# openGemini/openGemini

Measured on NVIDIA H100. Metric: decoded+aggregated rows/s, higher is better.
Workload: dtype f64

## Files before the change

### include/ogpu.h

```cpp
#ifndef OGPU_H
#define OGPU_H

#include <stddef.h>
#include <stdint.h>

#ifdef __cplusplus
extern "C" {
#endif

#define OG_API __attribute__((visibility("default")))

enum {
    OG_OK = 0,
    OG_EOF = 1,
    OG_E_INVAL = -1,
    OG_E_CUDA = -2,
    OG_E_NOMEM = -3,
    OG_E_UNSUPPORTED = -4,
    OG_E_CORRUPT = -5,
    OG_E_ABORTED = -6,
    OG_E_TYPE = -7,
    OG_E_STATE = -8
};

enum { OG_TYPE_INT = 1, OG_TYPE_FLOAT = 3, OG_TYPE_STRING = 4, OG_TYPE_BOOL = 5 };

enum { OG_AGG_COUNT = 1, OG_AGG_SUM = 2, OG_AGG_MIN = 3, OG_AGG_MAX = 4, OG_AGG_FIRST = 5, OG_AGG_LAST = 6 };

enum { OG_F_TERM = 0, OG_F_AND = 1, OG_F_OR = 2 };
enum { OG_OP_LT = 0, OG_OP_LTE = 1, OG_OP_GT = 2, OG_OP_GTE = 3, OG_OP_EQ = 4, OG_OP_NEQ = 5 };

typedef struct og_filter_item {
    int32_t kind;
    int32_t column;
    int32_t op;
    int32_t const_is_float;
    double fval;
    int64_t ival;
} og_filter_item;

typedef struct og_call {
    int32_t func;
    int32_t column;
} og_call;

enum { OG_GROUP_ALL = 0, OG_GROUP_PER_SERIES = 1, OG_GROUP_MAP = 2 };
enum {
    OG_Q_STRICT_ORDER = 1u << 0
    ,
    OG_Q_NO_FUSED = 1u << 1
    ,
    OG_Q_NO_FAST = 1u << 2
    ,
    OG_Q_RESERVED_8 = 1u << 3
    ,
    OG_Q_QUERY_GRID = 1u << 4
};

typedef struct og_query_desc {
    int64_t interval;
    int64_t offset;
    int64_t tmin, tmax;
    int32_t ascending;
    uint32_t n_calls;
    const og_call *calls;
    uint32_t n_filter;
    const og_filter_item *filter;
    int32_t group_mode;
    uint32_t n_groups;
    const uint32_t *series_group;
    int32_t chunk_size;
    uint32_t flags;
} og_query_desc;

typedef struct og_column_desc {
    const char *name;
    int32_t type;
    const uint64_t *page_off;
    const uint32_t *page_len;
} og_column_desc;

enum {
    OG_SHARD_DEVICE_DATA = 1u << 0
};

typedef struct og_shard_desc {
    const uint8_t *data;
    uint64_t data_len;
    uint32_t n_series;
    const uint64_t *sids;
    const uint32_t *series_seg_begin;
    uint32_t n_segments;
    const int64_t *seg_tmin;
    const int64_t *seg_tmax;
    uint32_t n_columns;
    const og_column_desc *columns;
    const uint64_t *time_page_off;
    const uint32_t *time_page_len;
    uint32_t flags;
} og_shard_desc;

typedef struct og_colval_view {
    const uint8_t *val;
    uint64_t val_bytes;
    const uint8_t *bitmap;
    const int64_t *times;
    int32_t type;
    int32_t len;
    int32_t nil_count;
    int32_t bitmap_offset;
} og_colval_view;

typedef struct og_record_view {
    uint32_t n_cols;
    const og_colval_view *cols;
    const int64_t *times;
    int32_t rows;
    uint32_t group;
    uint64_t sid;
} og_record_view;

typedef struct og_dense_col {
    void *values;
    uint8_t *valid;
    int64_t *times;
    int32_t type;
    int32_t func;
} og_dense_col;

typedef struct og_dense_view {
    uint32_t n_groups;
    uint32_t n_buckets;
    int64_t start;
    int64_t interval;
    uint32_t n_cols;
    const og_dense_col *cols;
    void *stream;
} og_dense_view;

typedef struct og_stats {
    uint64_t rows_decoded;
    uint64_t segments_scanned;
    uint64_t page_bytes;
    uint64_t dir_bytes;
    uint64_t out_bytes;
    double kernel_ms;
    double h2d_ms;
    double main_kernel_ms;
    uint32_t kernel_launches;
    int32_t path;
    int32_t il_state;
    int32_t per_series_cells_used;
    double il_build_ms;
    uint64_t il_bytes;
    uint64_t general_segments;
    double merge_ms;
    uint64_t il_packed_segments;
} og_stats;

typedef struct og_shard og_shard;
typedef struct og_query og_query;

OG_API int og_init(int device_ordinal);
OG_API int og_device_count(void);
OG_API const char *og_strerror(int status);
OG_API const char *og_last_error(void);
OG_API const char *og_version(void);
OG_API int og_release_cached_memory(void);

typedef struct og_tssp og_tssp;
OG_API int og_tssp_parse(const uint8_t *file, uint64_t len, og_tssp **out);
OG_API int og_tssp_desc(const og_tssp *t, og_shard_desc *out);
OG_API const char *og_tssp_measurement(const og_tssp *t);
OG_API int og_tssp_time_range(const og_tssp *t, int64_t *min_time, int64_t *max_time);
OG_API void og_tssp_free(og_tssp *t);

OG_API int og_shard_open(const og_shard_desc *desc, og_shard **out);
OG_API void og_shard_close(og_shard *s);
OG_API int og_shard_info(const og_shard *s, uint64_t *n_series, uint64_t *n_segments, uint64_t *n_rows,
                         uint64_t *page_bytes, int64_t *tmin, int64_t *tmax);

enum { OG_FILE_OUT_OF_ORDER = 1u << 0 };
OG_API int og_shard_open_files(const og_shard_desc *files, const uint32_t *file_flags, uint32_t n_files, og_shard **out);
typedef struct og_merge_info {
    uint32_t n_files, n_out_of_order_files;
    uint64_t series_merged;
    uint64_t out_of_order_rows;
    uint64_t rows_replaced;
    uint64_t rows_after_merge;
    uint64_t segments_kept;
    uint64_t segments_rewritten_in, segments_rewritten_out;
    double merge_ms;
} og_merge_info;
OG_API int og_shard_merge_info(const og_shard *s, og_merge_info *out);

OG_API int og_shard_append_files(og_shard *s, const og_shard_desc *files, const uint32_t *file_flags, uint32_t n_files);

typedef struct og_compact_desc {
    uint32_t rows_per_segment;
    uint32_t flags;
} og_compact_desc;
typedef struct og_compact_info {
    uint64_t series_rewritten;
    uint64_t segments_kept;
    uint64_t segments_rewritten_in, segments_rewritten_out;
    uint64_t rows_rewritten;
    double compact_ms;
} og_compact_info;
OG_API int og_shard_compact(og_shard *s, const og_compact_desc *d, og_compact_info *info );

OG_API int og_query_create(og_shard *s, const og_query_desc *desc, og_query **out);
OG_API int og_query_run(og_query *q);
OG_API int og_query_next(og_query *q, og_record_view *out);
OG_API int og_query_dense(og_query *q, og_dense_view *out);
OG_API int og_query_stats(const og_query *q, og_stats *out);
OG_API void og_query_abort(og_query *q);
OG_API void og_query_destroy(og_query *q);

OG_API int og_query_merge_dense(og_query *q, const og_dense_view *other);

typedef struct og_comm og_comm;
OG_API int og_comm_unique_id(uint8_t id[128]);
OG_API int og_comm_init_rank(const uint8_t id[128], int rank, int world, og_comm **out);
OG_API void og_comm_destroy(og_comm *c);
OG_API int og_comm_info(const og_comm *c, int *rank, int *world, int *nccl_version);
OG_API int og_comm_allreduce_f64(og_comm *c, double *vals, int n, int op_max);
OG_API int og_query_allreduce(og_query *q, og_comm *c);

OG_API int og_decode_segment(og_shard *s, uint32_t segment, og_record_view *out);
enum { OG_DECODE_DESCENDING = 1u << 0 };
OG_API int og_decode_segment_ex(og_shard *s, uint32_t segment, uint32_t flags, og_record_view *out);
OG_API int og_decode_column_device(og_shard *s, uint32_t column, uint32_t seg_begin, uint32_t seg_end,
                                   void *d_values, uint64_t value_stride_bytes, uint32_t *d_rows_out);

enum { OG_SYNTH_F_HI = 0, OG_SYNTH_F_LO = 1, OG_SYNTH_INT_WALK = 2, OG_SYNTH_BOOL = 3 };
typedef struct og_synth_column {
    int32_t type;
    int32_t dist;
    uint32_t null_permille;
} og_synth_column;
typedef struct og_synth_desc {
    uint32_t n_series;
    uint32_t rows_per_series;
    uint32_t rows_per_segment;
    int64_t t0;
    int64_t dt;
    uint64_t seed;
    uint32_t n_columns;
    const og_synth_column *columns;
    uint32_t series_base;
} og_synth_desc;
OG_API int og_shard_synth(const og_synth_desc *desc, og_shard **out);
typedef struct og_shard_layout {
    uint64_t data_len;
    uint32_t n_series, n_segments, n_columns;
} og_shard_layout;
OG_API int og_shard_layout_get(const og_shard *s, og_shard_layout *out);
OG_API int og_shard_export(const og_shard *s, uint8_t *data, uint64_t *sids, uint32_t *series_seg_begin,
                           int64_t *seg_tmin, int64_t *seg_tmax, uint64_t *page_off ,
                           uint32_t *page_len, int32_t *col_types );

OG_API int og_encode_pages(int32_t type, int32_t is_time, const void *d_values, const uint8_t *d_valid,
                           const uint32_t *d_rows , uint32_t n_segments,
                           uint32_t rows_per_segment, uint8_t *d_out, uint64_t out_cap, uint64_t *d_page_off,
                           uint32_t *d_page_len, uint64_t *total_bytes_out);

typedef struct og_downsampled og_downsampled;
OG_API int og_downsample(og_shard *s, uint32_t column, int64_t interval, int64_t tmin, int64_t tmax, og_downsampled **out);

typedef struct og_downsample_ops {
    int32_t type;
    uint32_t n_funcs;
    const int32_t *funcs;
} og_downsample_ops;
typedef struct og_downsample_desc {
    int64_t interval, tmin, tmax;
    uint32_t n_types;
    const og_downsample_ops *ops;
} og_downsample_desc;
OG_API int og_downsample_shard(og_shard *s, const og_downsample_desc *d, og_downsampled **out);
OG_API int og_downsampled_timing(const og_downsampled *d, double phase_ms[4]);
OG_API int og_downsampled_desc(const og_downsampled *d, og_shard_desc *desc, uint64_t *rows );
OG_API int og_downsampled_export(const og_downsampled *d, uint8_t *host_data );
OG_API void og_downsampled_free(og_downsampled *d);

typedef struct og_tssp_write_desc {
    const char *measurement;
    uint32_t series_begin, series_end;
    uint32_t flags;
} og_tssp_write_desc;
typedef struct og_tssp_image og_tssp_image;
OG_API int og_shard_write_tssp(og_shard *s, const og_tssp_write_desc *d, og_tssp_image **out);
OG_API int og_tssp_image_size(const og_tssp_image *f, uint64_t *bytes);
OG_API int og_tssp_image_export(const og_tssp_image *f, uint8_t *host);
OG_API int og_tssp_image_timing(const og_tssp_image *f, double phase_ms[4]);
OG_API void og_tssp_image_free(og_tssp_image *f);

#ifdef __cplusplus
}
#endif
#endif
```

### opengemini_b200/_lib.py

```python
import ctypes as C
import os

_HERE = os.path.dirname(os.path.abspath(__file__))
LIB_PATH = os.environ.get("OGPU_LIB") or os.path.join(_HERE, "libogpu.so")

OG_OK, OG_EOF = 0, 1
OG_E_INVAL, OG_E_CUDA, OG_E_NOMEM, OG_E_UNSUPPORTED, OG_E_CORRUPT, OG_E_ABORTED, OG_E_TYPE, OG_E_STATE = -1, -2, -3, -4, -5, -6, -7, -8
TYPE_INT, TYPE_FLOAT, TYPE_STRING, TYPE_BOOL = 1, 3, 4, 5
AGG_COUNT, AGG_SUM, AGG_MIN, AGG_MAX, AGG_FIRST, AGG_LAST = 1, 2, 3, 4, 5, 6
F_TERM, F_AND, F_OR = 0, 1, 2
OP_LT, OP_LTE, OP_GT, OP_GTE, OP_EQ, OP_NEQ = 0, 1, 2, 3, 4, 5
GROUP_ALL, GROUP_PER_SERIES, GROUP_MAP = 0, 1, 2
Q_STRICT_ORDER = 1
Q_NO_FUSED = 2
Q_NO_FAST = 4
Q_QUERY_GRID = 16
SYNTH_F_HI, SYNTH_F_LO, SYNTH_INT_WALK, SYNTH_BOOL = 0, 1, 2, 3
SHARD_DEVICE_DATA = 1
FILE_OUT_OF_ORDER = 1

u8p, u32p, u64p, i64p, i32p = C.POINTER(C.c_uint8), C.POINTER(C.c_uint32), C.POINTER(C.c_uint64), C.POINTER(C.c_int64), C.POINTER(C.c_int32)


class FilterItem(C.Structure):
    _fields_ = [("kind", C.c_int32), ("column", C.c_int32), ("op", C.c_int32), ("const_is_float", C.c_int32),
                ("fval", C.c_double), ("ival", C.c_int64)]


class Call(C.Structure):
    _fields_ = [("func", C.c_int32), ("column", C.c_int32)]


class QueryDesc(C.Structure):
    _fields_ = [("interval", C.c_int64), ("offset", C.c_int64), ("tmin", C.c_int64), ("tmax", C.c_int64),
                ("ascending", C.c_int32), ("n_calls", C.c_uint32), ("calls", C.POINTER(Call)),
                ("n_filter", C.c_uint32), ("filter", C.POINTER(FilterItem)), ("group_mode", C.c_int32),
                ("n_groups", C.c_uint32), ("series_group", u32p), ("chunk_size", C.c_int32), ("flags", C.c_uint32)]


class ColumnDesc(C.Structure):
    _fields_ = [("name", C.c_char_p), ("type", C.c_int32), ("page_off", u64p), ("page_len", u32p)]


class ShardDesc(C.Structure):
    _fields_ = [("data", u8p), ("data_len", C.c_uint64), ("n_series", C.c_uint32), ("sids", u64p),
                ("series_seg_begin", u32p), ("n_segments", C.c_uint32), ("seg_tmin", i64p), ("seg_tmax", i64p),
                ("n_columns", C.c_uint32), ("columns", C.POINTER(ColumnDesc)), ("time_page_off", u64p),
                ("time_page_len", u32p), ("flags", C.c_uint32)]


class ColValView(C.Structure):
    _fields_ = [("val", u8p), ("val_bytes", C.c_uint64), ("bitmap", u8p), ("times", i64p), ("type", C.c_int32),
                ("len", C.c_int32), ("nil_count", C.c_int32), ("bitmap_offset", C.c_int32)]


class RecordView(C.Structure):
    _fields_ = [("n_cols", C.c_uint32), ("cols", C.POINTER(ColValView)), ("times", i64p), ("rows", C.c_int32),
                ("group", C.c_uint32), ("sid", C.c_uint64)]


class DenseCol(C.Structure):
    _fields_ = [("values", C.c_void_p), ("valid", C.c_void_p), ("times", C.c_void_p), ("type", C.c_int32), ("func", C.c_int32)]


class DenseView(C.Structure):
    _fields_ = [("n_groups", C.c_uint32), ("n_buckets", C.c_uint32), ("start", C.c_int64), ("interval", C.c_int64),
                ("n_cols", C.c_uint32), ("cols", C.POINTER(DenseCol)), ("stream", C.c_void_p)]


class Stats(C.Structure):
    _fields_ = [("rows_decoded", C.c_uint64), ("segments_scanned", C.c_uint64), ("page_bytes", C.c_uint64),
                ("dir_bytes", C.c_uint64), ("out_bytes", C.c_uint64), ("kernel_ms", C.c_double), ("h2d_ms", C.c_double), ("main_kernel_ms", C.c_double),
                ("kernel_launches", C.c_uint32), ("path", C.c_int32), ("il_state", C.c_int32), ("per_series_cells_used", C.c_int32),
                ("il_build_ms", C.c_double), ("il_bytes", C.c_uint64), ("general_segments", C.c_uint64), ("merge_ms", C.c_double),
                ("il_packed_segments", C.c_uint64)]


class SynthColumn(C.Structure):
    _fields_ = [("type", C.c_int32), ("dist", C.c_int32), ("null_permille", C.c_uint32)]


class SynthDesc(C.Structure):
    _fields_ = [("n_series", C.c_uint32), ("rows_per_series", C.c_uint32), ("rows_per_segment", C.c_uint32),
                ("t0", C.c_int64), ("dt", C.c_int64), ("seed", C.c_uint64), ("n_columns", C.c_uint32),
                ("columns", C.POINTER(SynthColumn)), ("series_base", C.c_uint32)]


class ShardLayout(C.Structure):
    _fields_ = [("data_len", C.c_uint64), ("n_series", C.c_uint32), ("n_segments", C.c_uint32), ("n_columns", C.c_uint32)]


class DownsampleOps(C.Structure):
    _fields_ = [("type", C.c_int32), ("n_funcs", C.c_uint32), ("funcs", i32p)]


class DownsampleDesc(C.Structure):
    _fields_ = [("interval", C.c_int64), ("tmin", C.c_int64), ("tmax", C.c_int64), ("n_types", C.c_uint32),
                ("ops", C.POINTER(DownsampleOps))]


class MergeInfo(C.Structure):
    _fields_ = [("n_files", C.c_uint32), ("n_out_of_order_files", C.c_uint32), ("series_merged", C.c_uint64),
                ("out_of_order_rows", C.c_uint64), ("rows_replaced", C.c_uint64), ("rows_after_merge", C.c_uint64),
                ("segments_kept", C.c_uint64), ("segments_rewritten_in", C.c_uint64), ("segments_rewritten_out", C.c_uint64),
                ("merge_ms", C.c_double)]


class CompactDesc(C.Structure):
    _fields_ = [("rows_per_segment", C.c_uint32), ("flags", C.c_uint32)]


class CompactInfo(C.Structure):
    _fields_ = [("series_rewritten", C.c_uint64), ("segments_kept", C.c_uint64), ("segments_rewritten_in", C.c_uint64),
                ("segments_rewritten_out", C.c_uint64), ("rows_rewritten", C.c_uint64), ("compact_ms", C.c_double)]


class TsspWriteDesc(C.Structure):
    _fields_ = [("measurement", C.c_char_p), ("series_begin", C.c_uint32), ("series_end", C.c_uint32), ("flags", C.c_uint32)]


EXPORTS = [
    "og_init", "og_device_count", "og_strerror", "og_last_error", "og_version", "og_shard_open", "og_shard_close",
    "og_shard_info", "og_query_create", "og_query_run", "og_query_next", "og_query_dense", "og_query_stats",
    "og_query_abort", "og_query_destroy", "og_query_merge_dense", "og_decode_segment", "og_decode_segment_ex", "og_decode_column_device",
    "og_shard_synth", "og_shard_layout_get", "og_shard_export", "og_encode_pages",
    "og_release_cached_memory", "og_comm_unique_id", "og_comm_init_rank", "og_comm_destroy", "og_comm_info", "og_comm_allreduce_f64", "og_query_allreduce",
    "og_downsample", "og_downsampled_desc", "og_downsampled_export", "og_downsampled_free",
    "og_downsample_shard", "og_downsampled_timing",
    "og_tssp_parse", "og_tssp_desc", "og_tssp_measurement", "og_tssp_time_range", "og_tssp_free",
    "og_shard_open_files", "og_shard_merge_info", "og_shard_append_files", "og_shard_compact",
    "og_shard_write_tssp", "og_tssp_image_size", "og_tssp_image_export", "og_tssp_image_timing", "og_tssp_image_free",
]

_lib = None


class OgpuError(RuntimeError):
    def __init__(self, status, where):
        self.status = status
        msg = lib().og_last_error().decode(errors="replace")
        super().__init__(f"{where}: {lib().og_strerror(status).decode()} ({status}) {msg}")


def lib():
    global _lib
    if _lib is not None:
        return _lib
    if not os.path.exists(LIB_PATH):
        raise RuntimeError(f"{LIB_PATH} is missing: run `python -c 'import __graft_entry__ as g; g.build()'` "
                           "(nvcc, sm_90a). There is no CPU fallback for the scan/aggregate path.")
    L = C.CDLL(LIB_PATH)
    L.og_strerror.restype = C.c_char_p
    L.og_strerror.argtypes = [C.c_int]
    L.og_last_error.restype = C.c_char_p
    L.og_version.restype = C.c_char_p
    L.og_init.argtypes = [C.c_int]
    L.og_shard_open.argtypes = [C.POINTER(ShardDesc), C.POINTER(C.c_void_p)]
    L.og_shard_open_files.argtypes = [C.POINTER(ShardDesc), u32p, C.c_uint32, C.POINTER(C.c_void_p)]
    L.og_shard_merge_info.argtypes = [C.c_void_p, C.POINTER(MergeInfo)]
    L.og_shard_append_files.argtypes = [C.c_void_p, C.POINTER(ShardDesc), u32p, C.c_uint32]
    L.og_shard_compact.argtypes = [C.c_void_p, C.POINTER(CompactDesc), C.POINTER(CompactInfo)]
    L.og_shard_close.argtypes = [C.c_void_p]
    L.og_shard_close.restype = None
    L.og_shard_info.argtypes = [C.c_void_p, u64p, u64p, u64p, u64p, i64p, i64p]
    L.og_query_create.argtypes = [C.c_void_p, C.POINTER(QueryDesc), C.POINTER(C.c_void_p)]
    L.og_query_run.argtypes = [C.c_void_p]
    L.og_query_next.argtypes = [C.c_void_p, C.POINTER(RecordView)]
    L.og_query_dense.argtypes = [C.c_void_p, C.POINTER(DenseView)]
    L.og_query_stats.argtypes = [C.c_void_p, C.POINTER(Stats)]
    L.og_query_abort.argtypes = [C.c_void_p]
    L.og_query_abort.restype = None
    L.og_query_destroy.argtypes = [C.c_void_p]
    L.og_query_destroy.restype = None
    L.og_query_merge_dense.argtypes = [C.c_void_p, C.POINTER(DenseView)]
    L.og_decode_segment.argtypes = [C.c_void_p, C.c_uint32, C.POINTER(RecordView)]
    L.og_downsample.argtypes = [C.c_void_p, C.c_uint32, C.c_int64, C.c_int64, C.c_int64, C.POINTER(C.c_void_p)]
    L.og_downsample_shard.argtypes = [C.c_void_p, C.POINTER(DownsampleDesc), C.POINTER(C.c_void_p)]
    L.og_downsampled_timing.argtypes = [C.c_void_p, C.POINTER(C.c_double)]
    L.og_downsampled_desc.argtypes = [C.c_void_p, C.POINTER(ShardDesc), C.POINTER(C.c_uint64)]
    L.og_downsampled_export.argtypes = [C.c_void_p, C.c_void_p]
    L.og_downsampled_free.argtypes = [C.c_void_p]
    L.og_downsampled_free.restype = None
    L.og_tssp_parse.argtypes = [C.c_void_p, C.c_uint64, C.POINTER(C.c_void_p)]
    L.og_tssp_desc.argtypes = [C.c_void_p, C.POINTER(ShardDesc)]
    L.og_tssp_measurement.argtypes = [C.c_void_p]
    L.og_tssp_measurement.restype = C.c_char_p
    L.og_tssp_time_range.argtypes = [C.c_void_p, C.POINTER(C.c_int64), C.POINTER(C.c_int64)]
    L.og_tssp_free.argtypes = [C.c_void_p]
    L.og_tssp_free.restype = None
    L.og_shard_write_tssp.argtypes = [C.c_void_p, C.POINTER(TsspWriteDesc), C.POINTER(C.c_void_p)]
    L.og_tssp_image_size.argtypes = [C.c_void_p, u64p]
    L.og_tssp_image_export.argtypes = [C.c_void_p, C.c_void_p]
    L.og_tssp_image_timing.argtypes = [C.c_void_p, C.POINTER(C.c_double)]
    L.og_tssp_image_free.argtypes = [C.c_void_p]
    L.og_tssp_image_free.restype = None
    L.og_decode_segment_ex.argtypes = [C.c_void_p, C.c_uint32, C.c_uint32, C.POINTER(RecordView)]
    L.og_decode_column_device.argtypes = [C.c_void_p, C.c_uint32, C.c_uint32, C.c_uint32, C.c_void_p, C.c_uint64, C.c_void_p]
    L.og_shard_synth.argtypes = [C.POINTER(SynthDesc), C.POINTER(C.c_void_p)]
    L.og_shard_layout_get.argtypes = [C.c_void_p, C.POINTER(ShardLayout)]
    L.og_shard_export.argtypes = [C.c_void_p, C.c_void_p, C.c_void_p, C.c_void_p, C.c_void_p, C.c_void_p, C.c_void_p, C.c_void_p, C.c_void_p]
    L.og_encode_pages.argtypes = [C.c_int32, C.c_int32, C.c_void_p, C.c_void_p, C.c_void_p, C.c_uint32, C.c_uint32,
                                  C.c_void_p, C.c_uint64, C.c_void_p, C.c_void_p, u64p]
    L.og_comm_unique_id.argtypes = [C.c_void_p]
    L.og_comm_init_rank.argtypes = [C.c_void_p, C.c_int, C.c_int, C.POINTER(C.c_void_p)]
    L.og_comm_destroy.argtypes = [C.c_void_p]
    L.og_comm_destroy.restype = None
    L.og_comm_info.argtypes = [C.c_void_p, C.POINTER(C.c_int), C.POINTER(C.c_int), C.POINTER(C.c_int)]
    L.og_comm_allreduce_f64.argtypes = [C.c_void_p, C.POINTER(C.c_double), C.c_int, C.c_int]
    L.og_query_allreduce.argtypes = [C.c_void_p, C.c_void_p]
    _lib = L
    return L


def check(status, where):
    if status != OG_OK:
        raise OgpuError(status, where)
```

### opengemini_b200/csrc/agg_kernels.cuh

```cuda
#pragma once
#include "agg_ops.cuh"
#include "decode.cuh"
#include "internal.h"

namespace ogpu {

#define OG_NO_BUCKET 0xFFFFFFFFu

struct DirP {
    const uint8_t *data;
    const uint64_t *page_off;
    const uint32_t *page_len;
    const uint32_t *seg_series, *seg_rows, *series_seg_begin;
    const int64_t *seg_tmin, *seg_tmax;
    uint32_t n_segments, n_columns;
};

struct ChunkP {
    uint32_t series_begin, series_end;
    uint32_t seg_begin, seg_end;
    Tri cells[OG_MAX_CALLS];
    uint32_t nb;
    Tri edges[OG_MAX_CALLS];
    uint32_t *edge_bucket;
    Tri gcells[OG_MAX_CALLS];
    uint32_t gc_cols, gc_tail0, gc_edge0, gc_col0;
    uint32_t J;
    int *err;
    int *flags;
};

__device__ __forceinline__ size_t cell_idx(const ChunkP &ch, uint32_t series, uint32_t b) { return (size_t)(series - ch.series_begin) * ch.nb + b; }

__device__ __forceinline__ void report_err(int *err, int code, uint32_t seg) {
    if (atomicCAS(&err[0], 0, code) == 0) err[1] = (int)seg;
}

__device__ __forceinline__ void store_part(const Tri &a, size_t i, const Part &p) {
    a.val[i] = p.v; a.ok[i] = (uint8_t)p.ok;
    if (a.tim) a.tim[i] = p.t;
}
__device__ __forceinline__ Part load_part(const Tri &a, size_t i) {
    Part p; p.ok = a.ok[i]; p.v = a.val[i]; p.t = a.tim ? a.tim[i] : 0; return p;
}
__device__ __forceinline__ void store_cell(const ChunkP &ch, int call, uint32_t series, uint32_t b, const Part &p) {
    store_part(ch.cells[call], cell_idx(ch, series, b), p);
    ch.flags[0] = 1;
}

struct SegWindows {
    const QueryP &q; const ChunkP &ch;
    const uint32_t seg; const size_t e; const uint32_t series;
    uint32_t cur_b = OG_NO_BUCKET, head_b = OG_NO_BUCKET; bool head_done = false;
    int64_t we = 0;

    __device__ __forceinline__ SegWindows(const QueryP &q_, const ChunkP &ch_, uint32_t seg_, size_t e_, uint32_t series_)
        : q(q_), ch(ch_), seg(seg_), e(e_), series(series_) {}
    template <int NC> __device__ __forceinline__ void flush(const Part (&parts)[NC], bool final) {
        if (cur_b == OG_NO_BUCKET) return;
#pragma unroll
        for (int c = 0; c < NC; c++) {
            if (!head_done) store_part(ch.edges[c], e, parts[c]);
            else if (final) store_part(ch.edges[c], e + 1, parts[c]);
            else if (parts[c].ok) store_cell(ch, c, series, cur_b, parts[c]);
        }
        if (!head_done) { head_done = true; head_b = cur_b; }
    }
    template <int NC> __device__ __forceinline__ bool enter(int64_t t, Part (&parts)[NC]) {
        if (cur_b != OG_NO_BUCKET && t < we) return true;
        flush(parts, false);
        cur_b = bucket_of(t, q.start, q.interval);
        if (cur_b >= q.n_buckets) { report_err(ch.err, D_CORRUPT, seg); cur_b = OG_NO_BUCKET; return false; }
        we = q.start + (int64_t)(cur_b + 1) * q.interval;
#pragma unroll
        for (int c = 0; c < NC; c++) parts[c] = part_empty();
        return true;
    }
    template <int NC> __device__ __forceinline__ void end(const Part (&parts)[NC]) {
        const uint32_t last_b = cur_b;
        const bool single = !head_done;
        flush(parts, true);
        ch.edge_bucket[e] = head_b;
        ch.edge_bucket[e + 1] = (single || head_b == OG_NO_BUCKET) ? OG_NO_BUCKET : last_b;
        if (head_b != OG_NO_BUCKET) ch.flags[1] = 1;
    }
};

__global__ void k_validate(DirP d, const int32_t *col_types, uint32_t *seg_rows, unsigned long long *totals ,
                           uint32_t *max_rows, int *err) {
    uint32_t seg = blockIdx.x * blockDim.x + threadIdx.x;
    if (seg >= d.n_segments) return;
    size_t ti = (size_t)d.n_columns * d.n_segments + seg;
    TimeDesc t;
    int rc = parse_time_page(d.data + d.page_off[ti], d.page_len[ti], t);
    if (rc == D_OK && t.rows == 0) rc = D_CORRUPT;
    if (rc == D_OK) {
        int64_t last = t.t0; bool unsorted = false;
        if (t.kind == 0) last = (int64_t)((uint64_t)t.t0 + (uint64_t)(t.rows - 1) * t.delta);
        else {
            TimeIter it; it.init(t);
            for (uint32_t i = 0; i < t.rows; i++) { const int64_t x = it.next(); unsorted |= x < last; last = x; }
            it.finish(); rc = it.err;
        }
        if (rc == D_OK && (t.t0 < d.seg_tmin[seg] || last > d.seg_tmax[seg] || last < t.t0 || unsorted)) rc = D_CORRUPT;
    }
    if (rc != D_OK) { report_err(err, rc, seg); seg_rows[seg] = 0; return; }
    seg_rows[seg] = t.rows;
    unsigned long long bytes = d.page_len[ti];
    for (uint32_t c = 0; c < d.n_columns; c++) {
        size_t pi = (size_t)c * d.n_segments + seg;
        uint32_t len = d.page_len[pi];
        if (len == 0) continue;
        bytes += len;
        PageHdr h;
        rc = parse_field_header(d.data + d.page_off[pi], len, col_types[c], t.rows, h);
        if (rc == D_OK && h.rows != t.rows) rc = D_CORRUPT;
        if (rc == D_OK && h.bitmap && hdr_valid_rows(h) != h.rows - h.nil_count) rc = D_CORRUPT;
        if (rc == D_OK && !h.one_row && h.nil_count < h.rows) {
            if (h.block_len < 1) rc = D_CORRUPT;
            else {
                int tag = __ldg(h.block) >> 4, ty = col_types[c];
                if (ty == OG_TYPE_FLOAT) rc = (tag == 0 || tag == 3 || tag == 4 || tag == 5) ? D_OK : (tag == 1 || tag == 2 || tag == 6) ? D_UNSUPPORTED : D_CORRUPT;
                else if (ty == OG_TYPE_INT) rc = (tag == 1 || tag == 2 || tag == 4) ? D_OK : tag == 3 ? D_UNSUPPORTED : D_CORRUPT;
                else if (ty == OG_TYPE_BOOL) rc = tag == 1 ? D_OK : D_CORRUPT;
                else if (ty == OG_TYPE_STRING) rc = D_OK;
                else rc = D_UNSUPPORTED;
            }
        }
        if (rc != D_OK) { report_err(err, rc, seg); return; }
    }
    atomicAdd(&totals[0], (unsigned long long)t.rows);
    atomicAdd(&totals[1], bytes);
    atomicMax(max_rows, t.rows);
    if (t.kind != 0 && t.kind != 3) atomicAdd(&totals[2], 1ull);
}

__global__ void k_fill_seg_series(const uint32_t *series_seg_begin, uint32_t n_series, uint32_t *seg_series) {
    uint32_t s = blockIdx.x;
    if (s >= n_series) return;
    for (uint32_t g = series_seg_begin[s] + threadIdx.x; g < series_seg_begin[s + 1]; g += blockDim.x) seg_series[g] = s;
}

struct TileP {
    uint32_t tile_begin, tile_end, R;
    uint32_t S;
    uint64_t *vals[OG_MAX_COLS];
    uint8_t *okb[OG_MAX_COLS];
    int64_t *times;
    uint8_t *keep;
};

__global__ void k_decode_tile(DirP d, QueryP q, TileP tp, int *err) {
    uint32_t seg = tp.tile_begin + blockIdx.x * blockDim.x + threadIdx.x;
    if (seg >= tp.tile_end) return;
    uint32_t slot = blockIdx.y;
    const size_t base = seg - tp.tile_begin, S = tp.S;
    uint32_t rows = d.seg_rows[seg];
    if (slot == q.n_cols) {
        size_t ti = (size_t)d.n_columns * d.n_segments + seg;
        TimeDesc t;
        int rc = parse_time_page(d.data + d.page_off[ti], d.page_len[ti], t);
        if (rc == D_OK) {
            TimeIter it; it.init(t);
            for (uint32_t i = 0; i < t.rows; i++) tp.times[base + i * S] = it.next();
            it.finish(); rc = it.err;
        }
        if (rc != D_OK) report_err(err, rc, seg);
        return;
    }
    size_t pi = (size_t)q.col_index[slot] * d.n_segments + seg;
    uint64_t *out = tp.vals[slot] + base; uint8_t *okb = tp.okb[slot] + base;
    ColIter it;
    it.init(d.data + d.page_off[pi], d.page_len[pi], q.col_type[slot], rows);
    for (uint32_t i = 0; i < rows; i++) { uint64_t v = 0; okb[i * S] = it.next(v); out[i * S] = v; }
    it.finish();
    if (it.err != D_OK) report_err(err, it.err, seg);
}

__device__ __forceinline__ bool term_pass(const FilterP &f, uint64_t raw) {
// ... 7 lines not shown
        case OG_OP_GTE: return !(v < c);
        case OG_OP_EQ: return !(v != c);
        default: return !(v == c);
        }
    }
    int64_t v = f.type == OG_TYPE_BOOL ? (int64_t)(raw != 0) : (int64_t)raw, c = f.ival;
    switch (f.op) {
    case OG_OP_LT: return !(v >= c);
    case OG_OP_LTE: return !(v > c);
    case OG_OP_GT: return !(v <= c);
    case OG_OP_GTE: return !(v < c);
    case OG_OP_EQ: return !(v != c);
    default: return !(v == c);
    }
}

__global__ void k_filter_tile(DirP d, QueryP q, TileP tp) {
    size_t idx = (size_t)blockIdx.x * blockDim.x + threadIdx.x;
    size_t total = (size_t)tp.S * tp.R;
    if (idx >= total) return;
    uint32_t row = (uint32_t)(idx / tp.S), sl = (uint32_t)(idx % tp.S);
    if (sl >= tp.tile_end - tp.tile_begin) return;
    if (row >= d.seg_rows[tp.tile_begin + sl]) { tp.keep[idx] = 0; return; }
    int64_t t = tp.times[idx];
    bool keep = t >= q.tmin && t <= q.tmax;
    if (keep && q.n_filter) {
        uint32_t stack = 0; int sp = 0;
        for (uint32_t i = 0; i < q.n_filter; i++) {
            const FilterP &f = q.filter[i];
            if (f.kind == OG_F_TERM) {
                bool pass = tp.okb[f.col_slot][idx] && term_pass(f, tp.vals[f.col_slot][idx]);
                stack |= (uint32_t)pass << sp; sp++;
            } else {
                uint32_t b = (stack >> (sp - 1)) & 1, a = (stack >> (sp - 2)) & 1;
                uint32_t r = f.kind == OG_F_AND ? (a & b) : (a | b);
                sp -= 2; stack &= ~(3u << sp); stack |= r << sp; sp++;
            }
        }
        keep = stack & 1;
    }
    tp.keep[idx] = keep;
}

__global__ void k_window_reduce(DirP d, QueryP q, TileP tp, ChunkP ch) {
    uint32_t sl = blockIdx.x * blockDim.x + threadIdx.x;
    uint32_t seg = tp.tile_begin + sl;
    if (seg >= tp.tile_end) return;
    const uint32_t rows = d.seg_rows[seg], series = d.seg_series[seg];
    const size_t S = tp.S, e = 2 * (size_t)(seg - ch.seg_begin);
    Part parts[OG_MAX_CALLS];
    uint32_t cur_b = OG_NO_BUCKET, head_b = OG_NO_BUCKET; bool head_done = false;
    int64_t we = 0;
    auto flush = [&](bool final) {
        if (cur_b == OG_NO_BUCKET) return;
        for (uint32_t c = 0; c < q.n_calls; c++) {
            if (!head_done) store_part(ch.edges[c], e, parts[c]);
            else if (final) store_part(ch.edges[c], e + 1, parts[c]);
            else if (parts[c].ok) store_cell(ch, (int)c, series, cur_b, parts[c]);
        }
        if (!head_done) { head_done = true; head_b = cur_b; }
    };
    for (uint32_t r = 0; r < rows; r++) {
        const size_t ix = (size_t)r * S + sl;
        const int64_t t = tp.times[ix];
        if (t < q.tmin) continue;
        if (t > q.tmax) break;
        if (cur_b == OG_NO_BUCKET || t >= we) {
            flush(false);
            cur_b = bucket_of(t, q.start, q.interval);
            if (cur_b >= q.n_buckets) { report_err(ch.err, D_CORRUPT, seg); cur_b = OG_NO_BUCKET; break; }
            we = q.start + (int64_t)(cur_b + 1) * q.interval;
#pragma unroll
            for (uint32_t c = 0; c < OG_MAX_CALLS; c++) parts[c] = part_empty();
        }
        if (!tp.keep[ix]) continue;
#pragma unroll
        for (uint32_t c = 0; c < OG_MAX_CALLS; c++) {
            if (c >= q.n_calls) break;
            const CallP &cp = q.calls[c];
            if (tp.okb[cp.col_slot][ix]) acc_row(cp.func, cp.type, parts[c], tp.vals[cp.col_slot][ix], t);
        }
    }
    flush(true);
    ch.edge_bucket[e] = head_b;
    ch.edge_bucket[e + 1] = (head_b == OG_NO_BUCKET || cur_b == head_b) ? OG_NO_BUCKET : cur_b;
}

struct EdgeRuns { uint32_t hb, tb, s_end; bool head_leader; };
__device__ __forceinline__ EdgeRuns edge_runs(const DirP &d, const ChunkP &ch, uint32_t seg, uint32_t series) {
    EdgeRuns r;
    const uint32_t s_first = d.series_seg_begin[series];
    r.s_end = d.series_seg_begin[series + 1];
    const uint32_t *eb = ch.edge_bucket;
    const size_t e = 2 * (size_t)(seg - ch.seg_begin);
    r.hb = eb[e]; r.tb = eb[e + 1];
    r.head_leader = true;
    if (r.hb != OG_NO_BUCKET && seg > s_first) {
        const size_t pe = e - 2;
        const uint32_t pb = eb[pe + 1] != OG_NO_BUCKET ? eb[pe + 1] : eb[pe];
        if (pb != OG_NO_BUCKET && pb == r.hb) r.head_leader = false;
    }
    return r;
}
__device__ __forceinline__ Part edge_stitch(const QueryP &q, const ChunkP &ch, const EdgeRuns &r, uint32_t seg, int which, uint32_t c) {
    const CallP &cp = q.calls[c];
    const uint32_t *eb = ch.edge_bucket;
    const size_t e = 2 * (size_t)(seg - ch.seg_begin);
    const uint32_t b = which == 0 ? r.hb : r.tb;
    Part acc = load_part(ch.edges[c], e + which);
    if (which == 1 || r.tb == OG_NO_BUCKET) {
        for (uint32_t nx = seg + 1; nx < r.s_end; nx++) {
            const size_t ne = 2 * (size_t)(nx - ch.seg_begin);
            if (eb[ne] != b) break;
            acc = series_merge(cp.func, cp.type, acc, load_part(ch.edges[c], ne));
            if (eb[ne + 1] != OG_NO_BUCKET) break;
        }
    }
    return acc;
}

__global__ void k_fix_edges(DirP d, QueryP q, ChunkP ch) {
    uint32_t seg = ch.seg_begin + blockIdx.x * blockDim.x + threadIdx.x;
    if (seg >= ch.seg_end) return;
    const uint32_t series = d.seg_series[seg];
    const EdgeRuns r = edge_runs(d, ch, seg, series);
    if (r.hb == OG_NO_BUCKET) return;
    for (int which = 0; which < 2; which++) {
        if (which == 0 && !r.head_leader) continue;
        if (which == 1 && r.tb == OG_NO_BUCKET) continue;
        const uint32_t b = which == 0 ? r.hb : r.tb;
        if (b >= q.n_buckets) { report_err(ch.err, D_CORRUPT, seg); continue; }
        for (uint32_t c = 0; c < q.n_calls; c++) {
            const Part acc = edge_stitch(q, ch, r, seg, which, c);
            if (acc.ok) store_cell(ch, (int)c, series, b, acc);
        }
    }
}

__device__ __forceinline__ Part shfl_xor_part(const Part &p, int o, bool with_time) {
    Part r; r.v = __shfl_xor_sync(0xffffffffu, p.v, o); r.ok = __shfl_xor_sync(0xffffffffu, p.ok, o);
    r.t = with_time ? __shfl_xor_sync(0xffffffffu, p.t, o) : 0;
    return r;
}
__device__ __forceinline__ Part warp_fold(int func, int type, bool multi, Part p, bool with_time) {
#pragma unroll
    for (int o = 16; o; o >>= 1) { const Part other = shfl_xor_part(p, o, with_time); group_update(func, type, multi, p, other); }
    return p;
}
__device__ __forceinline__ bool call_has_time(const QueryP &q, uint32_t c) { return q.calls[c].func >= OG_AGG_MIN && !(q.multi && q.calls[c].func <= OG_AGG_MAX); }
__device__ __forceinline__ int call_ftype(const QueryP &q, uint32_t c) { return q.calls[c].func == OG_AGG_COUNT ? OG_TYPE_INT : q.calls[c].type; }

__global__ void k_fix_edges_fold(DirP d, QueryP q, ChunkP ch) {
    if (ch.flags[1] == 0) return;
    const uint32_t w = (blockIdx.x * blockDim.x + threadIdx.x) >> 5, lane = threadIdx.x & 31;
    const uint32_t n_blk = (ch.series_end - ch.series_begin + 31) / 32;
    if (w >= n_blk * ch.J) return;
    const uint32_t blk = w / ch.J, j = w % ch.J;
    const uint32_t series = ch.series_begin + blk * 32 + lane;
    const bool in = series < ch.series_end;
    const uint32_t seg = in ? d.series_seg_begin[series] + j : 0;
    EdgeRuns r; r.hb = r.tb = OG_NO_BUCKET; r.head_leader = false; r.s_end = 0;
    if (in) r = edge_runs(d, ch, seg, series);
    const uint32_t n_bk = (ch.gc_cols - ch.gc_edge0) / 3;
    for (int which = 0; which < 2; which++) {
        const uint32_t gcol = ch.gc_edge0 + (which ? 2u : (j & 1u)) * n_bk + ch.series_begin / 32 + blk - ch.gc_col0;
        const bool has = r.hb != OG_NO_BUCKET && (which == 0 ? r.head_leader : r.tb != OG_NO_BUCKET);
        const uint32_t b = which == 0 ? r.hb : r.tb;
        const uint32_t hm = __ballot_sync(0xffffffffu, has);
        if (hm == 0) continue;
        const int leader = __ffs(hm) - 1;
        const uint32_t bL = __shfl_sync(0xffffffffu, b, leader);
        const bool unif = __all_sync(0xffffffffu, !has || b == bL) && bL < q.n_buckets;
        if (!unif && has && b >= q.n_buckets) { report_err(ch.err, D_CORRUPT, seg); continue; }
        for (uint32_t c = 0; c < q.n_calls; c++) {
            Part acc = part_empty();
            if (has) acc = edge_stitch(q, ch, r, seg, which, c);
            if (unif) {
                acc = warp_fold(q.calls[c].func, call_ftype(q, c), q.multi != 0, acc, call_has_time(q, c));
                if ((int)lane == leader && acc.ok) store_part(ch.gcells[c], (size_t)bL * ch.gc_cols + gcol, acc);
            } else if (has && acc.ok) store_cell(ch, (int)c, series, b, acc);
        }
    }
}

struct GroupP {
    const uint32_t *grp_begin;
    const uint32_t *grp_series;
    uint32_t n_groups;
    Tri dense[OG_MAX_CALLS];
};

__global__ void k_merge_groups(QueryP q, ChunkP ch, GroupP gp) {
    if (ch.flags[0] == 0) return;
    size_t idx = (size_t)blockIdx.x * blockDim.x + threadIdx.x;
    size_t total = (size_t)gp.n_groups * q.n_buckets;
    if (idx >= total) return;
    uint32_t g = (uint32_t)(idx / q.n_buckets), b = (uint32_t)(idx % q.n_buckets);
    uint32_t lo = gp.grp_begin[g], hi = gp.grp_begin[g + 1];
    {
        uint32_t a = lo, z = hi;
        while (a < z) { uint32_t m = (a + z) >> 1; if (gp.grp_series[m] < ch.series_begin) a = m + 1; else z = m; }
        lo = a;
    }
    if (lo >= hi || gp.grp_series[lo] >= ch.series_end) return;
    {
        const uint32_t c = blockIdx.y;
        const CallP &cp = q.calls[c];
        Part acc = load_part(gp.dense[c], idx);
        const Tri cells = ch.cells[c];
        constexpr int U = 16;
        for (uint32_t i = lo; i < hi; i += U) {
            uint32_t okv[U]; uint64_t vv[U]; int64_t tt[U];
#pragma unroll
            for (int u = 0; u < U; u++) {
                uint32_t ii = i + u;
                uint32_t s = ii < hi ? gp.grp_series[ii] : 0xffffffffu;
                bool in = s < ch.series_end;
                size_t ci = in ? cell_idx(ch, s, b) : 0;
                okv[u] = in ? cells.ok[ci] : 0;
                vv[u] = okv[u] ? cells.val[ci] : 0;
                tt[u] = (okv[u] && cells.tim) ? cells.tim[ci] : 0;
            }
#pragma unroll
            for (int u = 0; u < U; u++) {
                if (!okv[u]) continue;
                Part p; p.ok = 1; p.v = vv[u]; p.t = tt[u];
                group_update(cp.func, cp.out_type == OG_TYPE_INT && cp.func == OG_AGG_COUNT ? OG_TYPE_INT : cp.type, q.multi != 0, acc, p);
            }
        }
        store_part(gp.dense[c], idx, acc);
    }
}

__global__ void k_merge_per_series(QueryP q, ChunkP ch, GroupP gp) {
    const uint32_t c = blockIdx.y;
    const size_t n = (size_t)(ch.series_end - ch.series_begin) * q.n_buckets;
    const size_t i = (size_t)blockIdx.x * blockDim.x + threadIdx.x;
    if (i >= n) return;
    const CallP &cp = q.calls[c];
    const int ftype = cp.out_type == OG_TYPE_INT && cp.func == OG_AGG_COUNT ? OG_TYPE_INT : cp.type;
    const uint32_t b = (uint32_t)(i % q.n_buckets);
    Part p; p.ok = ch.cells[c].ok[i]; p.v = p.ok ? ch.cells[c].val[i] : 0; p.t = (p.ok && ch.cells[c].tim) ? ch.cells[c].tim[i] : 0;
    Part a; a.v = 0; a.ok = 0; a.t = q.multi ? 0 : q.start + (int64_t)b * q.interval;
    group_update(cp.func, ftype, q.multi != 0, a, p);
    store_part(gp.dense[c], (size_t)ch.series_begin * q.n_buckets + i, a);
}

#define OG_MERGE_SB 256u
__global__ void __launch_bounds__(128) k_merge_all_blocks(QueryP q, ChunkP ch, GroupP gp) {
    if (ch.flags[0] == 0) return;
    const uint32_t b = blockIdx.x * blockDim.x + threadIdx.x, blk = blockIdx.y, c = blockIdx.z;
    if (b >= q.n_buckets) return;
    const uint32_t nS = ch.series_end - ch.series_begin;
    const uint32_t s0 = blk * OG_MERGE_SB, s1 = min(nS, s0 + OG_MERGE_SB);
    const int func = q.calls[c].func, ftype = call_ftype(q, c);
    const bool multi = q.multi != 0;
    const Tri cells = ch.cells[c];
    Part acc = part_empty();
    constexpr int U = 8;
    for (uint32_t s = s0; s < s1; s += U) {
        uint32_t okv[U]; uint64_t vv[U]; int64_t tt[U];
#pragma unroll
        for (int u = 0; u < U; u++) {
            const bool in = s + u < s1;
            const size_t ci = in ? (size_t)(s + u) * ch.nb + b : 0;
            okv[u] = in ? cells.ok[ci] : 0;
            vv[u] = okv[u] ? cells.val[ci] : 0;
            tt[u] = (okv[u] && cells.tim) ? cells.tim[ci] : 0;
        }
#pragma unroll
        for (int u = 0; u < U; u++) {
            if (!okv[u]) continue;
            Part p; p.ok = 1; p.v = vv[u]; p.t = tt[u];
            group_update(func, ftype, multi, acc, p);
        }
    }
    if (acc.ok) store_part(ch.gcells[c], (size_t)b * ch.gc_cols + blk, acc);
}

__global__ void k_merge_folded(QueryP q, ChunkP ch, GroupP gp) {
    const uint32_t b = (blockIdx.x * blockDim.x + threadIdx.x) >> 5, lane = threadIdx.x & 31, c = blockIdx.y;
    if (b >= q.n_buckets) return;
    const int func = q.calls[c].func, ftype = call_ftype(q, c);
    const bool wt = call_has_time(q, c), multi = q.multi != 0;
    const Tri g = ch.gcells[c];
    Part acc = part_empty();
    const size_t row = (size_t)b * ch.gc_cols;
    for (uint32_t col = lane; col < ch.gc_cols; col += 32) {
        if (!g.ok[row + col]) continue;
        Part p; p.ok = 1; p.v = g.val[row + col]; p.t = wt ? g.tim[row + col] : 0;
        group_update(func, ftype, multi, acc, p);
    }
    acc = warp_fold(func, ftype, multi, acc, wt);
    if (lane == 0 && acc.ok) {
        Part a = load_part(gp.dense[c], b);
        group_update(func, ftype, multi, a, acc);
        store_part(gp.dense[c], b, a);
    }
}

__global__ void k_init_dense(QueryP q, GroupP gp) {
    size_t idx = (size_t)blockIdx.x * blockDim.x + threadIdx.x;
    size_t total = (size_t)gp.n_groups * q.n_buckets;
    if (idx >= total) return;
    uint32_t b = (uint32_t)(idx % q.n_buckets);
    for (uint32_t c = 0; c < q.n_calls; c++) {
        gp.dense[c].val[idx] = 0; gp.dense[c].ok[idx] = 0;
        if (gp.dense[c].tim) gp.dense[c].tim[idx] = q.multi ? 0 : q.start + (int64_t)b * q.interval;
    }
}

__global__ void k_merge_dense(QueryP q, GroupP mine, GroupP other) {
    size_t idx = (size_t)blockIdx.x * blockDim.x + threadIdx.x;
    size_t total = (size_t)mine.n_groups * q.n_buckets;
    if (idx >= total) return;
    for (uint32_t c = 0; c < q.n_calls; c++) {
        const CallP &cp = q.calls[c];
        Part a = load_part(mine.dense[c], idx), p = load_part(other.dense[c], idx);
        group_update(cp.func, cp.func == OG_AGG_COUNT ? OG_TYPE_INT : cp.type, q.multi != 0, a, p);
        store_part(mine.dense[c], idx, a);
    }
}

}
```

### opengemini_b200/csrc/api.cu

```cuda
#include <algorithm>
#include <cstdarg>
#include <cstdio>
#include <cstring>
#include <numeric>

#include "agg_kernels.cuh"
#include "il_build.cuh"
#include "fused_multi.cuh"
#include "fused_cols.cuh"
#include "snappy_load.cuh"
#include <cub/device/device_scan.cuh>
#include <cub/device/device_radix_sort.cuh>
#include "internal.h"

namespace ogpu {

static thread_local char g_err[512] = "";
void set_error(const char *fmt, ...) {
    va_list ap; va_start(ap, fmt); vsnprintf(g_err, sizeof g_err, fmt, ap); va_end(ap);
}
int cuda_fail(cudaError_t e, const char *what, const char *file, int line) {
    set_error("CUDA error %d (%s) at %s:%d: %s", (int)e, cudaGetErrorString(e), file, line, what);
    return OG_E_CUDA;
}
// ... 247 lines not shown
}

OG_API int og_shard_export(const og_shard *s, uint8_t *data, uint64_t *sids, uint32_t *series_seg_begin, int64_t *seg_tmin,
                           int64_t *seg_tmax, uint64_t *page_off, uint32_t *page_len, int32_t *col_types) {
    if (!s) return OG_E_INVAL;
    CU(cudaSetDevice(s->device));
    size_t nseg = s->n_segments, ncol1 = (size_t)s->n_columns + 1;
    if (data) CU(cudaMemcpy(data, s->d_data, s->data_len, cudaMemcpyDeviceToHost));
    if (sids) memcpy(sids, s->sids.data(), s->sids.size() * 8);
    if (series_seg_begin) memcpy(series_seg_begin, s->h_series_seg_begin.data(), s->h_series_seg_begin.size() * 4);
    if (seg_tmin) CU(cudaMemcpy(seg_tmin, s->d_tmin, nseg * 8, cudaMemcpyDeviceToHost));
    if (seg_tmax) CU(cudaMemcpy(seg_tmax, s->d_tmax, nseg * 8, cudaMemcpyDeviceToHost));
    if (page_off) CU(cudaMemcpy(page_off, s->d_page_off, ncol1 * nseg * 8, cudaMemcpyDeviceToHost));
    if (page_len) CU(cudaMemcpy(page_len, s->d_page_len, ncol1 * nseg * 4, cudaMemcpyDeviceToHost));
    if (col_types) memcpy(col_types, s->col_types.data(), s->col_types.size() * 4);
    return OG_OK;
}

static const int64_t MIN_TIME = INT64_MIN + 2, MAX_TIME = INT64_MAX - 1;
static void window_of(int64_t interval, int64_t offset, int64_t tmin, int64_t tmax, int64_t t, int64_t *s, int64_t *e) {
    if (interval == 0) { *s = tmin; *e = tmax + 1; return; }
    t -= offset;
    int64_t dt = t % interval;
    if (dt < 0) dt += interval;
    int64_t st = ((int64_t)((uint64_t)MIN_TIME + (uint64_t)dt) >= t) ? MIN_TIME : t - dt;
    st += offset;
    int64_t d2 = interval - dt;
    int64_t en = (MAX_TIME - d2 <= t) ? MAX_TIME : t + d2;
    en += offset;
    *s = st; *e = en;
}
static bool window_clamped(int64_t interval, int64_t offset, int64_t t) {
    const __int128 x = (__int128)t - offset;
    __int128 r = x % interval;
    if (r < 0) r += interval;
    const __int128 s = x - r, e = s + interval;
    return s < MIN_TIME || e > MAX_TIME || s + offset < INT64_MIN || e + offset > INT64_MAX;
}

}
namespace { void free_plan(void *plan); }
extern "C" void og_query_free_merge_state(void *p);
og_query::~og_query() {
    if (stream) cudaStreamSynchronize(stream);
    if (live) { std::lock_guard<std::mutex> lock(live->mu); live->n--; }
    og_query_free_merge_state(merge_state);
    free_plan(plan);
    if (ev0) cudaEventDestroy(ev0);
    if (ev1) cudaEventDestroy(ev1);
    for (cudaEvent_t e : main_ev) cudaEventDestroy(e);
    if (stream) cudaStreamDestroy(stream);
}
extern "C" {
OG_API void og_query_destroy(og_query *q) { delete q; }

OG_API int og_query_create(og_shard *s, const og_query_desc *d_in, og_query **out) {
    if (!s || !d_in || !out) { set_error("null argument"); return OG_E_INVAL; }
    *out = nullptr;
    og_query_desc d_clamped = *d_in;
    d_clamped.tmin = std::max(d_in->tmin, MIN_TIME); d_clamped.tmax = std::min(d_in->tmax, MAX_TIME);
    const og_query_desc *d = &d_clamped;
    CU(cudaSetDevice(s->device));
    if (d->n_calls == 0 || d->n_calls > OG_MAX_CALLS) { set_error("n_calls must be 1..%d", OG_MAX_CALLS); return OG_E_INVAL; }
    if (d->n_filter > OG_MAX_FILTER) { set_error("filter too long (max %d items)", OG_MAX_FILTER); return OG_E_INVAL; }
    if (d->interval < 0 || d->tmin > d->tmax) { set_error("bad interval or time range"); return OG_E_INVAL; }
    std::unique_ptr<og_query> q(new og_query);
    {
        std::lock_guard<std::mutex> lock(s->live->mu);
        s->live->n++;
        q->sh = s; q->live = s->live;
    }
    q->desc = *d;
    q->calls.assign(d->calls, d->calls + d->n_calls);
    if (d->n_filter) q->filter.assign(d->filter, d->filter + d->n_filter);
    q->desc.calls = q->calls.data(); q->desc.filter = q->filter.data();
    QueryP &p = q->qp;
    memset(&p, 0, sizeof p);
    auto slot_of = [&](int col) -> int {
        for (uint32_t i = 0; i < p.n_cols; i++) if (p.col_index[i] == col) return (int)i;
        if (p.n_cols >= OG_MAX_COLS) return -1;
        p.col_index[p.n_cols] = col; p.col_type[p.n_cols] = s->col_types[col];
        return (int)p.n_cols++;
    };
    for (uint32_t i = 0; i < d->n_calls; i++) {
        const og_call &c = d->calls[i];
        if (c.column < 0 || (uint32_t)c.column >= s->n_columns || c.func < OG_AGG_COUNT || c.func > OG_AGG_LAST) { set_error("call %u: bad column or function", i); return OG_E_INVAL; }
        int type = s->col_types[c.column];
        if (type == OG_TYPE_STRING && c.func != OG_AGG_COUNT) { set_error("call %u: only count() is pushed down for string columns (their values are never decoded on the GPU path)", i); return OG_E_UNSUPPORTED; }
        if (c.func == OG_AGG_SUM && type == OG_TYPE_BOOL) { set_error("sum() over a boolean column (unsupported sum iterator type, series_call_processor.go:140)"); return OG_E_INVAL; }
        int sl = slot_of(c.column);
        if (sl < 0) { set_error("too many distinct columns"); return OG_E_INVAL; }
        p.calls[i].func = c.func; p.calls[i].col_slot = sl; p.calls[i].type = type;
        p.calls[i].out_type = c.func == OG_AGG_COUNT ? OG_TYPE_INT : type;
    }
    p.n_calls = d->n_calls; p.multi = d->n_calls > 1;
    int sp = 0;
    for (uint32_t i = 0; i < d->n_filter; i++) {
        const og_filter_item &f = d->filter[i];
        FilterP &fp = p.filter[i];
        fp.kind = f.kind;
        if (f.kind == OG_F_TERM) {
            if (f.column < 0 || (uint32_t)f.column >= s->n_columns || f.op < OG_OP_LT || f.op > OG_OP_NEQ) { set_error("filter item %u: bad column or op", i); return OG_E_INVAL; }
            if (s->col_types[f.column] == OG_TYPE_STRING) { set_error("filter item %u: WHERE on a string column is not pushed down", i); return OG_E_UNSUPPORTED; }
            int sl = slot_of(f.column);
            if (sl < 0) { set_error("too many distinct columns"); return OG_E_INVAL; }
            fp.col_slot = sl; fp.op = f.op; fp.type = s->col_types[f.column]; fp.const_is_float = f.const_is_float; fp.fval = f.fval; fp.ival = f.ival;
            sp++;
        } else if (f.kind == OG_F_AND || f.kind == OG_F_OR) {
            if (sp < 2) { set_error("filter RPN underflow at item %u", i); return OG_E_INVAL; }
            sp--;
        } else { set_error("filter item %u: bad kind", i); return OG_E_INVAL; }
    }
    if (d->n_filter && sp != 1) { set_error("filter RPN does not reduce to one value"); return OG_E_INVAL; }
    p.n_filter = d->n_filter;
    int64_t gmin = std::max(d->tmin, s->tmin), gmax = std::min(d->tmax, s->tmax);
    bool overlap = gmin <= gmax;
    if (!overlap) gmin = gmax = d->tmin;
    if (d->flags & OG_Q_QUERY_GRID) {
        if (d_in->tmin <= MIN_TIME || d_in->tmax >= MAX_TIME) { set_error("OG_Q_QUERY_GRID needs a bounded time range"); return OG_E_INVAL; }
        gmin = d->tmin; gmax = d->tmax; overlap = true;
    }
    int64_t s0, e0, s1, e1;
    if (d->interval == 0) { s0 = gmin; e0 = gmax + 1; s1 = s0; e1 = e0; }
    else {
        if (overlap && (window_clamped(d->interval, d->offset, gmin) || window_clamped(d->interval, d->offset, gmax))) {
            set_error("the first or last window of the range is clamped at the int64 time limits"); return OG_E_UNSUPPORTED;
        }
        window_of(d->interval, d->offset, d->tmin, d->tmax, gmin, &s0, &e0);
        window_of(d->interval, d->offset, d->tmin, d->tmax, gmax + 1, &s1, &e1);
    }
    p.tmin = d->tmin; p.tmax = d->tmax; p.start = s0; p.interval = e0 - s0;
    if (p.interval <= 0) { set_error("degenerate window"); return OG_E_INVAL; }
    uint64_t nb = d->interval ? (uint64_t)(e1 - s0) / (uint64_t)p.interval : 1;
    if (nb == 0 || nb > 0x7fffffffull) { set_error("query range yields %llu buckets", (unsigned long long)nb); return OG_E_INVAL; }
    p.n_buckets = (uint32_t)nb;
    q->n_groups = d->group_mode == OG_GROUP_ALL ? 1 : d->group_mode == OG_GROUP_PER_SERIES ? s->n_series : d->n_groups;
    if (d->group_mode == OG_GROUP_MAP) {
        if (!d->series_group || d->n_groups == 0) { set_error("OG_GROUP_MAP needs series_group and n_groups"); return OG_E_INVAL; }
        q->series_group.assign(d->series_group, d->series_group + s->n_series);
        for (uint32_t g : q->series_group) if (g >= d->n_groups) { set_error("series_group entry out of range"); return OG_E_INVAL; }
    } else if (d->group_mode != OG_GROUP_ALL && d->group_mode != OG_GROUP_PER_SERIES) { set_error("bad group_mode"); return OG_E_INVAL; }
    if (q->n_groups == 0) q->n_groups = 1;
    cudaError_t e = cudaStreamCreateWithFlags(&q->stream, cudaStreamNonBlocking);
    if (e != cudaSuccess) return cuda_fail(e, "cudaStreamCreate", __FILE__, __LINE__);
    cudaEventCreate(&q->ev0); cudaEventCreate(&q->ev1);
    *out = q.release();
    return OG_OK;
}

OG_API void og_query_abort(og_query *q) { if (q) q->aborted = 1; }

}
namespace {
struct Plan {
    ChunkP ch; TileP tp; GroupP gp;
    bool fused;
    bool cols;
    bool multi;
    bool fast;
    bool blockmerge;
    bool fold;
    int fm; bool times;
    IlP il;
    const og_shard::IlCol *ic;
};
void free_plan(void *plan) { delete (Plan *)plan; }

template <int NC> void launch_fused(const DirP &d, const QueryP &p, const ChunkP &ch, const uint32_t *list, uint32_t n, cudaStream_t st) {
    if (n) k_fused_segment<NC><<<(n + 127) / 128, 128, 0, st>>>(d, p, ch, list, n);
}
template <int FM, bool TIMES> void launch_fast_t(bool fold, const IlP &il, uint32_t g0, uint32_t g1, const QueryP &p, const ChunkP &ch, cudaStream_t st) {
    constexpr uint32_t WPB = OG_FAST_THREADS / 32;
    dim3 grid((g1 - g0 + WPB - 1) / WPB), block(OG_FAST_THREADS);
    if (fold) k_fused_il<FM, TIMES, true><<<grid, block, WPB * il_acc_bytes(p.n_calls, TIMES), st>>>(p, ch, il, g0, g1);
    else k_fused_il<FM, TIMES, false><<<grid, block, 0, st>>>(p, ch, il, g0, g1);
}
void launch_fast(int fm, bool times, bool fold, const IlP &il, uint32_t g0, uint32_t g1, const QueryP &p, const ChunkP &ch, cudaStream_t st) {
    if (g1 <= g0) return;
    if (!times) {
        switch (fm) {
        case FM_SUM | FM_COUNT: return launch_fast_t<FM_SUM | FM_COUNT, false>(fold, il, g0, g1, p, ch, st);
        case FM_SUM | FM_COUNT | FM_MAX: return launch_fast_t<FM_SUM | FM_COUNT | FM_MAX, false>(fold, il, g0, g1, p, ch, st);
        case FM_SUM | FM_COUNT | FM_MIN | FM_MAX: return launch_fast_t<FM_SUM | FM_COUNT | FM_MIN | FM_MAX, false>(fold, il, g0, g1, p, ch, st);
        case FM_COUNT: return launch_fast_t<FM_COUNT, false>(fold, il, g0, g1, p, ch, st);
        default: break;
        }
    } else {
        switch (fm) {
        case FM_MAX | FM_COUNT: return launch_fast_t<FM_MAX | FM_COUNT, true>(fold, il, g0, g1, p, ch, st);
        case FM_MIN | FM_COUNT: return launch_fast_t<FM_MIN | FM_COUNT, true>(fold, il, g0, g1, p, ch, st);
        default: break;
        }
    }
    return launch_fast_t<63, true>(fold, il, g0, g1, p, ch, st);
}

template <int NCOL, int NCALL> void launch_multi_t(const QueryP &p, const DirP &d, const ChunkP &ch, uint32_t nseg, cudaStream_t st) {
    bool simple = true;
    for (uint32_t c = 0; c < p.n_calls; c++) simple &= p.calls[c].func == OG_AGG_COUNT || p.calls[c].func == OG_AGG_SUM;
    const unsigned gb = (nseg + 127) / 128;
    if (simple) k_fused_multi<NCOL, NCALL, true><<<gb, 128, 0, st>>>(d, p, ch);
    else k_fused_multi<NCOL, NCALL, false><<<gb, 128, 0, st>>>(d, p, ch);
}
template <int NCOL> void launch_multi_c(const QueryP &p, const DirP &d, const ChunkP &ch, uint32_t nseg, cudaStream_t st) {
    switch (p.n_calls) {
    case 1: return launch_multi_t<NCOL, 1>(p, d, ch, nseg, st);
    case 2: return launch_multi_t<NCOL, 2>(p, d, ch, nseg, st);
    case 3: return launch_multi_t<NCOL, 3>(p, d, ch, nseg, st);
    case 4: return launch_multi_t<NCOL, 4>(p, d, ch, nseg, st);
    case 5: return launch_multi_t<NCOL, 5>(p, d, ch, nseg, st);
    case 6: return launch_multi_t<NCOL, 6>(p, d, ch, nseg, st);
    case 7: return launch_multi_t<NCOL, 7>(p, d, ch, nseg, st);
    default: return launch_multi_t<NCOL, 8>(p, d, ch, nseg, st);
    }
}
void launch_cols(const QueryP &p, const DirP &d, const ChunkP &ch, uint32_t nseg, cudaStream_t st) {
    bool simple = true;
    for (uint32_t c = 0; c < p.n_calls; c++) simple &= p.calls[c].func == OG_AGG_COUNT || p.calls[c].func == OG_AGG_SUM;
    const unsigned gb = (nseg + 127) / 128;
    if (simple) k_fused_cols<true><<<gb, 128, 0, st>>>(d, p, ch);
    else k_fused_cols<false><<<gb, 128, 0, st>>>(d, p, ch);
}
void launch_multi(const QueryP &p, const DirP &d, const ChunkP &ch, uint32_t nseg, cudaStream_t st) {
    switch (p.n_cols) {
    case 1: return launch_multi_c<1>(p, d, ch, nseg, st);
    case 2: return launch_multi_c<2>(p, d, ch, nseg, st);
    case 3: return launch_multi_c<3>(p, d, ch, nseg, st);
#ifdef OG_WIDE_MULTI
    case 5: return launch_multi_c<5>(p, d, ch, nseg, st);
    case 6: return launch_multi_c<6>(p, d, ch, nseg, st);
    case 7: return launch_multi_c<7>(p, d, ch, nseg, st);
    case 8: return launch_multi_c<8>(p, d, ch, nseg, st);
#endif
    default: return launch_multi_c<4>(p, d, ch, nseg, st);
    }
}

int ensure_il(og_shard *s, int col, cudaStream_t st) {
    std::lock_guard<std::mutex> lock(s->il_mu);
    if (s->il.size() != s->n_columns) s->il.resize(s->n_columns);
    og_shard::IlCol &ic = s->il[col];
    if (ic.state != 0) return OG_OK;
    ic.state = -1;
    if (s->n_segments == 0 || s->col_types[col] != OG_TYPE_FLOAT) return OG_OK;
    const uint32_t nseg = s->n_segments;
    uint32_t J = s->n_series ? s->h_series_seg_begin[1] - s->h_series_seg_begin[0] : 0;
    for (uint32_t i = 0; i < s->n_series && J; i++) if (s->h_series_seg_begin[i + 1] - s->h_series_seg_begin[i] != J) J = 0;
    const uint32_t n_super = J ? (s->n_series + OG_IL_SUPER - 1) / OG_IL_SUPER : 1;
    const uint64_t n_dom64 = J ? (uint64_t)n_super * J : 1;
    if (n_dom64 >= (1ull << 31)) return OG_OK;
    const uint32_t n_dom = (uint32_t)n_dom64;
    int rc;
    struct Ev { cudaEvent_t e = nullptr; Ev() { cudaEventCreate(&e); } ~Ev() { if (e) cudaEventDestroy(e); } } ev0, ev1;
    cudaEventRecord(ev0.e, st);
    Scratch tmp(st);
    IlScanOut so{};
    uint32_t *seg_words; uint64_t *keys2; uint32_t *vals2;
    if ((rc = tmp.get(&so.seg_win, nseg)) || (rc = tmp.get(&so.n_packed, 1)) ||
        (rc = tmp.get(&seg_words, nseg)) || (rc = tmp.get(&so.seg_t0, nseg)) || (rc = tmp.get(&so.seg_dt, nseg)) || (rc = tmp.get(&so.keys, nseg)) ||
        (rc = tmp.get(&so.vals, nseg)) || (rc = tmp.get(&keys2, nseg)) || (rc = tmp.get(&vals2, nseg)) || (rc = tmp.get(&so.dom_cnt, n_dom))) return rc;
    so.seg_words = seg_words;
    if ((rc = tmp.get(&so.misaligned, 1))) return rc;
    CU(cudaMemsetAsync(so.dom_cnt, 0, (size_t)n_dom * 4, st));
    CU(cudaMemsetAsync(so.misaligned, 0, 4, st));
    CU(cudaMemsetAsync(so.n_packed, 0, 8, st));
    DirP d = make_dir(s);
    k_il_scan<<<(nseg + 255) / 256, 256, 0, st>>>(d, col, s->col_types[col], J, so);
    CU(cudaGetLastError());
    int dbits = 1; while ((1ull << dbits) < n_dom64 + 1) dbits++;
    {
        size_t tb = 0;
        CU(cub::DeviceRadixSort::SortPairs(nullptr, tb, so.keys, keys2, so.vals, vals2, (int)nseg, 0, (int)OG_IL_WORD_BITS + dbits, st));
        void *dtmp; if ((rc = tmp.get((uint8_t **)&dtmp, tb))) return rc;
        CU(cub::DeviceRadixSort::SortPairs(dtmp, tb, so.keys, keys2, so.vals, vals2, (int)nseg, 0, (int)OG_IL_WORD_BITS + dbits, st));
    }
    std::vector<uint32_t> dom_cnt(n_dom); uint32_t misaligned = 1; unsigned long long n_packed = 0;
    CU(cudaMemcpyAsync(dom_cnt.data(), so.dom_cnt, (size_t)n_dom * 4, cudaMemcpyDeviceToHost, st));
    CU(cudaMemcpyAsync(&misaligned, so.misaligned, 4, cudaMemcpyDeviceToHost, st));
    CU(cudaMemcpyAsync(&n_packed, so.n_packed, 8, cudaMemcpyDeviceToHost, st));
    CU(cudaStreamSynchronize(st));
    std::vector<uint32_t> elem_first(n_dom), grp_first(n_dom);
    uint64_t n_elig = 0, ng64 = 0;
    for (uint32_t i = 0; i < n_dom; i++) { elem_first[i] = (uint32_t)n_elig; grp_first[i] = (uint32_t)ng64; n_elig += dom_cnt[i]; ng64 += (dom_cnt[i] + 31) / 32; }
    const uint32_t n_gen = nseg - (uint32_t)n_elig;
    if (n_gen) {
        if ((rc = dalloc(&ic.gen_list, (size_t)n_gen))) return rc;
        CU(cudaMemcpyAsync(ic.gen_list, vals2 + n_elig, (size_t)n_gen * 4, cudaMemcpyDeviceToDevice, st));
        ic.gen_host.resize(n_gen);
        CU(cudaMemcpyAsync(ic.gen_host.data(), vals2 + n_elig, (size_t)n_gen * 4, cudaMemcpyDeviceToHost, st));
        CU(cudaStreamSynchronize(st));
    }
    if (n_elig == 0) return OG_OK;
    const uint32_t ng = (uint32_t)ng64;
    ic.n_groups = ng; ic.J = J; ic.aligned = J != 0 && misaligned == 0; ic.n_super = n_super; ic.cols_per_super = OG_IL_SUPER / 32 + 1;
    ic.super_grp_first.assign(n_super + 1, ng);
    for (uint32_t sp = 0; sp < n_super; sp++) ic.super_grp_first[sp] = grp_first[J ? sp * J : 0];
    uint32_t *d_elem_first, *d_grp_first;
    if ((rc = tmp.get(&d_elem_first, n_dom)) || (rc = tmp.get(&d_grp_first, n_dom))) return rc;
    CU(cudaMemcpyAsync(d_elem_first, elem_first.data(), (size_t)n_dom * 4, cudaMemcpyHostToDevice, st));
    CU(cudaMemcpyAsync(d_grp_first, grp_first.data(), (size_t)n_dom * 4, cudaMemcpyHostToDevice, st));
    const size_t n_slots = (size_t)ng * 32;
    if ((rc = dalloc(&ic.lane_seg, n_slots)) || (rc = dalloc(&ic.lane_rows, n_slots)) || (rc = dalloc(&ic.lane_win, n_slots)) || (rc = dalloc(&ic.lane_series, n_slots)) ||
        (rc = dalloc(&ic.lane_t0, n_slots)) || (rc = dalloc(&ic.lane_dt, n_slots)) || (rc = dalloc(&ic.grp_col, (size_t)ng)) ||
        (rc = dalloc(&ic.grp_rows, (size_t)ng)) || (rc = dalloc(&ic.grp_off, (size_t)ng))) return rc;
    CU(cudaMemsetAsync(ic.lane_seg, 0xff, n_slots * 4, st));
    CU(cudaMemsetAsync(ic.lane_rows, 0, n_slots * 4, st));
    CU(cudaMemsetAsync(ic.lane_win, 0, n_slots * 2, st));
    IlAssign as{};
    as.keys = keys2; as.segs = vals2; as.elem_first = d_elem_first; as.grp_first = d_grp_first;
    as.seg_words = seg_words; as.seg_t0 = so.seg_t0; as.seg_dt = so.seg_dt; as.seg_win = so.seg_win;
    as.lane_seg = ic.lane_seg; as.lane_rows = ic.lane_rows; as.lane_series = ic.lane_series; as.grp_col = ic.grp_col; as.lane_win = ic.lane_win; as.lane_t0 = ic.lane_t0; as.lane_dt = ic.lane_dt;
    as.n_elig = (uint32_t)n_elig; as.J = J; as.cols_per_super = ic.cols_per_super;
    k_il_assign<<<(unsigned)((n_elig + 255) / 256), 256, 0, st>>>(d, as);
    k_il_group_rows<<<(unsigned)((n_slots + 255) / 256), 256, 0, st>>>(ng, ic.lane_seg, seg_words, ic.grp_rows);
    CU(cudaGetLastError());
    std::vector<uint32_t> gw(ng); std::vector<uint64_t> go(ng);
    CU(cudaMemcpyAsync(gw.data(), ic.grp_rows, (size_t)ng * 4, cudaMemcpyDeviceToHost, st));
    CU(cudaStreamSynchronize(st));
    uint64_t total = 0;
    for (uint32_t g = 0; g < ng; g++) { go[g] = total; total += (uint64_t)gw[g] * 32; }
    size_t free_b = 0, total_b = 0;
    CU(dev_mem_info(&free_b, &total_b));
    size_t headroom = (size_t)8 << 30;
    if (const char *ov = getenv("OGPU_IL_HEADROOM_MB")) headroom = (size_t)atoll(ov) << 20;
    if (total * 4 + headroom > free_b || dev_malloc((void **)&ic.words, total * 4) != cudaSuccess) {
        cudaGetLastError(); ic.words = nullptr; ic.state = -2;
        return OG_OK;
    }
    CU(cudaMemcpyAsync(ic.grp_off, go.data(), (size_t)ng * 8, cudaMemcpyHostToDevice, st));
    k_il_repack<<<(unsigned)((n_slots + 127) / 128), 128, 0, st>>>(d, col, ic.lane_seg, ic.lane_win, ic.grp_off, ic.grp_rows, ng, ic.words);
    CU(cudaGetLastError());
    cudaEventRecord(ev1.e, st);
    CU(cudaStreamSynchronize(st));
    float ms = 0; cudaEventElapsedTime(&ms, ev0.e, ev1.e);
    ic.n_words = total; ic.n_packed = n_packed; ic.build_ms = ms; ic.state = 1;
    return OG_OK;
}

int build_plan(og_query *q) {
    og_shard *s = q->sh;
    const QueryP &p = q->qp;
    cudaStream_t st = q->stream;
    int rc;
    Plan *pl = new Plan;
    memset((void *)pl, 0, sizeof *pl);
    q->plan = pl;
    size_t cells_dense = (size_t)q->n_groups * p.n_buckets;
    for (uint32_t c = 0; c < p.n_calls; c++) {
        bool sel = p.calls[c].func >= OG_AGG_MIN && !(p.multi && p.calls[c].func <= OG_AGG_MAX);
        if ((rc = q->bufs.get(&q->dense[c].val, cells_dense))) return rc;
        if ((rc = q->bufs.get(&q->dense[c].ok, cells_dense))) return rc;
        if (sel && (rc = q->bufs.get(&q->dense[c].tim, cells_dense))) return rc;
    }
    std::vector<uint32_t> grp_begin(q->n_groups + 1, 0), grp_series(s->n_series);
    if (q->desc.group_mode == OG_GROUP_MAP) {
        for (uint32_t sr = 0; sr < s->n_series; sr++) grp_begin[q->series_group[sr] + 1]++;
        for (uint32_t g = 0; g < q->n_groups; g++) grp_begin[g + 1] += grp_begin[g];
        std::vector<uint32_t> cur(grp_begin.begin(), grp_begin.end() - 1);
        for (uint32_t sr = 0; sr < s->n_series; sr++) grp_series[cur[q->series_group[sr]]++] = sr;
    } else if (q->desc.group_mode == OG_GROUP_PER_SERIES) {
        for (uint32_t g = 0; g <= q->n_groups; g++) grp_begin[g] = std::min(g, s->n_series);
        std::iota(grp_series.begin(), grp_series.end(), 0u);
    } else { grp_begin[1] = s->n_series; std::iota(grp_series.begin(), grp_series.end(), 0u); }
    uint32_t *d_grp_begin, *d_grp_series;
    if ((rc = q->bufs.get(&d_grp_begin, grp_begin.size()))) return rc;
    if ((rc = q->bufs.get(&d_grp_series, grp_series.size()))) return rc;
    if ((rc = q->bufs.get(&q->d_err, 16))) return rc;
    CU(cudaMemcpyAsync(d_grp_begin, grp_begin.data(), grp_begin.size() * 4, cudaMemcpyHostToDevice, st));
    CU(cudaMemcpyAsync(d_grp_series, grp_series.data(), grp_series.size() * 4, cudaMemcpyHostToDevice, st));
    CU(cudaStreamSynchronize(st));
    pl->gp.grp_begin = d_grp_begin; pl->gp.grp_series = d_grp_series; pl->gp.n_groups = q->n_groups;
    for (uint32_t c = 0; c < p.n_calls; c++) pl->gp.dense[c] = q->dense[c];

    bool has_string = false;
    for (uint32_t k = 0; k < p.n_cols; k++) has_string |= p.col_type[k] == OG_TYPE_STRING;
    pl->fused = p.n_cols == 1 && p.n_filter == 0 && !has_string && !(q->desc.flags & OG_Q_NO_FUSED);
    const bool multi_ok = !pl->fused && (has_string || !(q->desc.flags & OG_Q_NO_FUSED));
    pl->cols = false;
    if (multi_ok && !(q->desc.flags & OG_Q_NO_FAST) && s->irregular_time_pages == 0 && s->max_seg_rows <= OG_COLS_MAXROWS &&
        (p.n_filter == 0 || (p.n_filter == 1 && p.filter[0].kind == OG_F_TERM)) && !getenv("OGPU_NO_COLS")) {
        pl->cols = true;
        for (uint32_t k = 0; k < p.n_cols; k++) {
            int n = 0;
            for (uint32_t c = 0; c < p.n_calls; c++) n += p.calls[c].col_slot == (int)k;
            if (n > OG_COLS_MAXMINE) pl->cols = false;
        }
    }
    if (has_string && !pl->cols && p.n_cols > OG_MULTI_MAXC) { set_error("a query that counts a string column may touch at most %d columns on this shard", OG_MULTI_MAXC); return OG_E_UNSUPPORTED; }
    pl->multi = pl->cols || (multi_ok && p.n_cols <= OG_MULTI_MAXC);
    q->path_used = pl->fused ? 1 : pl->cols ? 5 : pl->multi ? 4 : 0;
    const bool want_fast = pl->fused && p.col_type[0] == OG_TYPE_FLOAT && !(q->desc.flags & OG_Q_NO_FAST) && s->n_segments;
    if (want_fast && (rc = ensure_il(s, p.col_index[0], st))) return rc;
    pl->fast = want_fast && s->il[p.col_index[0]].state == 1;
    const og_shard::IlCol *ic = pl->fast ? &s->il[p.col_index[0]] : nullptr;
    pl->ic = ic;
    pl->fold = pl->fast && ic->J != 0 && ic->aligned && q->desc.group_mode == OG_GROUP_ALL && !(q->desc.flags & OG_Q_STRICT_ORDER);

    size_t cell_bytes_per_series = 0;
    for (uint32_t c = 0; c < p.n_calls; c++) cell_bytes_per_series += (size_t)p.n_buckets * (9 + (p.calls[c].func >= OG_AGG_MIN ? 8 : 0));
    size_t free_b = 0, total_b = 0;
    CU(dev_mem_info(&free_b, &total_b));
    size_t budget = std::min<size_t>(free_b / 3, (size_t)24 << 30);
    q->chunk_series = (uint32_t)std::max<size_t>(1, std::min<size_t>(s->n_series, budget / std::max<size_t>(1, cell_bytes_per_series)));
    if (const char *ov = getenv("OGPU_CHUNK_SERIES")) {
        long v = atol(ov);
        if (v > 0) q->chunk_series = (uint32_t)std::min<long>(v, (long)std::max<uint32_t>(1, s->n_series));
    }
    if (q->chunk_series < s->n_series) {
        if (q->chunk_series >= OG_IL_SUPER) q->chunk_series = q->chunk_series / OG_IL_SUPER * OG_IL_SUPER;
        else q->chunk_series = std::max<uint32_t>(32, q->chunk_series & ~31u);
    }
    uint32_t max_chunk_segs = 0;
    for (uint32_t a = 0; a < s->n_series; a += q->chunk_series) {
        uint32_t b = std::min(s->n_series, a + q->chunk_series);
        max_chunk_segs = std::max(max_chunk_segs, s->h_series_seg_begin[b] - s->h_series_seg_begin[a]);
    }
    ChunkP &ch = pl->ch;
    ch.err = q->d_err; ch.flags = q->d_err + 2;
    ch.nb = p.n_buckets;
    ch.J = ic ? ic->J : 0;
    size_t chunk_cells = (size_t)std::min(q->chunk_series, s->n_series) * p.n_buckets;
    for (uint32_t c = 0; c < p.n_calls; c++) {
        bool sel = p.calls[c].func >= OG_AGG_MIN;
        if ((rc = q->bufs.get(&ch.cells[c].val, chunk_cells))) return rc;
        if ((rc = q->bufs.get(&ch.cells[c].ok, chunk_cells))) return rc;
        if (sel && (rc = q->bufs.get(&ch.cells[c].tim, chunk_cells))) return rc;
        if ((rc = q->bufs.get(&ch.edges[c].val, 2 * (size_t)max_chunk_segs))) return rc;
        if ((rc = q->bufs.get(&ch.edges[c].ok, 2 * (size_t)max_chunk_segs))) return rc;
        if (sel && (rc = q->bufs.get(&ch.edges[c].tim, 2 * (size_t)max_chunk_segs))) return rc;
    }
    if ((rc = q->bufs.get(&ch.edge_bucket, 2 * (size_t)max_chunk_segs))) return rc;
    pl->blockmerge = !pl->fold && q->desc.group_mode == OG_GROUP_ALL && !(q->desc.flags & OG_Q_STRICT_ORDER) &&
                     (s->n_series > 2 * OG_MERGE_SB || getenv("OGPU_FORCE_BLOCKMERGE") );
    if (pl->blockmerge) {
        ch.gc_edge0 = 0; ch.gc_col0 = 0;
        ch.gc_cols = (std::min(q->chunk_series, s->n_series) + OG_MERGE_SB - 1) / OG_MERGE_SB;
        const size_t n = (size_t)p.n_buckets * ch.gc_cols;
        for (uint32_t c = 0; c < p.n_calls; c++) {
            bool sel = p.calls[c].func >= OG_AGG_MIN;
            if ((rc = q->bufs.get(&ch.gcells[c].val, n))) return rc;
            if ((rc = q->bufs.get(&ch.gcells[c].ok, n))) return rc;
            if (sel && (rc = q->bufs.get(&ch.gcells[c].tim, n))) return rc;
        }
    }
    if (pl->fold) {
        ch.gc_tail0 = ic->n_super * ic->cols_per_super; ch.gc_edge0 = 2 * ch.gc_tail0; ch.gc_col0 = 0;
        ch.gc_cols = ch.gc_edge0 + 3 * ((s->n_series + 31) / 32);
        const size_t n = (size_t)p.n_buckets * ch.gc_cols;
        for (uint32_t c = 0; c < p.n_calls; c++) {
            bool sel = p.calls[c].func >= OG_AGG_MIN;
            if ((rc = q->bufs.get(&ch.gcells[c].val, n))) return rc;
            if ((rc = q->bufs.get(&ch.gcells[c].ok, n))) return rc;
            if (sel && (rc = q->bufs.get(&ch.gcells[c].tim, n))) return rc;
        }
    }
    if (pl->fast) {
        pl->il.words = ic->words; pl->il.grp_off = ic->grp_off; pl->il.grp_rows = ic->grp_rows; pl->il.grp_col = ic->grp_col;
        pl->il.lane_seg = ic->lane_seg; pl->il.lane_rows = ic->lane_rows; pl->il.lane_win = ic->lane_win; pl->il.lane_series = ic->lane_series; pl->il.lane_t0 = ic->lane_t0; pl->il.lane_dt = ic->lane_dt;
        pl->fm = 0; pl->times = false;
        for (uint32_t c = 0; c < p.n_calls; c++) {
            pl->fm |= 1 << (p.calls[c].func - 1);
            if (p.calls[c].func >= OG_AGG_MIN && !(p.multi && p.calls[c].func <= OG_AGG_MAX)) pl->times = true;
        }
        pl->fm |= FM_COUNT;
        q->path_used = pl->fold ? 3 : 2;
    }
    if (!pl->fused && !pl->multi) {
        TileP &tp = pl->tp;
        tp.R = std::max<uint32_t>(1, s->max_seg_rows);
        size_t per_seg = (size_t)tp.R * (p.n_cols * 9 + 8 + 1);
        size_t fb = 0, tb = 0;
        CU(dev_mem_info(&fb, &tb));
        const size_t tile_budget = std::max<size_t>((size_t)96 << 20, std::min<size_t>(fb / 4, (size_t)12 << 30));
        q->tile_segs = (uint32_t)std::max<size_t>(1, std::min<size_t>(std::max<uint32_t>(1, max_chunk_segs), tile_budget / per_seg));
        q->tile_segs = std::max<uint32_t>(32, q->tile_segs & ~31u);
        tp.S = q->tile_segs;
        for (uint32_t k = 0; k < p.n_cols; k++) {
            if ((rc = q->bufs.get(&tp.vals[k], (size_t)q->tile_segs * tp.R))) return rc;
            if ((rc = q->bufs.get(&tp.okb[k], (size_t)q->tile_segs * tp.R))) return rc;
        }
        if ((rc = q->bufs.get(&tp.times, (size_t)q->tile_segs * tp.R))) return rc;
        if ((rc = q->bufs.get(&tp.keep, (size_t)q->tile_segs * tp.R))) return rc;
    }
    q->planned = true;
    return OG_OK;
}
}
extern "C" {

OG_API int og_query_run(og_query *q) {
    if (!q) return OG_E_INVAL;
    og_shard *s = q->sh;
    CU(cudaSetDevice(s->device));
    const QueryP &p = q->qp;
    cudaStream_t st = q->stream;
    int rc;
    q->host_ready = false; q->next_group = 0; q->next_row = 0;
    if (!q->planned) {
        if (q->plan) { set_error("query plan failed earlier"); return OG_E_STATE; }
        if ((rc = build_plan(q))) return rc;
    }
    Plan *pl = (Plan *)q->plan;
    ChunkP ch = pl->ch; TileP tp = pl->tp; const GroupP &gp = pl->gp;
    size_t cells_dense = (size_t)q->n_groups * p.n_buckets;
    DirP dir = make_dir(s);
    uint32_t launches = 0, n_chunks = (s->n_series + q->chunk_series - 1) / q->chunk_series;
    while (q->main_ev.size() < 2 * (size_t)n_chunks) { cudaEvent_t e; CU(cudaEventCreate(&e)); q->main_ev.push_back(e); }
    CU(cudaMemsetAsync(q->d_err, 0, 64, st));
    CU(cudaEventRecord(q->ev0, st));
    const bool per_series = q->desc.group_mode == OG_GROUP_PER_SERIES;
    if (!per_series) { k_init_dense<<<(unsigned)((cells_dense + 255) / 256), 256, 0, st>>>(p, gp); launches++; }
    const bool clear_cells = !pl->fold || q->cells_dirty || n_chunks > 1;
    uint64_t segs_scanned = 0; uint32_t ci = 0, chunks_run = 0;
    for (uint32_t a = 0; a < s->n_series; a += q->chunk_series, ci++) {
        if (q->aborted) { cudaStreamSynchronize(st); set_error("query aborted"); return OG_E_ABORTED; }
        uint32_t b = std::min(s->n_series, a + q->chunk_series);
        ch.series_begin = a; ch.series_end = b;
        ch.seg_begin = s->h_series_seg_begin[a]; ch.seg_end = s->h_series_seg_begin[b];
        uint32_t nseg = ch.seg_end - ch.seg_begin;
        const size_t chunk_cells = (size_t)(b - a) * p.n_buckets;
        if (nseg == 0) {
            if (per_series) {
                for (uint32_t c = 0; c < p.n_calls; c++) CU(cudaMemsetAsync(ch.cells[c].ok, 0, chunk_cells, st));
                k_merge_per_series<<<dim3((unsigned)((chunk_cells + 255) / 256), p.n_calls), 256, 0, st>>>(p, ch, gp);
                launches++;
            }
            continue;
        }
        segs_scanned += nseg;
        if (clear_cells) for (uint32_t c = 0; c < p.n_calls; c++) CU(cudaMemsetAsync(ch.cells[c].ok, 0, chunk_cells, st));
        if (pl->fold || pl->blockmerge) for (uint32_t c = 0; c < p.n_calls; c++) CU(cudaMemsetAsync(ch.gcells[c].ok, 0, (size_t)p.n_buckets * ch.gc_cols, st));
        if (pl->fold && ci > 0) CU(cudaMemsetAsync(ch.flags + 1, 0, sizeof(int), st));
        CU(cudaEventRecord(q->main_ev[2 * chunks_run], st));
        if (pl->fused) {
            const uint32_t *gl = nullptr; uint32_t gn = nseg;
            if (pl->fast) {
                const og_shard::IlCol &ic = *pl->ic;
                uint32_t g0 = 0, g1 = ic.n_groups;
                if (ic.J) { g0 = ic.super_grp_first[a / OG_IL_SUPER]; g1 = ic.super_grp_first[std::min<uint32_t>(ic.n_super, (b + OG_IL_SUPER - 1) / OG_IL_SUPER)]; }
                launch_fast(pl->fm, pl->times, pl->fold, pl->il, g0, g1, p, ch, st); launches++;
                auto lo = std::lower_bound(ic.gen_host.begin(), ic.gen_host.end(), ch.seg_begin);
                auto hi = std::lower_bound(ic.gen_host.begin(), ic.gen_host.end(), ch.seg_end);
                gl = ic.gen_list + (lo - ic.gen_host.begin()); gn = (uint32_t)(hi - lo);
            }
            if (gn) {
                switch (p.n_calls) {
                case 1: launch_fused<1>(dir, p, ch, gl, gn, st); break;
                case 2: launch_fused<2>(dir, p, ch, gl, gn, st); break;
                case 3: launch_fused<3>(dir, p, ch, gl, gn, st); break;
                case 4: launch_fused<4>(dir, p, ch, gl, gn, st); break;
                case 5: launch_fused<5>(dir, p, ch, gl, gn, st); break;
                case 6: launch_fused<6>(dir, p, ch, gl, gn, st); break;
                case 7: launch_fused<7>(dir, p, ch, gl, gn, st); break;
                default: launch_fused<8>(dir, p, ch, gl, gn, st); break;
                }
                launches++;
            }
        } else if (pl->cols) {
            launch_cols(p, dir, ch, nseg, st);
        } else if (pl->multi) {
            launch_multi(p, dir, ch, nseg, st);
            launches++;
        } else {
            for (uint32_t t0 = ch.seg_begin; t0 < ch.seg_end; t0 += q->tile_segs) {
                tp.tile_begin = t0; tp.tile_end = std::min(ch.seg_end, t0 + q->tile_segs);
                uint32_t n = tp.tile_end - tp.tile_begin;
                dim3 g((n + 127) / 128, p.n_cols + 1);
                k_decode_tile<<<g, 128, 0, st>>>(dir, p, tp, q->d_err);
                size_t rows_total = (size_t)tp.S * tp.R;
                k_filter_tile<<<(unsigned)((rows_total + 255) / 256), 256, 0, st>>>(dir, p, tp);
                k_window_reduce<<<(n + 127) / 128, 128, 0, st>>>(dir, p, tp, ch);
                launches += 3;
            }
        }
        CU(cudaEventRecord(q->main_ev[2 * chunks_run + 1], st));
        chunks_run++;
        if (pl->fold) k_fix_edges_fold<<<(unsigned)(((size_t)((b - a + 31) / 32) * ch.J * 32 + 127) / 128), 128, 0, st>>>(dir, p, ch);
        else k_fix_edges<<<(nseg + 127) / 128, 128, 0, st>>>(dir, p, ch);
        if (per_series) k_merge_per_series<<<dim3((unsigned)((chunk_cells + 255) / 256), p.n_calls), 256, 0, st>>>(p, ch, gp);
        else if (pl->blockmerge) k_merge_all_blocks<<<dim3((p.n_buckets + 127) / 128, (b - a + OG_MERGE_SB - 1) / OG_MERGE_SB, p.n_calls), 128, 0, st>>>(p, ch, gp);
        else k_merge_groups<<<dim3((unsigned)((cells_dense + 127) / 128), p.n_calls), 128, 0, st>>>(p, ch, gp);
        launches += 2;
        if (pl->fold || pl->blockmerge) { k_merge_folded<<<dim3((unsigned)(((size_t)p.n_buckets * 32 + 127) / 128), p.n_calls), 128, 0, st>>>(p, ch, gp); launches++; }
    }
    CU(cudaEventRecord(q->ev1, st));
    CU(cudaGetLastError());
    CU(cudaStreamSynchronize(st));
    int err[16];
    CU(cudaMemcpy(err, q->d_err, 64, cudaMemcpyDeviceToHost));
    if (getenv("OGPU_IL_STATS")) {
        unsigned long long wait, life, pro, epi;
        memcpy(&wait, err + 8, 8); memcpy(&life, err + 10, 8); memcpy(&pro, err + 12, 8); memcpy(&epi, err + 14, 8);
        const double pc = life ? 100.0 / (double)life : 0.0;
        fprintf(stderr, "[ogpu] fused rounds: common %d rare %d (lanes not resident in %d, sit-outs %d); warp cycles: %llu waiting for batches of %llu (%.1f %%), "
                "prologue %llu (%.1f %%), epilogue %llu (%.1f %%)\n",
                err[4], err[5], err[6], err[7], wait, life, pc * (double)wait, pro, pc * (double)pro, epi, pc * (double)epi);
    }
    q->cells_dirty = err[2] != 0;
    if (err[0]) { set_error("segment %d failed to decode (device code %d)", err[1], err[0]); return map_dev_err(err[0]); }
    float ms = 0; cudaEventElapsedTime(&ms, q->ev0, q->ev1);
    double main_ms = 0;
    for (uint32_t i = 0; i < chunks_run; i++) { float m = 0; cudaEventElapsedTime(&m, q->main_ev[2 * i], q->main_ev[2 * i + 1]); main_ms += m; }
    og_stats &stt = q->stats;
    uint64_t keep_pb = stt.page_bytes, keep_rows = stt.rows_decoded, keep_segs = stt.segments_scanned;
    memset(&stt, 0, sizeof stt);
    stt.kernel_ms = ms; stt.main_kernel_ms = main_ms; stt.kernel_launches = launches; stt.path = q->path_used;
    stt.page_bytes = keep_pb; stt.rows_decoded = keep_pb ? keep_rows : s->n_rows; stt.segments_scanned = keep_pb ? keep_segs : segs_scanned;
    stt.dir_bytes = (uint64_t)segs_scanned * 32;
    stt.out_bytes = 0;
    for (uint32_t c = 0; c < p.n_calls; c++) stt.out_bytes += cells_dense * (9 + (q->dense[c].tim ? 8 : 0));
    if (p.n_cols == 1 && p.col_type[0] == OG_TYPE_FLOAT && p.col_index[0] < (int)s->il.size()) {
        const og_shard::IlCol &ic = s->il[p.col_index[0]];
        stt.il_state = ic.state; stt.il_build_ms = ic.build_ms; stt.il_bytes = ic.n_words * 4; stt.il_packed_segments = ic.state == 1 ? ic.n_packed : 0;
        stt.general_segments = ic.state == 1 ? (uint64_t)ic.gen_host.size() : s->n_segments;
    }
    stt.per_series_cells_used = err[2] != 0;
    q->ran = true;
    return OG_OK;
}

OG_API int og_query_dense(og_query *q, og_dense_view *out) {
    if (!q || !out) return OG_E_INVAL;
    if (!q->ran) { set_error("og_query_dense before og_query_run"); return OG_E_STATE; }
    const QueryP &p = q->qp;
    out->n_groups = q->n_groups; out->n_buckets = p.n_buckets; out->start = q->desc.interval ? p.start : 0; out->interval = q->desc.interval ? p.interval : 0;
    out->n_cols = p.n_calls;
    for (uint32_t c = 0; c < p.n_calls; c++) {
        q->dense_cols[c].values = q->dense[c].val; q->dense_cols[c].valid = q->dense[c].ok; q->dense_cols[c].times = q->dense[c].tim;
        q->dense_cols[c].type = p.calls[c].out_type; q->dense_cols[c].func = p.calls[c].func;
    }
    out->cols = q->dense_cols; out->stream = q->stream;
    return OG_OK;
}

}
namespace {
__global__ void k_sum_page_bytes(DirP d, QueryP q, int64_t tmin, int64_t tmax, unsigned long long *out ) {
    uint32_t seg = blockIdx.x * blockDim.x + threadIdx.x;
    if (seg >= d.n_segments) return;
    if (d.seg_tmax[seg] < tmin || d.seg_tmin[seg] > tmax) return;
    unsigned long long b = d.page_len[(size_t)d.n_columns * d.n_segments + seg];
    for (uint32_t k = 0; k < q.n_cols; k++) b += d.page_len[(size_t)q.col_index[k] * d.n_segments + seg];
    atomicAdd(&out[0], b); atomicAdd(&out[1], (unsigned long long)d.seg_rows[seg]); atomicAdd(&out[2], 1ull);
}
}
extern "C" {

OG_API int og_query_stats(const og_query *q, og_stats *out) {
    if (!q || !out) return OG_E_INVAL;
    og_query *mq = const_cast<og_query *>(q);
    if (q->ran && q->stats.page_bytes == 0) {
        CU(cudaSetDevice(q->sh->device));
        Scratch tmp;
        unsigned long long *d_o; int rc = tmp.get(&d_o, 3); if (rc) return rc;
        cudaMemset(d_o, 0, 24);
        if (q->sh->n_segments) k_sum_page_bytes<<<(q->sh->n_segments + 255) / 256, 256>>>(make_dir(q->sh), q->qp, q->qp.tmin, q->qp.tmax, d_o);
        unsigned long long h[3]; CU(cudaMemcpy(h, d_o, 24, cudaMemcpyDeviceToHost));
        mq->stats.page_bytes = h[0]; mq->stats.rows_decoded = h[1]; mq->stats.segments_scanned = h[2];
    }
    *out = q->stats;
    return OG_OK;
}

OG_API int og_query_merge_dense(og_query *q, const og_dense_view *other) {
    if (!q || !other) return OG_E_INVAL;
    if (!q->ran) return OG_E_STATE;
    const QueryP &p = q->qp;
    if (other->n_groups != q->n_groups || other->n_buckets != p.n_buckets || other->n_cols != p.n_calls) { set_error("dense shapes differ"); return OG_E_INVAL; }
    if (other->start != (q->desc.interval ? p.start : 0) || other->interval != (q->desc.interval ? p.interval : 0)) {
        set_error("dense grids differ (start %lld vs %lld, interval %lld vs %lld): create the queries with OG_Q_QUERY_GRID", (long long)other->start,
                  (long long)(q->desc.interval ? p.start : 0), (long long)other->interval, (long long)(q->desc.interval ? p.interval : 0));
        return OG_E_INVAL;
    }
    CU(cudaSetDevice(q->sh->device));
    GroupP mine, oth; memset(&mine, 0, sizeof mine); memset(&oth, 0, sizeof oth);
    mine.n_groups = oth.n_groups = q->n_groups;
    for (uint32_t c = 0; c < p.n_calls; c++) {
        mine.dense[c] = q->dense[c];
        oth.dense[c].val = (uint64_t *)other->cols[c].values; oth.dense[c].ok = other->cols[c].valid; oth.dense[c].tim = other->cols[c].times;
        if ((q->dense[c].tim != nullptr) != (oth.dense[c].tim != nullptr)) { set_error("dense column %u: times presence differs", c); return OG_E_INVAL; }
    }
    size_t total = (size_t)q->n_groups * p.n_buckets;
    k_merge_dense<<<(unsigned)((total + 255) / 256), 256, 0, q->stream>>>(p, mine, oth);
    CU(cudaGetLastError());
    CU(cudaStreamSynchronize(q->stream));
    q->host_ready = false;
    return OG_OK;
}

OG_API int og_query_next(og_query *q, og_record_view *out) {
    if (!q || !out) return OG_E_INVAL;
    if (!q->ran) { set_error("og_query_next before og_query_run"); return OG_E_STATE; }
    if (q->aborted) return OG_E_ABORTED;
    const QueryP &p = q->qp;
    size_t total = (size_t)q->n_groups * p.n_buckets;
    if (!q->host_ready) {
        CU(cudaSetDevice(q->sh->device));
        for (uint32_t c = 0; c < p.n_calls; c++) {
            q->h_val[c].resize(total); q->h_ok[c].resize(total);
            CU(cudaMemcpy(q->h_val[c].data(), q->dense[c].val, total * 8, cudaMemcpyDeviceToHost));
            CU(cudaMemcpy(q->h_ok[c].data(), q->dense[c].ok, total, cudaMemcpyDeviceToHost));
            if (q->dense[c].tim) { q->h_tim[c].resize(total); CU(cudaMemcpy(q->h_tim[c].data(), q->dense[c].tim, total * 8, cudaMemcpyDeviceToHost)); }
        }
        q->host_ready = true; q->next_group = 0; q->next_row = 0;
    }
    int chunk = q->desc.chunk_size > 0 ? q->desc.chunk_size : 1024;
    uint32_t nc = p.n_calls;
    q->rv_val.assign(nc, {}); q->rv_bitmap.assign(nc, {}); q->rv_coltimes.assign(nc, {}); q->rv_times.clear(); q->rv_cols.assign(nc, og_colval_view{});
    while (q->next_group < q->n_groups) {
        uint32_t g = q->next_group;
        std::vector<int32_t> nil(nc, 0);
        int rows = 0;
        uint32_t b = q->next_row;
        uint32_t b_end = (uint32_t)std::min<uint64_t>(p.n_buckets, (uint64_t)b + (uint64_t)chunk);
        for (; b < b_end; b++) {
            const uint32_t bb = q->desc.ascending ? b : p.n_buckets - 1 - b;
            size_t i = (size_t)g * p.n_buckets + bb;
            bool any = false;
            for (uint32_t c = 0; c < nc; c++) any |= q->h_ok[c][i] != 0;
            if (!any) continue;
            int64_t row_time = p.start + (int64_t)bb * p.interval;
            if (q->desc.interval == 0) row_time = 0;
            for (uint32_t c = 0; c < nc; c++) {
                bool ok = q->h_ok[c][i] != 0;
                if ((size_t)(rows >> 3) >= q->rv_bitmap[c].size()) q->rv_bitmap[c].push_back(0);
                if (ok) {
                    q->rv_bitmap[c][rows >> 3] |= (uint8_t)(1 << (rows & 7));
                    if (p.calls[c].out_type == OG_TYPE_BOOL) q->rv_val[c].push_back((uint8_t)(q->h_val[c][i] != 0));
                    else { const uint8_t *pv = (const uint8_t *)&q->h_val[c][i]; q->rv_val[c].insert(q->rv_val[c].end(), pv, pv + 8); }
                } else nil[c]++;
                if (q->dense[c].tim) {
                    if (p.multi) q->rv_coltimes[c].push_back(ok ? q->h_tim[c][i] : 0);
                    else if (ok) row_time = q->h_tim[c][i];
                }
            }
            q->rv_times.push_back(row_time);
            rows++;
        }
        q->next_row = b_end;
        if (q->next_row >= p.n_buckets) { q->next_group++; q->next_row = 0; }
        if (rows == 0) continue;
        for (uint32_t c = 0; c < nc; c++) {
            og_colval_view &v = q->rv_cols[c];
            v.val = q->rv_val[c].data(); v.val_bytes = q->rv_val[c].size(); v.bitmap = q->rv_bitmap[c].data();
            v.times = (p.multi && q->dense[c].tim) ? q->rv_coltimes[c].data() : nullptr;
            v.type = p.calls[c].out_type; v.len = rows; v.nil_count = nil[c]; v.bitmap_offset = 0;
        }
        out->n_cols = nc; out->cols = q->rv_cols.data(); out->times = q->rv_times.data(); out->rows = rows; out->group = g;
        out->sid = q->desc.group_mode == OG_GROUP_PER_SERIES ? q->sh->sids[g] : 0;
        return OG_OK;
    }
    return OG_EOF;
}

}
namespace {
__global__ void k_decode_column(DirP d, uint32_t column, int type, uint32_t seg_begin, uint32_t seg_end, uint8_t *out, uint64_t stride,
                                uint32_t *rows_out, uint8_t *bitmap_out, uint32_t bitmap_stride, int *err) {
    uint32_t seg = seg_begin + blockIdx.x * blockDim.x + threadIdx.x;
    if (seg >= seg_end) return;
    uint8_t *o = out + (size_t)(seg - seg_begin) * stride;
    uint32_t rows = d.seg_rows[seg];
    size_t pi = (size_t)column * d.n_segments + seg;
    if (column == d.n_columns) {
        TimeDesc t;
        int rc = parse_time_page(d.data + d.page_off[pi], d.page_len[pi], t);
        if (rc == D_OK) {
            TimeIter it; it.init(t);
            for (uint32_t i = 0; i < t.rows; i++) ((int64_t *)o)[i] = it.next();
// ... 134 lines not shown
```

### opengemini_b200/csrc/compact.cu

```cuda
#include <algorithm>
#include <cstdio>
#include <cstdlib>
#include <cstring>
#include <string>
#include <vector>

#include "decode.cuh"
#include "internal.h"
#include "span_pass.h"

namespace ogpu {

#define COMPACT_RPS_DEFAULT 1000u

__device__ __forceinline__ bool compact_claim(MergeErr *e, int code) { return atomicCAS(&e->code, 0, code) == 0; }

__global__ void k_compact_decode(SrcDir d, const int32_t *col_types, uint32_t nsrc, const uint32_t *src_seg, const uint32_t *src_local0,
                                 const uint32_t *src_out0, const uint32_t *src_span, uint32_t R, int64_t *out_t, uint8_t *const *out_cells,
                                 uint8_t *out_ok, size_t out_rows, MergeErr *err) {
    const uint64_t i = (uint64_t)blockIdx.x * blockDim.x + threadIdx.x;
    if (i >= (uint64_t)nsrc * (d.n_columns + 1)) return;
    const uint32_t c = (uint32_t)(i / nsrc), j = (uint32_t)(i % nsrc);
    const uint32_t seg = src_seg[j], rows = d.seg_rows[seg];
    size_t g = src_out0[j] + src_local0[j] / R;
// ... 44 lines not shown
    if (slot >= rows) return;
    const int64_t t = out_t[i];
    if (slot == 0) seg_tmin[g] = t;
    if (slot == rows - 1) seg_tmax[g] = t;
    const bool has_prev = slot > 0 || (g > 0 && seg_span[g - 1] == seg_span[g]);
    if (has_prev && out_t[i - 1] >= t && compact_claim(err, M_REPEAT)) { err->span = (int)seg_span[g]; err->time = (long long)t; }
}

__global__ void k_compact_null_pages(const uint32_t *seg_rows, uint32_t n_segments, uint8_t *out) {
    const uint32_t g = blockIdx.x * blockDim.x + threadIdx.x;
    if (g >= n_segments) return;
    const uint32_t r = seg_rows[g];
    uint8_t *p = out + 8ull * g;
    p[0] = 44; p[1] = (uint8_t)(r >> 24); p[2] = (uint8_t)(r >> 16); p[3] = (uint8_t)(r >> 8); p[4] = (uint8_t)r;
    p[5] = p[6] = p[7] = 0;
}

struct CSpan {
    uint32_t series, first, end;
    uint64_t rows = 0, mask = 0;
    uint32_t n_new = 0, batch = 0, first_new = 0;
};

static uint64_t page_bound(uint32_t r) { return std::min<uint64_t>(MERGE_PAGE_BOUND, (14ull + (r + 7) / 8 + 8ull * r + 16 + 7) & ~7ull); }

static int compact_spans(og_shard *s, uint32_t R, const std::vector<uint32_t> &rows, std::vector<CSpan> &spans, std::vector<NewSegs> &batches, Scratch &blobs) {
    int rc;
    const uint32_t nc = s->n_columns, ncol1 = nc + 1;
    const uint64_t per_slot = 8 + 9ull * nc + 8 + (MERGE_PAGE_BOUND + R - 1) / R + (ncol1 * page_bound(R) + 8 + R - 1) / R;
    uint64_t cap;
    if ((rc = batch_cap_rows(per_slot, R, "OGPU_COMPACT_BATCH_ROWS", &cap))) return rc;
    Scratch keep;
    MergeErr *d_err; int32_t *d_types;
    if ((rc = keep.get(&d_err, 1)) || (rc = keep.get(&d_types, nc))) return rc;
    CU(cudaMemcpy(d_types, s->col_types.data(), nc * 4ull, cudaMemcpyHostToDevice));
    CU(cudaMemset(d_err, 0, sizeof(MergeErr)));
    SrcDir dir{s->d_data, s->d_page_off, s->d_page_len, s->d_seg_rows, s->n_segments, nc};
    size_t a = 0;
    while (a < spans.size()) {
        size_t b = a; uint64_t slots = 0;
        while (b < spans.size() && (b == a || slots + (uint64_t)spans[b].n_new * R <= cap)) slots += (uint64_t)spans[b++].n_new * R;
        if (slots >= 0xffffffffull) { set_error("a re-cut span holds %llu row slots (limit 2^32 - 2)", (unsigned long long)slots); return OG_E_UNSUPPORTED; }
        const uint32_t nsp = (uint32_t)(b - a);
        std::vector<uint32_t> h_seg, h_local0, h_out0, h_span, h_rows, h_seg_span;
        NewSegs ns;
        for (uint32_t k = 0; k < nsp; k++) {
            CSpan &sp = spans[a + k];
            sp.batch = (uint32_t)batches.size(); sp.first_new = ns.n;
            uint32_t local = 0;
            for (uint32_t g = sp.first; g < sp.end; g++) {
                h_seg.push_back(g); h_local0.push_back(local); h_out0.push_back(ns.n); h_span.push_back(k);
                local += rows[g];
            }
            for (uint32_t g = 0; g < sp.n_new; g++) { h_rows.push_back((uint32_t)std::min<uint64_t>(R, sp.rows - (uint64_t)g * R)); h_seg_span.push_back(k); }
            ns.n += sp.n_new;
        }
        const uint32_t nsrc = (uint32_t)h_seg.size(), NS = ns.n;
        const size_t out_rows = (size_t)NS * R;
        Scratch t;
        uint32_t *d_seg, *d_local0, *d_out0, *d_span, *d_rows, *d_seg_span; int64_t *out_t, *d_tmin, *d_tmax; uint8_t *out_ok; uint8_t **d_cols;
        std::vector<uint8_t *> h_cols(nc);
        if ((rc = t.get(&d_seg, nsrc)) || (rc = t.get(&d_local0, nsrc)) || (rc = t.get(&d_out0, nsrc)) || (rc = t.get(&d_span, nsrc)) ||
            (rc = t.get(&d_rows, NS)) || (rc = t.get(&d_seg_span, NS)) || (rc = t.get(&out_t, out_rows)) || (rc = t.get(&d_tmin, NS)) ||
            (rc = t.get(&d_tmax, NS)) || (rc = t.get(&out_ok, std::max<size_t>(1, (size_t)nc * out_rows))) || (rc = t.get(&d_cols, nc)))
            return rc;
        for (uint32_t c = 0; c < nc; c++)
            if ((rc = t.get(&h_cols[c], out_rows * (s->col_types[c] == OG_TYPE_BOOL ? 1 : 8)))) return rc;
        CU(cudaMemcpy(d_seg, h_seg.data(), nsrc * 4ull, cudaMemcpyHostToDevice));
        CU(cudaMemcpy(d_local0, h_local0.data(), nsrc * 4ull, cudaMemcpyHostToDevice));
        CU(cudaMemcpy(d_out0, h_out0.data(), nsrc * 4ull, cudaMemcpyHostToDevice));
        CU(cudaMemcpy(d_span, h_span.data(), nsrc * 4ull, cudaMemcpyHostToDevice));
        CU(cudaMemcpy(d_rows, h_rows.data(), NS * 4ull, cudaMemcpyHostToDevice));
        CU(cudaMemcpy(d_seg_span, h_seg_span.data(), NS * 4ull, cudaMemcpyHostToDevice));
        CU(cudaMemcpy(d_cols, h_cols.data(), nc * sizeof(uint8_t *), cudaMemcpyHostToDevice));
        const uint64_t nthr = (uint64_t)nsrc * ncol1;
        k_compact_decode<<<(unsigned)((nthr + 127) / 128), 128>>>(dir, d_types, nsrc, d_seg, d_local0, d_out0, d_span, R, out_t, d_cols, out_ok, out_rows, d_err);
        k_compact_check<<<(unsigned)((out_rows + 255) / 256), 256>>>(out_t, d_rows, d_seg_span, NS, R, d_tmin, d_tmax, d_err);
        CU(cudaGetLastError());
        MergeErr he;
        CU(cudaMemcpy(&he, d_err, sizeof he, cudaMemcpyDeviceToHost));
        if (he.code) {
            if (he.code == M_STRING) return string_refusal((unsigned long long)s->sids[spans[a + he.span].series], s->col_names[he.col], "compaction");
            if (he.code == M_REPEAT) {
                set_error("series sid %llu: time %lld does not follow the row before it inside a span compaction re-cuts (times must strictly ascend)",
                          (unsigned long long)s->sids[spans[a + he.span].series], he.time);
                return OG_E_CORRUPT;
            }
            return decode_failure(he.code, (uint32_t)he.seg, "shard");
        }
        uint8_t *blob;
        const uint64_t bcap = (uint64_t)NS * ncol1 * page_bound(R) + 8ull * NS;
        if ((rc = t.get(&blob, bcap))) return rc;
        uint64_t used = 0;
        if ((rc = encode_columns(s->col_types, out_t, h_cols, out_ok, out_rows, d_rows, NS, R, blob, bcap, ns, &used))) return rc;
        const bool any_string = std::any_of(s->col_types.begin(), s->col_types.end(), [](int32_t ty) { return ty == OG_TYPE_STRING; });
        const uint64_t nulls = used;
        if (any_string) {
            k_compact_null_pages<<<(NS + 127) / 128, 128>>>(d_rows, NS, blob + nulls);
            CU(cudaGetLastError());
            used += 8ull * NS;
        }
        for (uint32_t k = 0; k < nsp; k++) {
            const CSpan &sp = spans[a + k];
            for (uint32_t c = 0; c < nc; c++)
                for (uint32_t g = sp.first_new; g < sp.first_new + sp.n_new; g++) {
                    const size_t pi = (size_t)c * NS + g;
                    if (!((sp.mask >> c) & 1)) { ns.off[pi] = 0; ns.len[pi] = 0; }
                    else if (s->col_types[c] == OG_TYPE_STRING) { ns.off[pi] = nulls + 8ull * g; ns.len[pi] = 5; }
                }
        }
        ns.tmin.resize(NS); ns.tmax.resize(NS); ns.rows = h_rows;
        CU(cudaMemcpy(ns.tmin.data(), d_tmin, NS * 8ull, cudaMemcpyDeviceToHost));
        CU(cudaMemcpy(ns.tmax.data(), d_tmax, NS * 8ull, cudaMemcpyDeviceToHost));
        if ((rc = keep_blob(blob, used, blobs, ns))) return rc;
        batches.push_back(std::move(ns));
        a = b;
    }
    return OG_OK;
}

static int compact(og_shard *s, uint32_t R, og_compact_info &info) {
    int rc;
    const uint32_t nc = s->n_columns, NSER = s->n_series, NSEG = s->n_segments;
    std::vector<uint32_t> len((size_t)(nc + 1) * NSEG), rows(NSEG);
    if (NSEG) {
        CU(cudaMemcpy(rows.data(), s->d_seg_rows, NSEG * 4ull, cudaMemcpyDeviceToHost));
        CU(cudaMemcpy(len.data(), s->d_page_len, len.size() * 4, cudaMemcpyDeviceToHost));
    }
    std::vector<CSpan> spans;
    for (uint32_t u = 0; u < NSER; u++) {
        const uint32_t g0 = s->h_series_seg_begin[u], g1 = s->h_series_seg_begin[u + 1];
        if (g1 == g0) continue;
        uint64_t any = 0, all = ~0ull >> (64 - std::max(nc, 1u));
        if (nc == 0) all = 0;
        for (uint32_t g = g0; g < g1; g++) {
            uint64_t m = 0;
            for (uint32_t c = 0; c < nc; c++) if (len[(size_t)c * NSEG + g]) m |= 1ull << c;
            any |= m; all &= m;
        }
        uint32_t k = g1;
        if (any != all) k = g0;
        else
            for (uint32_t g = g0; g < g1; g++)
                if (rows[g] > R || (g + 1 < g1 && rows[g] < R)) { k = g; break; }
        if (k == g1) continue;
        CSpan sp; sp.series = u; sp.first = k; sp.end = g1; sp.mask = any;
        for (uint32_t g = k; g < g1; g++) sp.rows += rows[g];
        sp.n_new = (uint32_t)((sp.rows + R - 1) / R);
        spans.push_back(sp);
    }
    if (spans.empty()) return OG_OK;
    {
        std::lock_guard<std::mutex> il_lock(s->il_mu);
        for (og_shard::IlCol &c : s->il)
            dev_free_all(c.words, c.grp_off, c.grp_rows, c.grp_col, c.lane_seg, c.lane_rows, c.lane_series, c.lane_win, c.lane_t0, c.lane_dt, c.gen_list);
        s->il.assign(s->n_columns, og_shard::IlCol{});
    }
    cudaEvent_t ev0, ev1;
    CU(cudaEventCreate(&ev0)); CU(cudaEventCreate(&ev1));
    struct FreeEv { cudaEvent_t a, b; ~FreeEv() { cudaEventDestroy(a); cudaEventDestroy(b); } } free_ev{ev0, ev1};
    CU(cudaEventRecord(ev0, 0));
    std::vector<NewSegs> batches;
    Scratch blobs;
    if ((rc = compact_spans(s, R, rows, spans, batches, blobs))) return rc;
    Scratch maps;
    int32_t *d_identity;
    if ((rc = maps.get(&d_identity, nc))) return rc;
    {
        std::vector<int32_t> identity(nc);
        for (uint32_t c = 0; c < nc; c++) identity[c] = (int32_t)c;
        CU(cudaMemcpy(d_identity, identity.data(), nc * 4ull, cudaMemcpyHostToDevice));
    }
    SegSrc src[3] = {};
    src[SRC_SHARD] = SegSrc{s->d_page_off, s->d_page_len, s->d_seg_rows, s->d_tmin, s->d_tmax, nullptr, 0, d_identity, NSEG, nc};
    std::vector<const uint8_t *> regions = {s->d_data, nullptr};
    std::vector<uint32_t> m_first;
    Scratch m_own;
    if ((rc = batches_source(batches, nc, d_identity, 2, regions, m_own, src[SRC_MERGED], m_first))) return rc;
    std::vector<Run> runs;
    std::vector<uint32_t> o_ssb(NSER + 1, 0);
    uint32_t NOUT = 0;
    size_t si = 0;
    for (uint32_t u = 0; u < NSER; u++) {
        o_ssb[u] = NOUT;
        const uint32_t g0 = s->h_series_seg_begin[u], g1 = s->h_series_seg_begin[u + 1];
        const CSpan *sp = si < spans.size() && spans[si].series == u ? &spans[si++] : nullptr;
        const uint32_t kept_end = sp ? sp->first : g1;
        if (kept_end > g0) { runs.push_back(Run{NOUT, g0, u, SRC_SHARD}); NOUT += kept_end - g0; info.segments_kept += kept_end - g0; }
        if (sp) {
            runs.push_back(Run{NOUT, m_first[sp->batch] + sp->first_new, u, SRC_MERGED}); NOUT += sp->n_new;
            info.series_rewritten++; info.segments_rewritten_in += sp->end - sp->first; info.segments_rewritten_out += sp->n_new;
            info.rows_rewritten += sp->rows;
        }
    }
    o_ssb[NSER] = NOUT;
    std::unique_ptr<og_shard> out(new og_shard);
    Scratch out_own;
    Spliced sd;
    if ((rc = splice_and_gather(src, runs, NOUT, nc, regions, out_own, sd))) return rc;
    CU(cudaEventRecord(ev1, 0));
    if ((rc = spliced_totals(sd, nc, *out, "compaction"))) return rc;
    out->rows_merged = true;
    out->device = s->device; out->n_series = NSER; out->n_segments = NOUT; out->n_columns = nc;
    out->sids = s->sids; out->col_types = s->col_types; out->col_names = s->col_names; out->h_series_seg_begin = o_ssb;
    out->merge = s->merge;
    if ((rc = dalloc(&out->d_series_seg_begin, (size_t)NSER + 1)) || (rc = dalloc(&out->d_sids, (size_t)NSER))) return rc;
    CU(cudaMemcpy(out->d_series_seg_begin, o_ssb.data(), ((size_t)NSER + 1) * 4, cudaMemcpyHostToDevice));
    if (NSER) CU(cudaMemcpy(out->d_sids, s->sids.data(), (size_t)NSER * 8, cudaMemcpyHostToDevice));
    float ms = 0;
    CU(cudaEventElapsedTime(&ms, ev0, ev1));
    info.compact_ms = ms;
    take_spliced(out_own, sd, *out);
    CU(cudaDeviceSynchronize());
    std::swap(static_cast<ShardState &>(*s), static_cast<ShardState &>(*out));
    {
        std::lock_guard<std::mutex> il_lock(s->il_mu);
        s->il.assign(s->n_columns, og_shard::IlCol{});
    }
    return OG_OK;
}

}

using namespace ogpu;

extern "C" {

OG_API int og_shard_compact(og_shard *s, const og_compact_desc *d, og_compact_info *info) {
    if (!s || !d) { set_error("null argument"); return OG_E_INVAL; }
    if (d->flags) { set_error("og_compact_desc.flags must be 0 (got %u)", d->flags); return OG_E_INVAL; }
    if (d->rows_per_segment > 1000) { set_error("rows_per_segment must be 0 (1000) or 1..1000 (got %u)", d->rows_per_segment); return OG_E_INVAL; }
    const uint32_t R = d->rows_per_segment ? d->rows_per_segment : COMPACT_RPS_DEFAULT;
    std::lock_guard<std::mutex> lock(s->live->mu);
    if (s->live->n) { set_error("%u queries on this shard are still open: destroy them before compacting it", s->live->n); return OG_E_STATE; }
    CU(cudaSetDevice(s->device));
    og_compact_info ci{};
    const int rc = compact(s, R, ci);
    if (rc == OG_OK && info) *info = ci;
    return rc;
}

}
```

### opengemini_b200/csrc/fused_il.cuh

```cuda
#pragma once
#include "agg_kernels.cuh"

namespace ogpu {

__device__ __forceinline__ uint32_t smem_u32(const void *p) { return (uint32_t)__cvta_generic_to_shared(p); }
__device__ __forceinline__ uint32_t opaque(uint32_t x) { asm volatile("mov.u32 %0, %0;" : "+r"(x)); return x; }
template <int OFF> __device__ __forceinline__ uint32_t lds32o(uint32_t a) { uint32_t v; asm volatile("ld.shared.u32 %0, [%1+%2];" : "=r"(v) : "r"(a), "n"(OFF)); return v; }
__device__ __forceinline__ void mbar_init(uint32_t bar, uint32_t count) { asm volatile("mbarrier.init.shared::cta.b64 [%0], %1;" ::"r"(bar), "r"(count) : "memory"); }
__device__ __forceinline__ void mbar_init_fence() { asm volatile("fence.mbarrier_init.release.cluster;\nfence.proxy.async.shared::cta;" ::: "memory"); }
__device__ __forceinline__ void mbar_expect_tx(uint32_t bar, uint32_t bytes) { asm volatile("mbarrier.arrive.expect_tx.shared::cta.b64 _, [%0], %1;" ::"r"(bar), "r"(bytes) : "memory"); }
__device__ __forceinline__ void bulk_g2s(uint32_t dst, const void *src, uint32_t bytes, uint32_t bar) {
    asm volatile("cp.async.bulk.shared::cluster.global.mbarrier::complete_tx::bytes [%0], [%1], %2, [%3];" ::"r"(dst), "l"(src), "r"(bytes), "r"(bar) : "memory");
}
__device__ __forceinline__ bool mbar_wait(uint32_t bar, uint32_t parity) {
#pragma unroll 1
    for (uint32_t i = 0; i < (1u << 16); i++) {
        uint32_t ok;
        asm volatile("{\n.reg .pred p;\nmbarrier.try_wait.parity.shared::cta.b64 p, [%1], %2;\nselp.u32 %0, 1, 0, p;\n}" : "=r"(ok) : "r"(bar), "r"(parity) : "memory");
        if (ok) return true;
    }
    return false;
}

enum { FM_COUNT = 1, FM_SUM = 2, FM_MIN = 4, FM_MAX = 8, FM_FIRST = 16, FM_LAST = 32 };
enum { SEG_GENERAL = 0, SEG_FAST = 1, SEG_PACKED = 2 };

#ifndef OG_FAST_THREADS
#define OG_FAST_THREADS 128
#endif
#ifndef OG_FAST_MAXREG
#define OG_FAST_MAXREG 80
#endif
#ifndef OG_IL_NW
#define OG_IL_NW 64u
#endif
#ifndef OG_IL_B
#define OG_IL_B 16u
#endif
#ifndef OG_IL_K
#define OG_IL_K 10u
#endif
#ifndef OG_IL_UNROLL
#define OG_IL_UNROLL 2
#endif
#define OG_IL_NB (OG_IL_NW / OG_IL_B)
#define OG_IL_ROWS (OG_IL_NW + 2u)
#define OG_IL_PAD_WORDS 6u
#define OG_IL_HDR 7u
#define OG_IL_RAW_HDR 6u
#define OG_IL_NONE 0xffffffffu
#define OG_IL_PACKED 0x8000u
#define OG_IL_LOOKBITS (77u * OG_IL_K + 29u + 13u + 64u + 64u)
static_assert(OG_IL_K >= 2, "packed lanes: K*64 + 63 + 128 <= OG_IL_LOOKBITS needs K >= 2");
static_assert(OG_IL_NW % OG_IL_B == 0 && (OG_IL_NW & (OG_IL_NW - 1)) == 0, "ring geometry");
static_assert(OG_IL_NW - OG_IL_B > (OG_IL_LOOKBITS + 31u) / 32u + 2u, "ring too small for the round length: the slowest lane could not proceed");

struct IlP {
    const uint32_t *words;
    const uint64_t *grp_off;
    const uint32_t *grp_rows;
    const uint32_t *grp_col;
    const uint32_t *lane_seg;
    const uint32_t *lane_rows;
    const uint16_t *lane_win;
    const uint32_t *lane_series;
    const int64_t *lane_t0;
    const uint64_t *lane_dt;
};

__device__ __forceinline__ uint64_t udiv_est(uint64_t a, uint64_t b, double inv_b) {
    const double qd = __ull2double_rn(a) * inv_b;
    if ((a >> 63) || !(qd < 1125899906842624.0)) return a / b;
    uint64_t q = (uint64_t)qd;
    uint64_t r = a - q * b;
    if ((int64_t)r < 0) { do { q--; r += b; } while ((int64_t)r < 0); }
    else while (r >= b) { q++; r -= b; }
    return q;
}

__device__ __forceinline__ uint64_t fetch64(uint32_t col, uint32_t p) {
    uint32_t a = col + ((p << 2) & ((OG_IL_NW - 1) << 7));
    uint32_t a0 = lds32o<0>(a), a1 = lds32o<128>(a), a2 = lds32o<256>(a);
    uint32_t hi = __funnelshift_l(a1, a0, p), lo = __funnelshift_l(a2, a1, p);
    return ((uint64_t)hi << 32) | lo;
}

__device__ __forceinline__ Part fold32(int func, int type, bool multi, Part p, bool with_time) {
    constexpr uint32_t FULL = 0xffffffffu;
    if (func == OG_AGG_COUNT) { p.v = __reduce_add_sync(FULL, p.ok ? (uint32_t)p.v : 0u); p.ok = p.v != 0; return p; }
    if (type == OG_TYPE_FLOAT && func == OG_AGG_SUM) {
        double s = p.ok ? u2d(p.v) : 0.0;
#pragma unroll
        for (int o = 16; o; o >>= 1) s += __shfl_xor_sync(FULL, s, o);
        p.ok = __any_sync(FULL, p.ok != 0); p.v = d2u(s); return p;
    }
    if (type == OG_TYPE_FLOAT && !with_time && (func == OG_AGG_MIN || func == OG_AGG_MAX)) {
        double v = u2d(p.v); uint32_t ok = p.ok;
#pragma unroll
        for (int o = 16; o; o >>= 1) {
            const double ov = __shfl_xor_sync(FULL, v, o); const uint32_t ook = __shfl_xor_sync(FULL, ok, o);
            const bool keep = ok && (func == OG_AGG_MIN ? v <= ov : v >= ov);
            if (ook && !keep) v = ov;
            ok |= ook;
        }
        p.v = d2u(v); p.ok = ok; return p;
    }
    return warp_fold(func, type, multi, p, with_time);
}

#define OG_IL_WCAP 24u
__host__ __device__ inline uint32_t il_acc_bytes(uint32_t n_calls, bool times) { return OG_IL_WCAP * n_calls * (times ? 17u : 9u) + 8u & ~7u; }

template <int FM, bool TIMES, bool FOLD>
__global__ void __maxnreg__(OG_FAST_MAXREG) k_fused_il(QueryP q, ChunkP ch, IlP il, uint32_t grp_begin, uint32_t grp_end) {
    constexpr uint32_t NW = OG_IL_NW, B = OG_IL_B, NB = OG_IL_NB, K = OG_IL_K;
    constexpr uint32_t FULL = 0xffffffffu;
    constexpr uint32_t WPB = OG_FAST_THREADS / 32;
    constexpr int UNR = OG_IL_UNROLL;
    __shared__ __align__(128) uint32_t s_win[WPB * OG_IL_ROWS * 32];
    __shared__ __align__(8) uint64_t s_bar[WPB * NB];
    extern __shared__ __align__(8) uint8_t s_acc[];

#ifdef OG_IL_STATS
    const long long st_clk0 = clock64();
    long long st_wait = 0;
#endif
    const uint32_t lane = threadIdx.x & 31;
    const uint32_t wid = __reduce_max_sync(FULL, threadIdx.x >> 5);
    const uint32_t grp = grp_begin + blockIdx.x * WPB + wid;
    if (grp >= grp_end) return;
    const uint32_t rows_w = __reduce_max_sync(FULL, il.grp_rows[grp]);
    if (rows_w == 0) return;
    const size_t slot = (size_t)grp * 32 + lane;
    const uint32_t seg = il.lane_seg[slot];
    bool active = seg != OG_IL_NONE && seg >= ch.seg_begin && seg < ch.seg_end;
    if (!__any_sync(FULL, active)) return;
    const size_t e = 2 * (size_t)(seg - ch.seg_begin);

    uint32_t rows = 0, series = 0, r_lo = 0, r_hi = 0, lwin = 0;
    int64_t t0 = 0, dt = 1; uint64_t dtu = 1; double inv_dt = 1.0;
    const double inv_iv = 1.0 / __ull2double_rn((uint64_t)q.interval);
    if (active) {
        rows = il.lane_rows[slot]; lwin = il.lane_win[slot]; series = il.lane_series[slot];
        t0 = il.lane_t0[slot]; dtu = il.lane_dt[slot]; dt = (int64_t)dtu;
        inv_dt = 1.0 / __ull2double_rn(dtu);
        r_lo = 0; r_hi = rows - 1;
        if (t0 < q.tmin) { uint64_t k = udiv_est((uint64_t)(q.tmin - t0) + dtu - 1, dtu, inv_dt); r_lo = k > rows ? rows : (uint32_t)k; }
        { int64_t t_last = t0 + (int64_t)(rows - 1) * dt; if (t_last > q.tmax) { if (q.tmax < t0) r_lo = rows; else r_hi = (uint32_t)udiv_est((uint64_t)(q.tmax - t0), dtu, inv_dt); } }
        const uint64_t span = (uint64_t)q.n_buckets * (uint64_t)q.interval;
        const bool outside = r_lo <= r_hi && r_lo < rows &&
                             ((uint64_t)(t0 + (int64_t)r_lo * dt - q.start) >= span || (uint64_t)(t0 + (int64_t)r_hi * dt - q.start) >= span);
        if (outside) report_err(ch.err, D_CORRUPT, seg);
        if (r_lo > r_hi || r_lo >= rows || outside) { *(uint2 *)(ch.edge_bucket + e) = make_uint2(OG_NO_BUCKET, OG_NO_BUCKET); active = false; }
    }
    if (!__any_sync(FULL, active)) return;

    const uint32_t win = smem_u32(s_win) + wid * (OG_IL_ROWS * 128);
    const uint32_t col = opaque(win + lane * 4);
    const uint32_t bar0 = smem_u32(s_bar) + wid * (NB * 8);
    if (lane == 0) {
#pragma unroll
        for (uint32_t i = 0; i < NB; i++) mbar_init(bar0 + i * 8, 1);
        mbar_init_fence();
    }
    __syncwarp();
    const uint32_t total_b = rows_w / B;
    uint64_t goff = il.grp_off[grp];
    goff = ((uint64_t)__reduce_max_sync(FULL, (uint32_t)(goff >> 32)) << 32) | __reduce_max_sync(FULL, (uint32_t)goff);
    const uint32_t *gsrc = il.words + goff;
    uint32_t issued_b = 0, ready_b = 0;
    uint32_t hung = 0;
    uint64_t pol;
    asm("createpolicy.fractional.L2::evict_first.b64 %0, 1.0;" : "=l"(pol));
    auto issue = [&](uint32_t k_any) {
        const uint32_t k = __reduce_max_sync(FULL, k_any);
        const uint32_t s = k % NB, dst = win + s * (B * 128), bar = bar0 + s * 8;
        const uint32_t *src = gsrc + (size_t)k * (B * 32);
        if (s == 0)
            asm volatile("{\n.reg .pred p;\nelect.sync _|p, 0xffffffff;\n@p mbarrier.arrive.expect_tx.shared::cta.b64 _, [%0], %1;\n"
                         "@p cp.async.bulk.shared::cluster.global.mbarrier::complete_tx::bytes.L2::cache_hint [%2], [%3], %4, [%0], %6;\n"
                         "@p cp.async.bulk.shared::cluster.global.mbarrier::complete_tx::bytes.L2::cache_hint [%5], [%3], 256, [%0], %6;\n}"
                         ::"r"(bar), "r"(B * 128 + 256u), "r"(dst), "l"(src), "r"(B * 128), "r"(win + NW * 128), "l"(pol) : "memory");
        else
            asm volatile("{\n.reg .pred p;\nelect.sync _|p, 0xffffffff;\n@p mbarrier.arrive.expect_tx.shared::cta.b64 _, [%0], %1;\n"
                         "@p cp.async.bulk.shared::cluster.global.mbarrier::complete_tx::bytes.L2::cache_hint [%2], [%3], %1, [%0], %4;\n}"
                         ::"r"(bar), "r"(B * 128), "r"(dst), "l"(src), "l"(pol) : "memory");
    };
    {
        const uint32_t first = total_b < NB ? total_b : NB;
        for (uint32_t k = 0; k < first; k++) issue(k);
        issued_b = first;
    }

    uint32_t cur_b = 0, rb = 0xffffffffu, step_q = 0; uint64_t rem = 0, step_r = 0;
    if (active) {
        const int64_t t_lo = t0 + (int64_t)r_lo * dt;
        cur_b = (uint32_t)udiv_est((uint64_t)(t_lo - q.start), (uint64_t)q.interval, inv_iv);
        const uint64_t ivl = (uint64_t)q.interval;
        const uint64_t sq64 = udiv_est(ivl, dtu, inv_dt);
        step_q = sq64 > 0xffffffffull ? 0xffffffffu : (uint32_t)sq64;
        step_r = ivl - sq64 * dtu;
        uint64_t D = (uint64_t)(q.start + (int64_t)(cur_b + 1) * q.interval - t0) + dtu - 1;
        uint64_t qq = udiv_est(D, dtu, inv_dt); rem = D - qq * dtu; rb = qq > 0xffffffffull ? 0xffffffffu : (uint32_t)qq;
    }

    bool uni = false; uint32_t b0 = 0, b_end = 0;
    uint64_t *acc_v = nullptr; int64_t *acc_t = nullptr; uint8_t *acc_k = nullptr;
    if (FOLD) {
        const int leader = __ffs(__ballot_sync(FULL, active)) - 1;
        const int64_t t0L = __shfl_sync(FULL, t0, leader); const uint64_t dtL = __shfl_sync(FULL, dtu, leader);
        const uint32_t loL = __shfl_sync(FULL, r_lo, leader), hiL = __shfl_sync(FULL, r_hi, leader);
        b0 = __shfl_sync(FULL, cur_b, leader);
        const bool same = t0 == t0L && dtu == dtL && r_lo == loL && r_hi == hiL;
        const uint32_t b_last = active ? (uint32_t)udiv_est((uint64_t)(t0 + (int64_t)r_hi * dt - q.start), (uint64_t)q.interval, inv_iv) : b0;
        uni = __all_sync(FULL, !active || (same && b_last - b0 < OG_IL_WCAP));
        if (uni) {
            b_end = __reduce_max_sync(FULL, active ? b_last : 0u);
            const uint32_t nacc = OG_IL_WCAP * q.n_calls;
            uint8_t *base = s_acc + (size_t)wid * il_acc_bytes(q.n_calls, TIMES);
            acc_v = (uint64_t *)base; acc_t = (int64_t *)(base + (size_t)nacc * 8); acc_k = base + (size_t)nacc * (TIMES ? 16 : 8);
            for (uint32_t i = lane; i < nacc; i += 32) acc_k[i] = 0;
            __syncwarp();
        }
    }
    const uint32_t gcol = FOLD ? il.grp_col[grp] - ch.gc_col0 : 0;
    const bool fold_edges = FOLD && uni && b_end > b0;

    double sum = 0.0, mn = 0.0, mx = 0.0; uint64_t fi = 0, lastv = 0;
    uint32_t n_mn = 0, n_mx = 0;
    uint32_t w_row0 = r_lo;
    bool head_done = false; uint32_t head_b = OG_NO_BUCKET;
    uint32_t stop = 0, n_ev = 0;
    auto part_of = [&](int func, uint32_t cnt) -> Part {
        Part pp; pp.ok = cnt != 0; pp.v = 0; pp.t = 0;
        switch (func) {
        case OG_AGG_COUNT: pp.v = cnt; break;
        case OG_AGG_SUM: if (FM & FM_SUM) pp.v = d2u(sum); break;
        case OG_AGG_MIN: if (FM & FM_MIN) { pp.v = d2u(mn); if (TIMES) pp.t = t0 + (int64_t)(stop - n_mn) * dt; } break;
        case OG_AGG_MAX: if (FM & FM_MAX) { pp.v = d2u(mx); if (TIMES) pp.t = t0 + (int64_t)(stop - n_mx) * dt; } break;
        case OG_AGG_FIRST: if (FM & FM_FIRST) { pp.v = fi; pp.t = t0 + (int64_t)w_row0 * dt; } break;
        default: if (FM & FM_LAST) { pp.v = lastv; pp.t = t0 + (int64_t)(stop - 1) * dt; } break;
        }
        return pp;
    };
    auto kind_of = [&]() -> int { return !head_done ? 0 : stop > r_hi ? 1 : 2; };
    auto flush_lane = [&](int kind) {
        const uint32_t cnt = stop - w_row0;
#pragma unroll 1
        for (uint32_t c = 0; c < q.n_calls; c++) {
            const Part pp = part_of(q.calls[c].func, cnt);
            if (kind == 2) { if (pp.ok) store_cell(ch, (int)c, series, cur_b, pp); }
            else store_part(ch.edges[c], e + kind, pp);
        }
        if (kind == 0) { head_done = true; head_b = cur_b; }
    };
    auto flush_fold = [&](bool ev) {
        uint32_t pend = __ballot_sync(FULL, ev);
#pragma unroll 1
        while (pend) {
            const int leader = __ffs(pend) - 1;
            const uint32_t bL = __shfl_sync(FULL, cur_b, leader);
            const bool mine = ev && cur_b == bL;
            const uint32_t cnt = mine ? stop - w_row0 : 0;
            const uint32_t w = bL - b0;
#pragma unroll 1
            for (uint32_t c = 0; c < q.n_calls; c++) {
                const int func = q.calls[c].func, ftype = func == OG_AGG_COUNT ? OG_TYPE_INT : q.calls[c].type;
                const bool wt = func >= OG_AGG_MIN && !(q.multi && func <= OG_AGG_MAX);
                Part pp = fold32(func, ftype, q.multi != 0, part_of(func, cnt), wt);
                if ((int)lane == leader && pp.ok) {
                    const uint32_t i = c * OG_IL_WCAP + w;
                    Part a; a.ok = acc_k[i]; a.v = a.ok ? acc_v[i] : 0; a.t = (TIMES && a.ok) ? acc_t[i] : 0;
                    group_update(func, ftype, q.multi != 0, a, pp);
                    acc_v[i] = a.v; acc_k[i] = 1; if (TIMES) acc_t[i] = a.t;
                }
            }
            pend &= ~__ballot_sync(FULL, mine);
        }
        __syncwarp();
    };

    uint32_t qp = 0, sr = 0, kfast = 0, CM = 0, CE = 0, m = 64, tr = 0, bad = 0; uint64_t MASK = 0;
    bool done = !active;
    uint64_t val = 0;

#ifdef OG_IL_STATS
    long long st_w0 = clock64();
#endif
    if (issued_b && !mbar_wait(bar0, 0)) hung = 1; else ready_b = issued_b ? 1 : 0;
#ifdef OG_IL_STATS
    st_wait += clock64() - st_w0;
#endif
    if (active && !hung) {
        val = fetch64(col, 0); qp = 64;
        if (lwin & OG_IL_PACKED) {
            const uint32_t lead = (lwin >> 8) & 63u, mw = lwin & 127u;
            qp = 64 - lead; kfast = mw;
            MASK = mw ? (~0ull >> (64 - mw)) << (64 - lead - mw) : 0ull;
        } else { CM = 0; CE = 1; }
    }

    bool skipping = r_lo > 0;
    stop = skipping ? r_lo : (rb < r_hi + 1 ? rb : r_hi + 1);
    n_ev = stop;
    if (!skipping) { fi = val; mn = mx = u2d(val); n_mn = n_mx = n_ev; }
    if (done) n_ev = 0xffffffffu;

    auto retire = [&]() { done = true; n_ev = 0xffffffffu; CM = 0; CE = 0; MASK = 0; kfast = 0; };
    auto advance = [&]() {
        bool fin = false;
        if (skipping) { skipping = false; sum = 0.0; }
        else {
            fin = stop > r_hi;
            sum = 0.0;
            if (!fin) while (stop >= rb) {
                cur_b++;
                rem += step_r; uint32_t adv = step_q;
                if (rem >= dtu) { rem -= dtu; adv++; }
                rb = (rb > 0xffffffffu - adv) ? 0xffffffffu : rb + adv;
            }
        }
        if (fin) retire();
        else {
            w_row0 = stop;
            uint32_t nstop = rb < r_hi + 1 ? rb : r_hi + 1;
            n_ev = nstop - stop; stop = nstop;
            fi = val; mn = mx = u2d(val); n_mn = n_mx = n_ev;
        }
    };
    auto slow_record = [&]() {
        uint32_t p = qp + sr;
        const uint64_t x = fetch64(col, p);
        const uint32_t ctrl = (uint32_t)(x >> 62);
        if (ctrl < 2) { qp += 1; return; }
        if (ctrl == 3) {
            const uint32_t lm = (uint32_t)(x >> 51) & 0x7ff;
            uint32_t lead = lm >> 6; m = lm & 0x3f;
            if (m == 0) { m = 64; tr = 0; lead = 0; }
            else { if (lead + m > 64) { if (!done) bad = 1; lead = 0; m = 64; } tr = 64 - lead - m; }
            p += 13;
            const bool slowwin = lead < 2;
            sr = slowwin ? 0 : lead - 2;
            CM = slowwin ? 0u : 3u << (30 - sr); CE = slowwin ? 1u : 2u << (30 - sr);
            kfast = 2 + m;
            MASK = (m == 64 ? ~0ull : ((1ull << m) - 1)) << tr;
        } else p += 2;
        const uint64_t y = fetch64(col, p);
        const uint64_t sig = m == 64 ? y : (y >> (64 - m));
        p += m;
        val ^= sig << tr;
        qp = p - sr;
    };
    auto accumulate = [&](uint32_t k_in_run) {
        if (FM & FM_SUM) sum = sum + u2d(val);
        if (FM & FM_MIN) { if (mn > u2d(val)) { mn = u2d(val); if (TIMES) n_mn = n_ev - k_in_run; } }
        if (FM & FM_MAX) { if (mx < u2d(val)) { mx = u2d(val); if (TIMES) n_mx = n_ev - k_in_run; } }
        if (FM & FM_LAST) lastv = val;
    };
    auto record = [&](uint32_t k_in_run) {
        accumulate(k_in_run);
        const uint64_t x = fetch64(col, qp);
        const bool slow = (((uint32_t)(x >> 32) & CM) ^ CE) != 0;
        if (slow) slow_record();
        else { val ^= x & MASK; qp += kfast; }
    };
    auto record2 = [&](uint32_t k_in_run) {
        const uint64_t x0 = fetch64(col, qp), x1 = fetch64(col, qp + kfast);
        accumulate(k_in_run);
#ifdef OG_IL_REC2B
        uint64_t x1b = x1;
        if ((((uint32_t)(x0 >> 32) & CM) ^ CE) != 0) { slow_record(); x1b = fetch64(col, qp); }
        else { val ^= x0 & MASK; qp += kfast; }
        accumulate(k_in_run + 1);
        if ((((uint32_t)(x1b >> 32) & CM) ^ CE) != 0) slow_record();
        else { val ^= x1b & MASK; qp += kfast; }
#else
        if ((((uint32_t)(x0 >> 32) & CM) ^ CE) != 0) { slow_record(); record(k_in_run + 1); return; }
        val ^= x0 & MASK; qp += kfast;
        accumulate(k_in_run + 1);
        if ((((uint32_t)(x1 >> 32) & CM) ^ CE) != 0) slow_record();
        else { val ^= x1 & MASK; qp += kfast; }
#endif
    };

    uint32_t rounds_left = hung ? 0u : 40u * (__reduce_max_sync(FULL, rows) / K + 8u);
#ifdef OG_IL_STATS
    uint32_t st_common = 0, st_rare = 0, st_sit = 0, st_notgo = 0;
    const long long st_pro = clock64() - st_clk0;
#endif
    for (;;) {
        const uint32_t qmin = __reduce_min_sync(FULL, done ? 0xffffffffu : qp);
        if (qmin == 0xffffffffu) break;
        const uint32_t f = qmin < 32 ? 0u : (qmin - 32) >> 5;
#pragma unroll 1
        while (issued_b < total_b && (issued_b + 1) * B <= f + NW) { issue(issued_b); issued_b++; }
        const uint32_t qmax = __reduce_max_sync(FULL, done ? 0u : qp);
        uint32_t need_max = ((qmax + OG_IL_LOOKBITS) >> 5) + 1; if (need_max > rows_w) need_max = rows_w;
        uint32_t want_b = (need_max + B - 1) / B; if (want_b > issued_b) want_b = issued_b;
#ifdef OG_IL_STATS
        st_w0 = clock64();
#endif
#pragma unroll 1
        while (ready_b < want_b) { if (!mbar_wait(bar0 + (ready_b % NB) * 8, (ready_b / NB) & 1)) { hung = 1; break; } ready_b++; }
#ifdef OG_IL_STATS
        st_wait += clock64() - st_w0;
#endif
        if (hung) break;
        uint32_t need = ((qp + OG_IL_LOOKBITS) >> 5) + 1; if (need > rows_w) need = rows_w;
        bool go = done || need <= ready_b * B;
        uint32_t run = __reduce_min_sync(FULL, go ? n_ev : 0u);
        if (run >= K) {
            static_assert(K % 2 == 0, "records are decoded in pairs");
#pragma unroll UNR
            for (uint32_t k = 0; k < K; k += 2) record2(k);
            n_ev -= K;
#ifdef OG_IL_STATS
            st_common++;
#endif
            continue;
        }
#ifdef OG_IL_STATS
        st_rare++;
#endif
        if (rounds_left-- == 0) { hung = 2; break; }
        const bool all_go = __all_sync(FULL, go);
#ifdef OG_IL_STATS
        if (!all_go) { st_notgo++; st_sit += __popc(__ballot_sync(FULL, !go)); }
#endif
        uint32_t left = K;
        for (;;) {
            run = __reduce_min_sync(FULL, go ? n_ev : 0xffffffffu);
            if (run > left) run = left;
            if (all_go) {
#pragma unroll 1
                for (uint32_t k = 0; k < run; k++) record(k);
            } else {
#pragma unroll 1
                for (uint32_t k = 0; k < run; k++) if (go) record(k);
            }
            if (go) n_ev -= run;
            left -= run;
            if (left == 0) break;
            const bool ev = go && !done && n_ev == 0;
            if (FOLD && uni) {
                const bool fl = ev && !skipping;
                const int kind = kind_of();
                const bool to_acc = fl && (kind == 2 || fold_edges);
                if (fl && !to_acc) flush_lane(kind);
                if (__any_sync(FULL, to_acc)) flush_fold(to_acc);
                if (to_acc && kind == 0) head_done = true;
            } else if (ev && !skipping) flush_lane(kind_of());
            if (ev) advance();
            if (__all_sync(FULL, ev || done)) break;
        }
    }
    if (active && (qp >> 5) >= rows_w) bad = 1;
#ifdef OG_IL_STATS
    const long long st_e0 = clock64();
    if (lane == 0) { atomicAdd((unsigned *)&ch.err[4], st_common); atomicAdd((unsigned *)&ch.err[5], st_rare); atomicAdd((unsigned *)&ch.err[6], st_notgo); atomicAdd((unsigned *)&ch.err[7], st_sit); }
#endif
    while (ready_b < issued_b && hung != 1) { if (!mbar_wait(bar0 + (ready_b % NB) * 8, (ready_b / NB) & 1)) hung = 1; ready_b++; }
    if (hung && lane == 0) report_err(ch.err, D_WATCHDOG, (grp << 2) | hung);
    if (FOLD && uni) {
        __syncwarp();
        const uint32_t w_tail = fold_edges ? b_end - b0 : OG_IL_WCAP;
        for (uint32_t i = lane; i < OG_IL_WCAP * q.n_calls; i += 32) {
            if (!acc_k[i]) continue;
            const uint32_t c = i / OG_IL_WCAP, w = i % OG_IL_WCAP;
            Part a; a.ok = 1; a.v = acc_v[i]; a.t = TIMES ? acc_t[i] : 0;
            store_part(ch.gcells[c], (size_t)(b0 + w) * ch.gc_cols + (w == w_tail ? ch.gc_tail0 + gcol : gcol), a);
        }
    }
    if (FOLD && __any_sync(FULL, active && head_b != OG_NO_BUCKET) && lane == 0) ch.flags[1] = 1;
    if (active) {
        if (bad) report_err(ch.err, D_CORRUPT, seg);
        *(uint2 *)(ch.edge_bucket + e) = make_uint2(head_b, (head_b == OG_NO_BUCKET || cur_b == head_b) ? OG_NO_BUCKET : cur_b);
    }
#ifdef OG_IL_STATS
    if (lane == 0) {
        atomicAdd((unsigned long long *)(ch.err + 8), (unsigned long long)st_wait);
        const long long st_end = clock64();
        atomicAdd((unsigned long long *)(ch.err + 10), (unsigned long long)(st_end - st_clk0));
        atomicAdd((unsigned long long *)(ch.err + 12), (unsigned long long)st_pro);
        atomicAdd((unsigned long long *)(ch.err + 14), (unsigned long long)(st_end - st_e0));
    }
#endif
}

}
```

### opengemini_b200/csrc/il_build.cuh

```cuda
#pragma once
#include "fused_il.cuh"

namespace ogpu {

#define OG_IL_SUPER 4096u
#define OG_IL_WORD_BITS 24u

struct IlScanOut {
    uint32_t *seg_words;
    uint16_t *seg_win;
    unsigned long long *n_packed;
    int64_t *seg_t0;
    uint64_t *seg_dt;
    uint64_t *keys;
    uint32_t *vals;
    uint32_t *dom_cnt;
    uint32_t *misaligned;
};

__device__ inline bool il_delta_window(const uint8_t *page, uint32_t len, uint32_t rows, uint32_t m_stop, uint32_t &lead, uint32_t &m) {
    ColIter it;
    it.init(page, len, OG_TYPE_FLOAT, rows);
    uint64_t prev = 0, acc = 0;
    if (it.err != D_OK || !it.next(prev)) return false;
    for (uint32_t r = 1; r < rows && it.err == D_OK; r++) {
        uint64_t v = 0;
        if (!it.next(v)) return false;
        acc |= v ^ prev; prev = v;
        if ((r & 31) == 0 && m_stop < 64 && acc && 64 - __clzll((long long)acc) - (__ffsll((long long)acc) - 1) >= (int)m_stop) return false;
    }
    if (it.err != D_OK) return false;
    lead = acc ? (uint32_t)__clzll((long long)acc) : 0u;
    m = acc ? 64u - lead - (uint32_t)(__ffsll((long long)acc) - 1) : 0u;
    return true;
}

__global__ void k_il_scan(DirP d, int col, int col_type, uint32_t J, IlScanOut o) {
    uint32_t seg = blockIdx.x * blockDim.x + threadIdx.x;
    if (seg >= d.n_segments) return;
    uint8_t c = SEG_GENERAL; uint32_t nw = 0; int64_t t0 = 0; uint64_t dt = 0; uint16_t win = 0;
    const uint32_t rows = d.seg_rows[seg];
    if (rows >= 2 && rows < (1u << 22) && col_type == OG_TYPE_FLOAT) {
        size_t pi = (size_t)col * d.n_segments + seg, ti = (size_t)d.n_columns * d.n_segments + seg;
        const uint8_t *p = d.data + d.page_off[pi], *t = d.data + d.page_off[ti];
        uint32_t len = d.page_len[pi], tlen = d.page_len[ti];
        TimeDesc td;
        if (len >= 16 && tlen >= 16 && __ldg(p) == 31 && __ldg(t) == 32 && (__ldg(t + 5) >> 4) == 1 && ld_be32(p + 1) == rows &&
            parse_time_page(t, tlen, td) == D_OK && td.kind == 0 && td.delta > 0 && td.delta < (1ull << 40)) {
            const int tag = __ldg(p + 5) >> 4;
            if (tag == 3 && __ldg(p + 6) == 0x10) {
                c = SEG_FAST; nw = (len - OG_IL_HDR + 3) / 4 + OG_IL_PAD_WORDS;
            } else if (tag == 0 && len == OG_IL_RAW_HDR + 8 * (size_t)rows) {
                c = SEG_PACKED; nw = 2 * rows + OG_IL_PAD_WORDS; win = OG_IL_PACKED | 64u;
            }
            uint32_t m_stop = 64, lead, m;
            if (c == SEG_FAST) {
                const uint32_t T = nw > 2 + OG_IL_PAD_WORDS ? nw - 2 - OG_IL_PAD_WORDS : 0;
                const uint64_t ms = T ? (32ull * (T - 1)) / (rows - 1) + 1 : 0;
                m_stop = ms < 64 ? (uint32_t)ms : 64u;
            }
            if (c != SEG_GENERAL && il_delta_window(p, len, rows, m_stop, lead, m)) {
                const uint32_t pw = 2u + (uint32_t)(((uint64_t)(rows - 1) * m + 31) / 32) + OG_IL_PAD_WORDS;
                if (c == SEG_PACKED || pw < nw) { c = SEG_PACKED; nw = pw; win = (uint16_t)(OG_IL_PACKED | lead << 8 | m); }
            }
            if (nw >= (1u << OG_IL_WORD_BITS)) { c = SEG_GENERAL; nw = 0; win = 0; }
            t0 = td.t0; dt = td.delta;
        }
    }
    o.seg_words[seg] = nw; o.seg_win[seg] = win; o.seg_t0[seg] = t0; o.seg_dt[seg] = dt; o.vals[seg] = seg;
    {
        const unsigned am = __activemask(), pm = __ballot_sync(am, c == SEG_PACKED);
        if (pm && (threadIdx.x & 31) == (unsigned)(__ffs(am) - 1)) atomicAdd(o.n_packed, (unsigned long long)__popc(pm));
    }
    const uint32_t series = d.seg_series[seg];
    if (J) {
        const uint32_t ref = d.series_seg_begin[series / OG_IL_SUPER * OG_IL_SUPER] + (seg - d.series_seg_begin[series]);
        if (d.seg_tmin[seg] != d.seg_tmin[ref] || d.seg_tmax[seg] != d.seg_tmax[ref]) *o.misaligned = 1;
    }
    if (c == SEG_GENERAL) { o.keys[seg] = ~0ull; return; }
    const uint32_t dom = J ? (series / OG_IL_SUPER) * J + (seg - d.series_seg_begin[series]) : 0u;
    o.keys[seg] = ((uint64_t)dom << OG_IL_WORD_BITS) | nw;
    atomicAdd(&o.dom_cnt[dom], 1u);
}

struct IlAssign {
    const uint64_t *keys; const uint32_t *segs;
    const uint32_t *elem_first, *grp_first;
    const uint32_t *seg_words; const int64_t *seg_t0; const uint64_t *seg_dt; const uint16_t *seg_win;
    uint32_t *lane_seg, *lane_rows, *lane_series, *grp_col; uint16_t *lane_win; int64_t *lane_t0; uint64_t *lane_dt;
    uint32_t n_elig, J, cols_per_super;
};
__global__ void k_il_assign(DirP d, IlAssign a) {
    uint32_t i = blockIdx.x * blockDim.x + threadIdx.x;
    if (i >= a.n_elig) return;
    const uint32_t seg = a.segs[i], dom = (uint32_t)(a.keys[i] >> OG_IL_WORD_BITS);
    const uint32_t rank = i - a.elem_first[dom], g = a.grp_first[dom] + rank / 32;
    const size_t slot = (size_t)g * 32 + (rank & 31);
    a.lane_seg[slot] = seg;
    a.lane_rows[slot] = d.seg_rows[seg];
    a.lane_win[slot] = a.seg_win[seg];
    a.lane_series[slot] = d.seg_series[seg];
    a.lane_t0[slot] = a.seg_t0[seg]; a.lane_dt[slot] = a.seg_dt[seg];
    if ((rank & 31) == 0) a.grp_col[g] = (a.J ? dom / a.J : 0u) * a.cols_per_super + rank / 32;
}

__global__ void k_il_group_rows(uint32_t n_groups, const uint32_t *lane_seg, const uint32_t *seg_words, uint32_t *grp_rows) {
    uint32_t g = (blockIdx.x * blockDim.x + threadIdx.x) >> 5, lane = threadIdx.x & 31;
    if (g >= n_groups) return;
    uint32_t seg = lane_seg[(size_t)g * 32 + lane];
    uint32_t w = seg != OG_IL_NONE ? seg_words[seg] : 0;
#pragma unroll
    for (int o = 16; o; o >>= 1) w = max(w, __shfl_xor_sync(0xffffffffu, w, o));
    if (lane == 0) grp_rows[g] = (w + OG_IL_B - 1) / OG_IL_B * OG_IL_B;
}

__global__ void k_il_repack(DirP d, int col, const uint32_t *lane_seg, const uint16_t *lane_win, const uint64_t *grp_off, const uint32_t *grp_rows,
                            uint32_t n_groups, uint32_t *il) {
    uint32_t g = (blockIdx.x * blockDim.x + threadIdx.x) >> 5, lane = threadIdx.x & 31;
    if (g >= n_groups) return;
    const uint32_t nw = grp_rows[g];
    if (nw == 0) return;
    const size_t slot = (size_t)g * 32 + lane;
    const uint32_t seg = lane_seg[slot];
    const bool live = seg != OG_IL_NONE;
    const uint32_t win = live ? lane_win[slot] : 0u;
    const bool packed = (win & OG_IL_PACKED) != 0;
    const uint32_t *base = nullptr; uint32_t sh = 0, own_words = 0, a = 0, sel = 0;
    ColIter it;
    uint64_t prev = 0, pend = 0, acc = 0; uint32_t pbits = 0, nb = 0, left = 0, mw = 0, tr = 0;
    if (live) {
        const size_t pi = (size_t)col * d.n_segments + seg;
        const uint8_t *page = d.data + d.page_off[pi];
        if (packed) {
            it.init(page, d.page_len[pi], OG_TYPE_FLOAT, d.seg_rows[seg]);
            it.next(prev);
            pend = prev; pbits = 64;
            mw = win & 127u;
            tr = mw ? 64u - ((win >> 8) & 63u) - mw : 0u;
            left = mw ? d.seg_rows[seg] - 1 : 0u;
        } else {
            const uint8_t *s = page + OG_IL_HDR;
            base = (const uint32_t *)((uintptr_t)s & ~(uintptr_t)3);
            sh = (uint32_t)((uintptr_t)s & 3);
            own_words = (d.page_len[pi] - OG_IL_HDR + 3) / 4 + OG_IL_PAD_WORDS;
            a = __ldg(base);
            sel = sh == 0 ? 0x0123u : sh == 1 ? 0x1234u : sh == 2 ? 0x2345u : 0x3456u;
        }
    }
    uint32_t *out = il + grp_off[g] + lane;
    for (uint32_t w = 0; w < nw; w++) {
        uint32_t v = 0;
        if (packed) {
            while (nb < 32) {
                if (pbits == 0) {
                    if (left == 0) break;
                    uint64_t x = 0;
                    it.next(x);
                    pend = (x ^ prev) >> tr; prev = x; pbits = mw; left--;
                }
                const uint32_t k = pbits < 32 ? pbits : 32;
                acc |= ((pend >> (pbits - k)) & (~0ull >> (64 - k))) << (64 - nb - k);
                nb += k; pbits -= k;
            }
            v = (uint32_t)(acc >> 32);
            acc <<= 32; nb = nb > 32 ? nb - 32 : 0;
        } else if (w < own_words) {
            const uint32_t b = __ldg(base + w + 1);
            v = __byte_perm(a, b, sel);
            a = b;
        }
        out[(size_t)w * 32] = v;
    }
}

}
```

### opengemini_b200/csrc/internal.h

```cpp
#pragma once
#include <cuda_runtime.h>

#include <cstdint>
#include <memory>
#include <string>
#include <mutex>
#include <vector>

#include "../../include/ogpu.h"

#define OG_MAX_CALLS 8
#define OG_MAX_FILTER 16
#define OG_MAX_COLS 8

namespace ogpu {

void set_error(const char *fmt, ...);
int cuda_fail(cudaError_t e, const char *what, const char *file, int line);
int ensure_device();

inline cudaError_t dev_malloc(void **p, size_t bytes) { return cudaMallocAsync(p, bytes ? bytes : 1, (cudaStream_t)0); }
inline void dev_free(void *p) { if (p) cudaFreeAsync(p, (cudaStream_t)0); }
template <class... T> void dev_free_all(T *...p) { (dev_free((void *)p), ...); }
cudaError_t dev_mem_info(size_t *free_b, size_t *total_b);
#define CU(call) do { cudaError_t e__ = (call); if (e__ != cudaSuccess) return ::ogpu::cuda_fail(e__, #call, __FILE__, __LINE__); } while (0)

template <class T> int dalloc(T **p, size_t n) {
    *p = nullptr;
    if (n == 0) n = 1;
    cudaError_t e = dev_malloc((void **)p, n * sizeof(T));
    if (e != cudaSuccess) { set_error("cudaMalloc(%zu bytes) failed: %s", n * sizeof(T), cudaGetErrorString(e)); return e == cudaErrorMemoryAllocation ? OG_E_NOMEM : OG_E_CUDA; }
    return OG_OK;
}

struct Scratch {
    cudaStream_t stream = nullptr;
    std::vector<void *> bufs;
    Scratch() = default;
    explicit Scratch(cudaStream_t st) : stream(st) {}
    Scratch(const Scratch &) = delete;
    Scratch &operator=(const Scratch &) = delete;
    ~Scratch() {
        if (stream && !bufs.empty()) cudaStreamSynchronize(stream);
        for (void *p : bufs) dev_free(p);
    }
    template <class T> int get(T **p, size_t n) { int rc = dalloc(p, n); if (rc == OG_OK) bufs.push_back(*p); return rc; }
};

struct LiveQueries { std::mutex mu; uint32_t n = 0; };

struct ShardState {
    int device = 0;
    uint8_t *d_data = nullptr; uint64_t data_len = 0; bool owns_data = true;
    uint32_t n_series = 0, n_segments = 0, n_columns = 0;
    uint32_t max_seg_rows = 0;
    uint64_t irregular_time_pages = 0;
    uint64_t n_rows = 0, page_bytes = 0;
    uint64_t snappy_pages = 0, snappy_bytes_in = 0, snappy_bytes_out = 0;
    og_merge_info merge{1, 0, 0, 0, 0, 0, 0, 0, 0, 0};
    bool rows_merged = false;
    int64_t tmin = 0, tmax = 0;
    std::vector<uint64_t> sids;
    std::vector<int32_t> col_types;
    std::vector<std::string> col_names;
    std::vector<uint32_t> h_series_seg_begin;
    uint32_t *d_series_seg_begin = nullptr;
    uint32_t *d_seg_series = nullptr;
    uint32_t *d_seg_rows = nullptr;
    int64_t *d_tmin = nullptr, *d_tmax = nullptr;
    uint64_t *d_page_off = nullptr;
    uint32_t *d_page_len = nullptr;
    uint64_t *d_sids = nullptr;
};

}

struct og_shard : ogpu::ShardState {
    void *h_seg_buf = nullptr; size_t h_seg_buf_bytes = 0;
    void *d_seg_buf = nullptr; size_t d_seg_buf_bytes = 0;
    std::vector<og_colval_view> seg_views;
    struct IlCol { int state = 0;
                   uint32_t *words = nullptr; uint64_t *grp_off = nullptr; uint32_t *grp_rows = nullptr, *grp_col = nullptr;
                   uint32_t *lane_seg = nullptr, *lane_rows = nullptr, *lane_series = nullptr; uint16_t *lane_win = nullptr; int64_t *lane_t0 = nullptr; uint64_t *lane_dt = nullptr;
                   uint32_t *gen_list = nullptr; std::vector<uint32_t> gen_host;
                   uint32_t n_groups = 0, J = 0;
                   bool aligned = false;
                   uint32_t n_super = 1, cols_per_super = 0; std::vector<uint32_t> super_grp_first;
                   uint64_t n_words = 0, n_packed = 0;  double build_ms = 0; };
    std::vector<IlCol> il;
    std::mutex il_mu;
    std::shared_ptr<ogpu::LiveQueries> live = std::make_shared<ogpu::LiveQueries>();
    ~og_shard() {
        using ogpu::dev_free_all;
        if (owns_data) dev_free_all(d_data);
        dev_free_all(d_series_seg_begin, d_seg_series, d_seg_rows, d_tmin, d_tmax, d_page_off, d_page_len, d_sids, d_seg_buf);
        if (h_seg_buf) cudaFreeHost(h_seg_buf);
        for (IlCol &c : il)
            dev_free_all(c.words, c.grp_off, c.grp_rows, c.grp_col, c.lane_seg, c.lane_rows, c.lane_series, c.lane_win, c.lane_t0, c.lane_dt, c.gen_list);
    }
};

namespace ogpu {

struct CallP { int32_t func, col_slot, type, out_type; };
struct FilterP { int32_t kind, col_slot, op, type, const_is_float; double fval; int64_t ival; };

struct Tri { uint64_t *val; int64_t *tim; uint8_t *ok; };

struct QueryP {
    int64_t tmin, tmax, start, interval;
    uint32_t n_buckets, n_calls, n_filter, n_cols;
    int32_t multi;
    CallP calls[OG_MAX_CALLS];
    FilterP filter[OG_MAX_FILTER];
    int32_t col_index[OG_MAX_COLS];
    int32_t col_type[OG_MAX_COLS];
};

}

struct og_query {
    og_shard *sh = nullptr;
    std::shared_ptr<ogpu::LiveQueries> live;
    og_query_desc desc{};
    std::vector<og_call> calls;
    std::vector<og_filter_item> filter;
    std::vector<uint32_t> series_group;
    cudaStream_t stream = nullptr;
    cudaEvent_t ev0 = nullptr, ev1 = nullptr;
    ogpu::QueryP qp{};
    uint32_t n_groups = 0;
    bool ran = false; volatile int aborted = 0;
    ogpu::Tri dense[OG_MAX_CALLS]{};
    og_dense_col dense_cols[OG_MAX_CALLS]{};
    ogpu::Scratch bufs;
    og_stats stats{};
    std::vector<uint64_t> h_val[OG_MAX_CALLS];
    std::vector<uint8_t> h_ok[OG_MAX_CALLS];
    std::vector<int64_t> h_tim[OG_MAX_CALLS];
    bool host_ready = false;
    uint32_t next_group = 0, next_row = 0;
    std::vector<std::vector<uint8_t>> rv_val, rv_bitmap;
    std::vector<std::vector<int64_t>> rv_coltimes;
    std::vector<int64_t> rv_times;
    std::vector<og_colval_view> rv_cols;
    int path_used = 0;
    bool cells_dirty = true;
    bool planned = false;
    uint32_t chunk_series = 0, tile_segs = 0;
    int *d_err = nullptr;
    void *plan = nullptr;
    std::vector<cudaEvent_t> main_ev;
    void *merge_state = nullptr;
    ~og_query();
};
```

### opengemini_b200/csrc/merge.cu

```cuda
#include <algorithm>
#include <cstdio>
#include <cstdlib>
#include <cstring>
#include <map>
#include <string>
#include <vector>

#include <cub/device/device_scan.cuh>
#include <cub/device/device_segmented_sort.cuh>

#include "decode.cuh"
#include "internal.h"
#include "span_pass.h"

namespace ogpu {

int shard_finalize(og_shard *s, bool scan_snappy);
int check_desc(const og_shard_desc *d);
int upload_dir(og_shard *s, const uint32_t *series_seg_begin, const int64_t *seg_tmin, const int64_t *seg_tmax, const uint64_t *page_off,
               const uint32_t *page_len, const uint64_t *sids);
int encode_pages(int32_t type, int32_t is_time, const void *d_values, const uint8_t *d_valid, const uint32_t *d_rows, uint32_t n_segments,
                 uint32_t rps, uint8_t *d_out, uint64_t out_cap, uint64_t *d_page_off, uint32_t *d_page_len, uint64_t *total_bytes_out,
                 bool nan_raw);

// ... 525 lines not shown
}

int decode_failure(int device_code, uint32_t seg, const char *where) {
    set_error("segment %u of the %s failed to decode (device code %d)", seg, where, device_code);
    return device_code == D_UNSUPPORTED ? OG_E_UNSUPPORTED : OG_E_CORRUPT;
}

int batches_source(const std::vector<NewSegs> &batches, uint32_t nc, const int32_t *d_identity, uint32_t first_region,
                   std::vector<const uint8_t *> &regions, Scratch &own, SegSrc &out, std::vector<uint32_t> &m_first) {
    int rc;
    m_first.assign(batches.size() + 1, 0);
    for (size_t b = 0; b < batches.size(); b++) m_first[b + 1] = m_first[b] + batches[b].n;
    const uint32_t NM = m_first[batches.size()];
    if (!NM) return OG_OK;
    std::vector<uint64_t> off((size_t)(nc + 1) * NM); std::vector<uint32_t> len((size_t)(nc + 1) * NM), rows(NM), reg(NM);
    std::vector<int64_t> tmin(NM), tmax(NM);
    for (size_t b = 0; b < batches.size(); b++) {
        const NewSegs &B = batches[b];
        regions.push_back(B.blob);
        for (uint32_t g = 0; g < B.n; g++) {
            const uint32_t m = m_first[b] + g;
            for (uint32_t c = 0; c <= nc; c++) { off[(size_t)c * NM + m] = B.off[(size_t)c * B.n + g]; len[(size_t)c * NM + m] = B.len[(size_t)c * B.n + g]; }
            rows[m] = B.rows[g]; reg[m] = first_region + (uint32_t)b; tmin[m] = B.tmin[g]; tmax[m] = B.tmax[g];
        }
    }
    uint64_t *d_off; uint32_t *d_len, *d_rows, *d_reg; int64_t *d_tmin, *d_tmax;
    if ((rc = own.get(&d_off, off.size())) || (rc = own.get(&d_len, len.size())) || (rc = own.get(&d_rows, NM)) || (rc = own.get(&d_reg, NM)) ||
        (rc = own.get(&d_tmin, NM)) || (rc = own.get(&d_tmax, NM)))
        return rc;
    CU(cudaMemcpy(d_off, off.data(), off.size() * 8, cudaMemcpyHostToDevice));
    CU(cudaMemcpy(d_len, len.data(), len.size() * 4, cudaMemcpyHostToDevice));
    CU(cudaMemcpy(d_rows, rows.data(), NM * 4ull, cudaMemcpyHostToDevice));
    CU(cudaMemcpy(d_reg, reg.data(), NM * 4ull, cudaMemcpyHostToDevice));
    CU(cudaMemcpy(d_tmin, tmin.data(), NM * 8ull, cudaMemcpyHostToDevice));
    CU(cudaMemcpy(d_tmax, tmax.data(), NM * 8ull, cudaMemcpyHostToDevice));
    out = SegSrc{d_off, d_len, d_rows, d_tmin, d_tmax, d_reg, 0, d_identity, NM, nc};
    return OG_OK;
}

int spliced_totals(const Spliced &sd, uint32_t nc, ShardState &out, const char *who) {
    int rc;
    Scratch t;
    unsigned long long *d_tot; uint32_t *d_max; long long *d_range; int *d_err;
    if ((rc = t.get(&d_tot, 3)) || (rc = t.get(&d_max, 1)) || (rc = t.get(&d_range, 2)) || (rc = t.get(&d_err, 2))) return rc;
    const long long r0[2] = {INT64_MAX, INT64_MIN};
    CU(cudaMemset(d_tot, 0, 24)); CU(cudaMemset(d_max, 0, 4)); CU(cudaMemset(d_err, 0, 8));
    CU(cudaMemcpy(d_range, r0, 16, cudaMemcpyHostToDevice));
    if (sd.n) k_append_stats<<<(sd.n + 127) / 128, 128>>>(sd.data, sd.off, sd.len, sd.rows, sd.tmin, sd.tmax, sd.n, nc, d_tot, d_max, d_range, d_err);
    CU(cudaGetLastError());
    unsigned long long tot[3]; long long range[2]; int err[2];
    CU(cudaMemcpy(tot, d_tot, 24, cudaMemcpyDeviceToHost));
    CU(cudaMemcpy(&out.max_seg_rows, d_max, 4, cudaMemcpyDeviceToHost));
    CU(cudaMemcpy(range, d_range, 16, cudaMemcpyDeviceToHost));
    CU(cudaMemcpy(err, d_err, 8, cudaMemcpyDeviceToHost));
    if (err[0]) { set_error("segment %d: time page failed to parse after %s (device code %d)", err[1], who, err[0]); return OG_E_CORRUPT; }
    out.n_rows = tot[0]; out.page_bytes = tot[1]; out.irregular_time_pages = tot[2]; out.tmin = range[0]; out.tmax = range[1];
    return OG_OK;
}

void take_spliced(Scratch &own, Spliced &sd, ShardState &out) {
    auto take = [&](void *p) { own.bufs.erase(std::find(own.bufs.begin(), own.bufs.end(), p)); };
    for (void *p : {(void *)sd.off, (void *)sd.len, (void *)sd.rows, (void *)sd.series, (void *)sd.tmin, (void *)sd.tmax, (void *)sd.data}) take(p);
    out.d_page_off = sd.off; out.d_page_len = sd.len; out.d_seg_rows = sd.rows; out.d_seg_series = sd.series; out.d_tmin = sd.tmin; out.d_tmax = sd.tmax;
    out.d_data = sd.data; out.data_len = sd.data_len; out.owns_data = true;
}


static int add_files(og_shard *s, const og_shard_desc *files, const uint32_t *file_flags, uint32_t n_files, const char *who) {
    int rc;
    const uint32_t onc = s->n_columns, ONSER = s->n_series, ONSEG = s->n_segments;
    std::map<std::string, int32_t> schema;
    for (uint32_t c = 0; c < onc; c++) schema[s->col_names[c]] = s->col_types[c];
    if (schema.size() != onc) { set_error("the shard holds two columns of one name"); return OG_E_UNSUPPORTED; }
    std::map<uint64_t, uint32_t> series_of_sid;
    if ((rc = scan_files(files, n_files, who, schema, series_of_sid))) return rc;
    std::map<uint64_t, uint32_t> old_of_sid;
    for (uint32_t i = 0; i < ONSER; i++) {
        if (!old_of_sid.emplace(s->sids[i], i).second) { set_error("the shard holds sid %llu twice", (unsigned long long)s->sids[i]); return OG_E_UNSUPPORTED; }
        series_of_sid[s->sids[i]] = 0;
    }
    std::vector<std::string> names; std::vector<int32_t> types;
    for (auto &kv : schema) { names.push_back(kv.first); types.push_back(kv.second); }
    std::vector<uint64_t> sids;
    for (auto &kv : series_of_sid) { kv.second = (uint32_t)sids.size(); sids.push_back(kv.first); }
    const uint32_t nc = (uint32_t)names.size(), NSER = (uint32_t)sids.size();
    std::vector<int32_t> col_of_old(nc, -1), identity(nc);
    for (uint32_t c = 0; c < onc; c++) col_of_old[std::lower_bound(names.begin(), names.end(), s->col_names[c]) - names.begin()] = (int32_t)c;
    for (uint32_t c = 0; c < nc; c++) identity[c] = (int32_t)c;
    std::vector<int64_t> old_of(NSER, -1);
    for (auto &kv : old_of_sid) old_of[series_of_sid[kv.first]] = kv.second;
    FileDir fd;
    if ((rc = build_file_dir(files, n_files, names, fd))) return rc;
    const uint32_t NN = fd.n;
    std::vector<std::vector<uint32_t>> ordered(NSER), ooo(NSER);
    og_merge_info info{}; info.n_files = n_files;
    if ((rc = split_segments(files, n_files, file_flags, fd, series_of_sid, sids, ordered, ooo, info))) return rc;
    std::vector<uint32_t> probe_u, probe_old; std::vector<int64_t> probe_lo, probe_hi;
    std::vector<int64_t> span_lo(NSER, INT64_MAX), span_hi(NSER, INT64_MIN);
    for (uint32_t u = 0; u < NSER; u++) {
        span_hull(ooo[u], fd, &span_lo[u], &span_hi[u]);
        if (old_of[u] >= 0 && (!ordered[u].empty() || !ooo[u].empty())) {
            probe_u.push_back(u); probe_old.push_back((uint32_t)old_of[u]); probe_lo.push_back(span_lo[u]); probe_hi.push_back(span_hi[u]);
        }
    }
    const uint32_t NP = (uint32_t)probe_u.size();
    std::vector<uint32_t> old_a(NSER, 0), old_b(NSER, 0);
    {
        Scratch t;
        uint32_t *d_ser, *d_a, *d_b; int64_t *d_lo, *d_hi, *d_last;
        if ((rc = t.get(&d_ser, NP)) || (rc = t.get(&d_lo, NP)) || (rc = t.get(&d_hi, NP)) || (rc = t.get(&d_last, NP)) || (rc = t.get(&d_a, NP)) || (rc = t.get(&d_b, NP))) return rc;
        if (NP) {
            CU(cudaMemcpy(d_ser, probe_old.data(), NP * 4ull, cudaMemcpyHostToDevice));
            CU(cudaMemcpy(d_lo, probe_lo.data(), NP * 8ull, cudaMemcpyHostToDevice));
            CU(cudaMemcpy(d_hi, probe_hi.data(), NP * 8ull, cudaMemcpyHostToDevice));
            k_append_probe<<<(NP + 127) / 128, 128>>>(s->d_series_seg_begin, s->d_tmin, s->d_tmax, d_ser, d_lo, d_hi, NP, d_last, d_a, d_b);
            CU(cudaGetLastError());
            std::vector<int64_t> last(NP); std::vector<uint32_t> a(NP), b(NP);
            CU(cudaMemcpy(last.data(), d_last, NP * 8ull, cudaMemcpyDeviceToHost));
            CU(cudaMemcpy(a.data(), d_a, NP * 4ull, cudaMemcpyDeviceToHost));
            CU(cudaMemcpy(b.data(), d_b, NP * 4ull, cudaMemcpyDeviceToHost));
            for (uint32_t k = 0; k < NP; k++) {
                const uint32_t u = probe_u[k];
                if (!ordered[u].empty() && fd.tmin[ordered[u][0]] <= last[k]) {
                    set_error("series sid %llu: ordered file %u starts at %lld, not after the shard's last time %lld; only out-of-order files may overlap the shard",
                              (unsigned long long)sids[u], fd.src_file[ordered[u][0]], (long long)fd.tmin[ordered[u][0]], (long long)last[k]);
                    return OG_E_UNSUPPORTED;
                }
                old_a[u] = a[k]; old_b[u] = b[k];
            }
        }
    }
    auto n_old = [&](uint32_t u) { return old_of[u] < 0 ? 0u : s->h_series_seg_begin[old_of[u] + 1] - s->h_series_seg_begin[old_of[u]]; };
    auto g0_old = [&](uint32_t u) { return old_of[u] < 0 ? 0u : s->h_series_seg_begin[old_of[u]]; };
    std::vector<uint32_t> before(NSER), after_begin(NSER);
    std::vector<int> span_of(NSER, -1);
    std::vector<Span> span_store;
    for (uint32_t u = 0; u < NSER; u++) {
        const uint32_t no = n_old(u);
        const auto &o = ordered[u];
        if (ooo[u].empty()) { before[u] = after_begin[u] = no + (uint32_t)o.size(); continue; }
        uint32_t na, nb;
        span_bounds(o, fd, span_lo[u], span_hi[u], &na, &nb);
        before[u] = old_a[u] < no ? old_a[u] : no + na;
        after_begin[u] = old_b[u] < no ? old_b[u] : no + nb;
        Span sp; sp.series = u;
        span_of[u] = (int)span_store.size();
        span_store.push_back(std::move(sp));
    }
    std::unique_ptr<og_shard> nw;
    std::vector<uint32_t> new_rows;
    if ((rc = upload_files(files, n_files, names, types, s->device, fd, nw, new_rows))) return rc;
    {
        std::lock_guard<std::mutex> il_lock(s->il_mu);
        for (og_shard::IlCol &c : s->il)
            dev_free_all(c.words, c.grp_off, c.grp_rows, c.grp_col, c.lane_seg, c.lane_rows, c.lane_series, c.lane_win, c.lane_t0, c.lane_dt, c.gen_list);
        s->il.assign(s->n_columns, og_shard::IlCol{});
    }
    Scratch d_maps;
    int32_t *d_col_old, *d_identity;
    if ((rc = d_maps.get(&d_col_old, nc)) || (rc = d_maps.get(&d_identity, nc))) return rc;
    CU(cudaMemcpy(d_col_old, col_of_old.data(), nc * 4ull, cudaMemcpyHostToDevice));
    CU(cudaMemcpy(d_identity, identity.data(), nc * 4ull, cudaMemcpyHostToDevice));
    SegSrc src[3] = {};
    src[SRC_SHARD] = SegSrc{s->d_page_off, s->d_page_len, s->d_seg_rows, s->d_tmin, s->d_tmax, nullptr, 0, d_col_old, ONSEG, onc};
    src[SRC_FILES] = SegSrc{nw->d_page_off, nw->d_page_len, nw->d_seg_rows, nw->d_tmin, nw->d_tmax, nullptr, 1, d_identity, NN, nc};
    cudaEvent_t ev0, ev1;
    CU(cudaEventCreate(&ev0)); CU(cudaEventCreate(&ev1));
    struct FreeEv { cudaEvent_t a, b; ~FreeEv() { cudaEventDestroy(a); cudaEventDestroy(b); } } free_ev{ev0, ev1};
    CU(cudaEventRecord(ev0, 0));
    std::vector<NewSegs> batches;
    Scratch blobs, msrc_own;
    if (!span_store.empty()) {
        std::vector<Run> runs;
        uint32_t n_src = 0;
        for (auto &sp : span_store) {
            const uint32_t u = sp.series, no = n_old(u);
            const auto &o = ordered[u];
            const uint32_t ob = std::min(before[u], no), oe = std::min(after_begin[u], no);
            if (oe > ob) {
                runs.push_back(Run{n_src, g0_old(u) + ob, 0, SRC_SHARD});
                for (uint32_t k = 0; k < oe - ob; k++) { sp.src.push_back(n_src + k); sp.src_file.push_back(n_files); }
                n_src += oe - ob;
            }
            std::vector<uint32_t> news;
            for (uint32_t k = std::max(before[u], no); k < after_begin[u]; k++) news.push_back(o[k - no]);
            news.insert(news.end(), ooo[u].begin(), ooo[u].end());
            sort_oldest_first(news, fd, file_flags);
            for (uint32_t g : news) {
                runs.push_back(Run{n_src, g, 0, SRC_FILES});
                sp.src.push_back(n_src++); sp.src_file.push_back(fd.src_file[g]);
            }
            info.series_merged++;
            info.segments_rewritten_in += sp.src.size();
        }
        for (uint32_t u = 0; u < NSER; u++) for (uint32_t g : ooo[u]) info.out_of_order_rows += new_rows[g];
        Spliced ms;
        if ((rc = splice_and_gather(src, runs, n_src, nc, {s->d_data, nw->d_data}, msrc_own, ms))) return rc;
        {
            std::vector<uint32_t> rows(n_src);
            CU(cudaMemcpy(rows.data(), ms.rows, n_src * 4ull, cudaMemcpyDeviceToHost));
            for (auto &sp : span_store)
                for (uint32_t i : sp.src) { sp.src_rows.push_back(rows[i]); sp.rows += rows[i]; }
        }
        SrcDir dir;
        dir.data = ms.data ? ms.data : nw->d_data; dir.page_off = ms.off; dir.page_len = ms.len; dir.seg_rows = ms.rows; dir.n_segments = ms.n; dir.n_columns = nc;
        std::vector<Span *> sp;
        for (auto &x : span_store) sp.push_back(&x);
        uint64_t replaced = 0;
        if ((rc = merge_spans(dir, runs, types, names, sp, sids, n_files, batches, blobs, &replaced))) return rc;
        info.rows_replaced = replaced;
    }
    std::vector<uint32_t> m_first;
    std::vector<const uint8_t *> regions = {s->d_data, nw->d_data};
    Scratch m_own;
    if ((rc = batches_source(batches, nc, d_identity, 2, regions, m_own, src[SRC_MERGED], m_first))) return rc;
    std::vector<Run> runs;
    std::vector<uint32_t> o_ssb(NSER + 1, 0);
    uint32_t NOUT = 0;
    auto emit = [&](uint32_t u, uint32_t k0, uint32_t k1) {
        const uint32_t no = n_old(u);
        if (std::min(k1, no) > k0) { runs.push_back(Run{NOUT, g0_old(u) + k0, u, SRC_SHARD}); NOUT += std::min(k1, no) - k0; }
        for (uint32_t k = std::max(k0, no); k < k1; k++) runs.push_back(Run{NOUT++, ordered[u][k - no], u, SRC_FILES});
        info.segments_kept += k1 - k0;
    };
    for (uint32_t u = 0; u < NSER; u++) {
        o_ssb[u] = NOUT;
        const uint32_t total = n_old(u) + (uint32_t)ordered[u].size();
        emit(u, 0, before[u]);
        if (span_of[u] >= 0) {
            const Span &sp = span_store[span_of[u]];
            if (sp.n_new) { runs.push_back(Run{NOUT, m_first[sp.batch] + sp.first_new, u, SRC_MERGED}); NOUT += sp.n_new; }
            info.segments_rewritten_out += sp.n_new;
        }
        emit(u, after_begin[u], total);
    }
    o_ssb[NSER] = NOUT;
    std::unique_ptr<og_shard> out(new og_shard);
    Scratch out_own;
    Spliced sd;
    if ((rc = splice_and_gather(src, runs, NOUT, nc, regions, out_own, sd))) return rc;
    if (!sd.data) { sd.data = nw->d_data; sd.data_len = nw->data_len; nw->d_data = nullptr; out_own.bufs.push_back(sd.data); }
    CU(cudaEventRecord(ev1, 0));
    if ((rc = spliced_totals(sd, nc, *out, "the append"))) return rc;
    out->rows_merged = s->rows_merged || !batches.empty();
    if (!out->rows_merged) {
        out->snappy_pages = s->snappy_pages + nw->snappy_pages;
        out->snappy_bytes_in = s->snappy_bytes_in + nw->snappy_bytes_in; out->snappy_bytes_out = s->snappy_bytes_out + nw->snappy_bytes_out;
    }
    out->page_bytes = out->page_bytes - out->snappy_bytes_out + out->snappy_bytes_in;
    out->device = s->device; out->n_series = NSER; out->n_segments = NOUT; out->n_columns = nc;
    out->sids = sids; out->col_types = types; out->col_names = names; out->h_series_seg_begin = o_ssb;
    if ((rc = dalloc(&out->d_series_seg_begin, (size_t)NSER + 1)) || (rc = dalloc(&out->d_sids, (size_t)NSER))) return rc;
    CU(cudaMemcpy(out->d_series_seg_begin, o_ssb.data(), ((size_t)NSER + 1) * 4, cudaMemcpyHostToDevice));
    CU(cudaMemcpy(out->d_sids, sids.data(), (size_t)NSER * 8, cudaMemcpyHostToDevice));
    float ms = 0;
    CU(cudaEventElapsedTime(&ms, ev0, ev1));
    info.merge_ms = ms;
    info.rows_after_merge = out->n_rows;
    take_spliced(out_own, sd, *out);
    out->merge = info;
    CU(cudaDeviceSynchronize());
    std::swap(static_cast<ShardState &>(*s), static_cast<ShardState &>(*out));
    {
        std::lock_guard<std::mutex> il_lock(s->il_mu);
        s->il.assign(s->n_columns, og_shard::IlCol{});
    }
    return OG_OK;
}

}

using namespace ogpu;

extern "C" {

OG_API int og_shard_open_files(const og_shard_desc *files, const uint32_t *file_flags, uint32_t n_files, og_shard **out) {
    if (!files || !out || n_files == 0) { set_error("null argument or no files"); return OG_E_INVAL; }
    *out = nullptr;
    int rc = ensure_device(); if (rc) return rc;
    std::unique_ptr<og_shard> s(new og_shard);
    CU(cudaGetDevice(&s->device));
    s->h_series_seg_begin = {0};
    if ((rc = add_files(s.get(), files, file_flags, n_files, "og_shard_open_files"))) return rc;
    *out = s.release();
    return OG_OK;
}

OG_API int og_shard_append_files(og_shard *s, const og_shard_desc *files, const uint32_t *file_flags, uint32_t n_files) {
    if (!s || !files || n_files == 0) { set_error("null argument or no files"); return OG_E_INVAL; }
    std::lock_guard<std::mutex> lock(s->live->mu);
    if (s->live->n) { set_error("%u queries on this shard are still open: destroy them before appending files", s->live->n); return OG_E_STATE; }
    CU(cudaSetDevice(s->device));
    return add_files(s, files, file_flags, n_files, "og_shard_append_files");
}

OG_API int og_shard_merge_info(const og_shard *s, og_merge_info *out) {
    if (!s || !out) { set_error("null argument"); return OG_E_INVAL; }
    *out = s->merge;
    return OG_OK;
}

}
```

Baseline: 500.2 billion.

## Trim interleaved fetch to exact bytes, sparse gcell merge, persistent edge fold

The interleaved decoder now fetches only the words each lane group actually needs (a per-group fetch bound computed from rows and packed width) instead of the padded full stream, with a partial final bulk copy. The final gcell merge walks only live column ranges, unrolled four-wide, and clears ok flags as it consumes them, so the per-chunk memset of gcells is dropped after a clean run. The edge fold kernel becomes grid-stride with a grid capped at a multiple of the SM count. A fetch-bytes statistic is added. The risks are over-reads if the fetch bound is wrong and stale gcells if an error path skips the clearing.

```diff
diff --git a/include/ogpu.h b/include/ogpu.h
--- a/include/ogpu.h
+++ b/include/ogpu.h
@@ -156,6 +156,7 @@
     uint64_t general_segments;
     double merge_ms;
     uint64_t il_packed_segments;
+    uint64_t il_fetch_bytes;
 } og_stats;
 
 typedef struct og_shard og_shard;
diff --git a/opengemini_b200/_lib.py b/opengemini_b200/_lib.py
--- a/opengemini_b200/_lib.py
+++ b/opengemini_b200/_lib.py
@@ -73,7 +73,7 @@
                 ("dir_bytes", C.c_uint64), ("out_bytes", C.c_uint64), ("kernel_ms", C.c_double), ("h2d_ms", C.c_double), ("main_kernel_ms", C.c_double),
                 ("kernel_launches", C.c_uint32), ("path", C.c_int32), ("il_state", C.c_int32), ("per_series_cells_used", C.c_int32),
                 ("il_build_ms", C.c_double), ("il_bytes", C.c_uint64), ("general_segments", C.c_uint64), ("merge_ms", C.c_double),
-                ("il_packed_segments", C.c_uint64)]
+                ("il_packed_segments", C.c_uint64), ("il_fetch_bytes", C.c_uint64)]
 
 
 class SynthColumn(C.Structure):
diff --git a/opengemini_b200/csrc/agg_kernels.cuh b/opengemini_b200/csrc/agg_kernels.cuh
--- a/opengemini_b200/csrc/agg_kernels.cuh
+++ b/opengemini_b200/csrc/agg_kernels.cuh
@@ -25,6 +25,9 @@
     uint32_t *edge_bucket;
     Tri gcells[OG_MAX_CALLS];
     uint32_t gc_cols, gc_tail0, gc_edge0, gc_col0;
+    const uint2 *gc_live; uint32_t n_gc_live;
+    uint32_t n_gc_dense;
+    unsigned long long *fetch_bytes;
     uint32_t J;
     int *err;
     int *flags;
@@ -338,33 +341,34 @@
 
 __global__ void k_fix_edges_fold(DirP d, QueryP q, ChunkP ch) {
     if (ch.flags[1] == 0) return;
-    const uint32_t w = (blockIdx.x * blockDim.x + threadIdx.x) >> 5, lane = threadIdx.x & 31;
+    const uint32_t lane = threadIdx.x & 31;
     const uint32_t n_blk = (ch.series_end - ch.series_begin + 31) / 32;
-    if (w >= n_blk * ch.J) return;
-    const uint32_t blk = w / ch.J, j = w % ch.J;
-    const uint32_t series = ch.series_begin + blk * 32 + lane;
-    const bool in = series < ch.series_end;
-    const uint32_t seg = in ? d.series_seg_begin[series] + j : 0;
-    EdgeRuns r; r.hb = r.tb = OG_NO_BUCKET; r.head_leader = false; r.s_end = 0;
-    if (in) r = edge_runs(d, ch, seg, series);
     const uint32_t n_bk = (ch.gc_cols - ch.gc_edge0) / 3;
-    for (int which = 0; which < 2; which++) {
-        const uint32_t gcol = ch.gc_edge0 + (which ? 2u : (j & 1u)) * n_bk + ch.series_begin / 32 + blk - ch.gc_col0;
-        const bool has = r.hb != OG_NO_BUCKET && (which == 0 ? r.head_leader : r.tb != OG_NO_BUCKET);
-        const uint32_t b = which == 0 ? r.hb : r.tb;
-        const uint32_t hm = __ballot_sync(0xffffffffu, has);
-        if (hm == 0) continue;
-        const int leader = __ffs(hm) - 1;
-        const uint32_t bL = __shfl_sync(0xffffffffu, b, leader);
-        const bool unif = __all_sync(0xffffffffu, !has || b == bL) && bL < q.n_buckets;
-        if (!unif && has && b >= q.n_buckets) { report_err(ch.err, D_CORRUPT, seg); continue; }
-        for (uint32_t c = 0; c < q.n_calls; c++) {
-            Part acc = part_empty();
-            if (has) acc = edge_stitch(q, ch, r, seg, which, c);
-            if (unif) {
-                acc = warp_fold(q.calls[c].func, call_ftype(q, c), q.multi != 0, acc, call_has_time(q, c));
-                if ((int)lane == leader && acc.ok) store_part(ch.gcells[c], (size_t)bL * ch.gc_cols + gcol, acc);
-            } else if (has && acc.ok) store_cell(ch, (int)c, series, b, acc);
+    for (uint32_t w = (blockIdx.x * blockDim.x + threadIdx.x) >> 5; w < n_blk * ch.J; w += (gridDim.x * blockDim.x) >> 5) {
+        const uint32_t blk = w / ch.J, j = w % ch.J;
+        const uint32_t series = ch.series_begin + blk * 32 + lane;
+        const bool in = series < ch.series_end;
+        const uint32_t seg = in ? d.series_seg_begin[series] + j : 0;
+        EdgeRuns r; r.hb = r.tb = OG_NO_BUCKET; r.head_leader = false; r.s_end = 0;
+        if (in) r = edge_runs(d, ch, seg, series);
+        for (int which = 0; which < 2; which++) {
+            const uint32_t gcol = ch.gc_edge0 + (which ? 2u : (j & 1u)) * n_bk + ch.series_begin / 32 + blk - ch.gc_col0;
+            const bool has = r.hb != OG_NO_BUCKET && (which == 0 ? r.head_leader : r.tb != OG_NO_BUCKET);
+            const uint32_t b = which == 0 ? r.hb : r.tb;
+            const uint32_t hm = __ballot_sync(0xffffffffu, has);
+            if (hm == 0) continue;
+            const int leader = __ffs(hm) - 1;
+            const uint32_t bL = __shfl_sync(0xffffffffu, b, leader);
+            const bool unif = __all_sync(0xffffffffu, !has || b == bL) && bL < q.n_buckets;
+            if (!unif && has && b >= q.n_buckets) { report_err(ch.err, D_CORRUPT, seg); continue; }
+            for (uint32_t c = 0; c < q.n_calls; c++) {
+                Part acc = part_empty();
+                if (has) acc = edge_stitch(q, ch, r, seg, which, c);
+                if (unif) {
+                    acc = warp_fold(q.calls[c].func, call_ftype(q, c), q.multi != 0, acc, call_has_time(q, c));
+                    if ((int)lane == leader && acc.ok) store_part(ch.gcells[c], (size_t)bL * ch.gc_cols + gcol, acc);
+                } else if (has && acc.ok) store_cell(ch, (int)c, series, b, acc);
+            }
         }
     }
 }
@@ -472,10 +476,32 @@
     const Tri g = ch.gcells[c];
     Part acc = part_empty();
     const size_t row = (size_t)b * ch.gc_cols;
-    for (uint32_t col = lane; col < ch.gc_cols; col += 32) {
-        if (!g.ok[row + col]) continue;
-        Part p; p.ok = 1; p.v = g.val[row + col]; p.t = wt ? g.tim[row + col] : 0;
-        group_update(func, ftype, multi, acc, p);
+    const uint32_t n_rng = ch.n_gc_live + (ch.gc_edge0 < ch.gc_cols && ch.flags[1] != 0 ? 1u : 0u);
+    for (uint32_t r = 0; r < n_rng; r++) {
+        const uint2 R = r < ch.n_gc_live ? ch.gc_live[r] : make_uint2(ch.gc_edge0, ch.gc_cols);
+        const bool dense = r < ch.n_gc_dense;
+        constexpr uint32_t U = 4;
+        for (uint32_t c0 = R.x + ((lane - R.x) & 31u); c0 < R.y; c0 += 32 * U) {
+            uint32_t okv[U]; uint64_t vv[U]; int64_t tt[U];
+#pragma unroll
+            for (uint32_t u = 0; u < U; u++) {
+                const bool in = c0 + 32 * u < R.y;
+                okv[u] = in ? g.ok[row + c0 + 32 * u] : 0;
+                vv[u] = (in && dense) ? g.val[row + c0 + 32 * u] : 0;
+                tt[u] = (in && dense && wt) ? g.tim[row + c0 + 32 * u] : 0;
+            }
+            if (!dense) {
+#pragma unroll
+                for (uint32_t u = 0; u < U; u++) { vv[u] = okv[u] ? g.val[row + c0 + 32 * u] : 0; tt[u] = (okv[u] && wt) ? g.tim[row + c0 + 32 * u] : 0; }
+            }
+#pragma unroll
+            for (uint32_t u = 0; u < U; u++) {
+                if (!okv[u]) continue;
+                Part p; p.ok = 1; p.v = vv[u]; p.t = tt[u];
+                group_update(func, ftype, multi, acc, p);
+                g.ok[row + c0 + 32 * u] = 0;
+            }
+        }
     }
     acc = warp_fold(func, ftype, multi, acc, wt);
     if (lane == 0 && acc.ok) {
diff --git a/opengemini_b200/csrc/api.cu b/opengemini_b200/csrc/api.cu
--- a/opengemini_b200/csrc/api.cu
+++ b/opengemini_b200/csrc/api.cu
@@ -423,6 +423,7 @@
 
 }
 namespace {
+#define OG_ERR_INTS 18
 struct Plan {
     ChunkP ch; TileP tp; GroupP gp;
     bool fused;
@@ -431,6 +432,7 @@
     bool fast;
     bool blockmerge;
     bool fold;
+    uint32_t edge_blocks;
     int fm; bool times;
     IlP il;
     const og_shard::IlCol *ic;
@@ -566,6 +568,8 @@
     ic.n_groups = ng; ic.J = J; ic.aligned = J != 0 && misaligned == 0; ic.n_super = n_super; ic.cols_per_super = OG_IL_SUPER / 32 + 1;
     ic.super_grp_first.assign(n_super + 1, ng);
     for (uint32_t sp = 0; sp < n_super; sp++) ic.super_grp_first[sp] = grp_first[J ? sp * J : 0];
+    ic.super_ranks.assign(n_super, 0);
+    for (uint32_t i = 0; i < n_dom; i++) { uint32_t &r = ic.super_ranks[J ? i / J : 0]; r = std::max(r, (dom_cnt[i] + 31) / 32); }
     uint32_t *d_elem_first, *d_grp_first;
     if ((rc = tmp.get(&d_elem_first, n_dom)) || (rc = tmp.get(&d_grp_first, n_dom))) return rc;
     CU(cudaMemcpyAsync(d_elem_first, elem_first.data(), (size_t)n_dom * 4, cudaMemcpyHostToDevice, st));
@@ -573,7 +577,7 @@
     const size_t n_slots = (size_t)ng * 32;
     if ((rc = dalloc(&ic.lane_seg, n_slots)) || (rc = dalloc(&ic.lane_rows, n_slots)) || (rc = dalloc(&ic.lane_win, n_slots)) || (rc = dalloc(&ic.lane_series, n_slots)) ||
         (rc = dalloc(&ic.lane_t0, n_slots)) || (rc = dalloc(&ic.lane_dt, n_slots)) || (rc = dalloc(&ic.grp_col, (size_t)ng)) ||
-        (rc = dalloc(&ic.grp_rows, (size_t)ng)) || (rc = dalloc(&ic.grp_off, (size_t)ng))) return rc;
+        (rc = dalloc(&ic.grp_rows, (size_t)ng)) || (rc = dalloc(&ic.grp_fetch, (size_t)ng)) || (rc = dalloc(&ic.grp_off, (size_t)ng))) return rc;
     CU(cudaMemsetAsync(ic.lane_seg, 0xff, n_slots * 4, st));
     CU(cudaMemsetAsync(ic.lane_rows, 0, n_slots * 4, st));
     CU(cudaMemsetAsync(ic.lane_win, 0, n_slots * 2, st));
@@ -583,7 +587,7 @@
     as.lane_seg = ic.lane_seg; as.lane_rows = ic.lane_rows; as.lane_series = ic.lane_series; as.grp_col = ic.grp_col; as.lane_win = ic.lane_win; as.lane_t0 = ic.lane_t0; as.lane_dt = ic.lane_dt;
     as.n_elig = (uint32_t)n_elig; as.J = J; as.cols_per_super = ic.cols_per_super;
     k_il_assign<<<(unsigned)((n_elig + 255) / 256), 256, 0, st>>>(d, as);
-    k_il_group_rows<<<(unsigned)((n_slots + 255) / 256), 256, 0, st>>>(ng, ic.lane_seg, seg_words, ic.grp_rows);
+    k_il_group_rows<<<(unsigned)((n_slots + 255) / 256), 256, 0, st>>>(ng, ic.lane_seg, ic.lane_rows, ic.lane_win, seg_words, ic.grp_rows, ic.grp_fetch);
     CU(cudaGetLastError());
     std::vector<uint32_t> gw(ng); std::vector<uint64_t> go(ng);
     CU(cudaMemcpyAsync(gw.data(), ic.grp_rows, (size_t)ng * 4, cudaMemcpyDeviceToHost, st));
@@ -636,7 +640,7 @@
     uint32_t *d_grp_begin, *d_grp_series;
     if ((rc = q->bufs.get(&d_grp_begin, grp_begin.size()))) return rc;
     if ((rc = q->bufs.get(&d_grp_series, grp_series.size()))) return rc;
-    if ((rc = q->bufs.get(&q->d_err, 16))) return rc;
+    if ((rc = q->bufs.get(&q->d_err, OG_ERR_INTS))) return rc;
     CU(cudaMemcpyAsync(d_grp_begin, grp_begin.data(), grp_begin.size() * 4, cudaMemcpyHostToDevice, st));
     CU(cudaMemcpyAsync(d_grp_series, grp_series.data(), grp_series.size() * 4, cudaMemcpyHostToDevice, st));
     CU(cudaStreamSynchronize(st));
@@ -687,7 +691,7 @@
         max_chunk_segs = std::max(max_chunk_segs, s->h_series_seg_begin[b] - s->h_series_seg_begin[a]);
     }
     ChunkP &ch = pl->ch;
-    ch.err = q->d_err; ch.flags = q->d_err + 2;
+    ch.err = q->d_err; ch.flags = q->d_err + 2; ch.fetch_bytes = (unsigned long long *)(q->d_err + 16);
     ch.nb = p.n_buckets;
     ch.J = ic ? ic->J : 0;
     size_t chunk_cells = (size_t)std::min(q->chunk_series, s->n_series) * p.n_buckets;
@@ -703,9 +707,12 @@
     if ((rc = q->bufs.get(&ch.edge_bucket, 2 * (size_t)max_chunk_segs))) return rc;
     pl->blockmerge = !pl->fold && q->desc.group_mode == OG_GROUP_ALL && !(q->desc.flags & OG_Q_STRICT_ORDER) &&
                      (s->n_series > 2 * OG_MERGE_SB || getenv("OGPU_FORCE_BLOCKMERGE") );
+    std::vector<uint2> live;
     if (pl->blockmerge) {
-        ch.gc_edge0 = 0; ch.gc_col0 = 0;
+        ch.gc_col0 = 0;
         ch.gc_cols = (std::min(q->chunk_series, s->n_series) + OG_MERGE_SB - 1) / OG_MERGE_SB;
+        ch.gc_edge0 = ch.gc_cols;
+        live.push_back(make_uint2(0, ch.gc_cols)); ch.n_gc_dense = 1;
         const size_t n = (size_t)p.n_buckets * ch.gc_cols;
         for (uint32_t c = 0; c < p.n_calls; c++) {
             bool sel = p.calls[c].func >= OG_AGG_MIN;
@@ -717,6 +724,14 @@
     if (pl->fold) {
         ch.gc_tail0 = ic->n_super * ic->cols_per_super; ch.gc_edge0 = 2 * ch.gc_tail0; ch.gc_col0 = 0;
         ch.gc_cols = ch.gc_edge0 + 3 * ((s->n_series + 31) / 32);
+        for (uint32_t t = 0; t < 2; t++)
+            for (uint32_t sp = 0; sp < ic->n_super; sp++)
+                if (ic->super_ranks[sp]) live.push_back(make_uint2(t * ch.gc_tail0 + sp * ic->cols_per_super, t * ch.gc_tail0 + sp * ic->cols_per_super + ic->super_ranks[sp]));
+        ch.n_gc_dense = (uint32_t)live.size() / 2;
+        int n_sm = 0;
+        CU(cudaDeviceGetAttribute(&n_sm, cudaDevAttrMultiProcessorCount, s->device));
+        const size_t edge_warps = (size_t)((s->n_series + 31) / 32) * ic->J;
+        pl->edge_blocks = (uint32_t)std::max<size_t>(1, std::min<size_t>((edge_warps + 3) / 4, (size_t)n_sm * 8));
         const size_t n = (size_t)p.n_buckets * ch.gc_cols;
         for (uint32_t c = 0; c < p.n_calls; c++) {
             bool sel = p.calls[c].func >= OG_AGG_MIN;
@@ -725,8 +740,15 @@
             if (sel && (rc = q->bufs.get(&ch.gcells[c].tim, n))) return rc;
         }
     }
+    if (!live.empty()) {
+        uint2 *d_live;
+        if ((rc = q->bufs.get(&d_live, live.size()))) return rc;
+        CU(cudaMemcpyAsync(d_live, live.data(), live.size() * sizeof(uint2), cudaMemcpyHostToDevice, st));
+        CU(cudaStreamSynchronize(st));
+        ch.gc_live = d_live; ch.n_gc_live = (uint32_t)live.size();
+    }
     if (pl->fast) {
-        pl->il.words = ic->words; pl->il.grp_off = ic->grp_off; pl->il.grp_rows = ic->grp_rows; pl->il.grp_col = ic->grp_col;
+        pl->il.words = ic->words; pl->il.grp_off = ic->grp_off; pl->il.grp_fetch = ic->grp_fetch; pl->il.grp_col = ic->grp_col;
         pl->il.lane_seg = ic->lane_seg; pl->il.lane_rows = ic->lane_rows; pl->il.lane_win = ic->lane_win; pl->il.lane_series = ic->lane_series; pl->il.lane_t0 = ic->lane_t0; pl->il.lane_dt = ic->lane_dt;
         pl->fm = 0; pl->times = false;
         for (uint32_t c = 0; c < p.n_calls; c++) {
@@ -777,11 +799,15 @@
     DirP dir = make_dir(s);
     uint32_t launches = 0, n_chunks = (s->n_series + q->chunk_series - 1) / q->chunk_series;
     while (q->main_ev.size() < 2 * (size_t)n_chunks) { cudaEvent_t e; CU(cudaEventCreate(&e)); q->main_ev.push_back(e); }
-    CU(cudaMemsetAsync(q->d_err, 0, 64, st));
+    CU(cudaMemsetAsync(q->d_err, 0, OG_ERR_INTS * sizeof(int), st));
     CU(cudaEventRecord(q->ev0, st));
     const bool per_series = q->desc.group_mode == OG_GROUP_PER_SERIES;
     if (!per_series) { k_init_dense<<<(unsigned)((cells_dense + 255) / 256), 256, 0, st>>>(p, gp); launches++; }
     const bool clear_cells = !pl->fold || q->cells_dirty || n_chunks > 1;
+    if (pl->fold) {
+        if (q->gcells_dirty) for (uint32_t c = 0; c < p.n_calls; c++) CU(cudaMemsetAsync(ch.gcells[c].ok, 0, (size_t)p.n_buckets * ch.gc_cols, st));
+        q->gcells_dirty = true;
+    }
     uint64_t segs_scanned = 0; uint32_t ci = 0, chunks_run = 0;
     for (uint32_t a = 0; a < s->n_series; a += q->chunk_series, ci++) {
         if (q->aborted) { cudaStreamSynchronize(st); set_error("query aborted"); return OG_E_ABORTED; }
@@ -800,7 +826,7 @@
         }
         segs_scanned += nseg;
         if (clear_cells) for (uint32_t c = 0; c < p.n_calls; c++) CU(cudaMemsetAsync(ch.cells[c].ok, 0, chunk_cells, st));
-        if (pl->fold || pl->blockmerge) for (uint32_t c = 0; c < p.n_calls; c++) CU(cudaMemsetAsync(ch.gcells[c].ok, 0, (size_t)p.n_buckets * ch.gc_cols, st));
+        if (pl->blockmerge) for (uint32_t c = 0; c < p.n_calls; c++) CU(cudaMemsetAsync(ch.gcells[c].ok, 0, (size_t)p.n_buckets * ch.gc_cols, st));
         if (pl->fold && ci > 0) CU(cudaMemsetAsync(ch.flags + 1, 0, sizeof(int), st));
         CU(cudaEventRecord(q->main_ev[2 * chunks_run], st));
         if (pl->fused) {
@@ -846,7 +872,7 @@
         }
         CU(cudaEventRecord(q->main_ev[2 * chunks_run + 1], st));
         chunks_run++;
-        if (pl->fold) k_fix_edges_fold<<<(unsigned)(((size_t)((b - a + 31) / 32) * ch.J * 32 + 127) / 128), 128, 0, st>>>(dir, p, ch);
+        if (pl->fold) k_fix_edges_fold<<<pl->edge_blocks, 128, 0, st>>>(dir, p, ch);
         else k_fix_edges<<<(nseg + 127) / 128, 128, 0, st>>>(dir, p, ch);
         if (per_series) k_merge_per_series<<<dim3((unsigned)((chunk_cells + 255) / 256), p.n_calls), 256, 0, st>>>(p, ch, gp);
         else if (pl->blockmerge) k_merge_all_blocks<<<dim3((p.n_buckets + 127) / 128, (b - a + OG_MERGE_SB - 1) / OG_MERGE_SB, p.n_calls), 128, 0, st>>>(p, ch, gp);
@@ -857,8 +883,8 @@
     CU(cudaEventRecord(q->ev1, st));
     CU(cudaGetLastError());
     CU(cudaStreamSynchronize(st));
-    int err[16];
-    CU(cudaMemcpy(err, q->d_err, 64, cudaMemcpyDeviceToHost));
+    int err[OG_ERR_INTS];
+    CU(cudaMemcpy(err, q->d_err, sizeof err, cudaMemcpyDeviceToHost));
     if (getenv("OGPU_IL_STATS")) {
         unsigned long long wait, life, pro, epi;
         memcpy(&wait, err + 8, 8); memcpy(&life, err + 10, 8); memcpy(&pro, err + 12, 8); memcpy(&epi, err + 14, 8);
@@ -869,6 +895,7 @@
     }
     q->cells_dirty = err[2] != 0;
     if (err[0]) { set_error("segment %d failed to decode (device code %d)", err[1], err[0]); return map_dev_err(err[0]); }
+    q->gcells_dirty = false;
     float ms = 0; cudaEventElapsedTime(&ms, q->ev0, q->ev1);
     double main_ms = 0;
     for (uint32_t i = 0; i < chunks_run; i++) { float m = 0; cudaEventElapsedTime(&m, q->main_ev[2 * i], q->main_ev[2 * i + 1]); main_ms += m; }
@@ -886,6 +913,7 @@
         stt.general_segments = ic.state == 1 ? (uint64_t)ic.gen_host.size() : s->n_segments;
     }
     stt.per_series_cells_used = err[2] != 0;
+    memcpy(&stt.il_fetch_bytes, err + 16, 8);
     q->ran = true;
     return OG_OK;
 }
diff --git a/opengemini_b200/csrc/compact.cu b/opengemini_b200/csrc/compact.cu
--- a/opengemini_b200/csrc/compact.cu
+++ b/opengemini_b200/csrc/compact.cu
@@ -220,8 +220,7 @@
     if (spans.empty()) return OG_OK;
     {
         std::lock_guard<std::mutex> il_lock(s->il_mu);
-        for (og_shard::IlCol &c : s->il)
-            dev_free_all(c.words, c.grp_off, c.grp_rows, c.grp_col, c.lane_seg, c.lane_rows, c.lane_series, c.lane_win, c.lane_t0, c.lane_dt, c.gen_list);
+        for (og_shard::IlCol &c : s->il) c.free_dev();
         s->il.assign(s->n_columns, og_shard::IlCol{});
     }
     cudaEvent_t ev0, ev1;
diff --git a/opengemini_b200/csrc/fused_il.cuh b/opengemini_b200/csrc/fused_il.cuh
--- a/opengemini_b200/csrc/fused_il.cuh
+++ b/opengemini_b200/csrc/fused_il.cuh
@@ -52,13 +52,18 @@
 #define OG_IL_PACKED 0x8000u
 #define OG_IL_LOOKBITS (77u * OG_IL_K + 29u + 13u + 64u + 64u)
 static_assert(OG_IL_K >= 2, "packed lanes: K*64 + 63 + 128 <= OG_IL_LOOKBITS needs K >= 2");
+__host__ __device__ inline uint32_t il_fetch_words(uint32_t seg_words, uint32_t rows, uint32_t lane_win) {
+    if (!(lane_win & OG_IL_PACKED)) return seg_words;
+    return (uint32_t)((64ull + (uint64_t)rows * (lane_win & 127u)) >> 5) + 1u;
+}
+static_assert(OG_IL_PAD_WORDS >= 3u, "the packed fetch bound must stay inside the stored stream");
 static_assert(OG_IL_NW % OG_IL_B == 0 && (OG_IL_NW & (OG_IL_NW - 1)) == 0, "ring geometry");
 static_assert(OG_IL_NW - OG_IL_B > (OG_IL_LOOKBITS + 31u) / 32u + 2u, "ring too small for the round length: the slowest lane could not proceed");
 
 struct IlP {
     const uint32_t *words;
     const uint64_t *grp_off;
-    const uint32_t *grp_rows;
+    const uint32_t *grp_fetch;
     const uint32_t *grp_col;
     const uint32_t *lane_seg;
     const uint32_t *lane_rows;
@@ -129,7 +134,7 @@
     const uint32_t wid = __reduce_max_sync(FULL, threadIdx.x >> 5);
     const uint32_t grp = grp_begin + blockIdx.x * WPB + wid;
     if (grp >= grp_end) return;
-    const uint32_t rows_w = __reduce_max_sync(FULL, il.grp_rows[grp]);
+    const uint32_t rows_w = __reduce_max_sync(FULL, il.grp_fetch[grp]);
     if (rows_w == 0) return;
     const size_t slot = (size_t)grp * 32 + lane;
     const uint32_t seg = il.lane_seg[slot];
@@ -164,7 +169,7 @@
         mbar_init_fence();
     }
     __syncwarp();
-    const uint32_t total_b = rows_w / B;
+    const uint32_t total_b = (rows_w + B - 1) / B, last_bytes = (rows_w - (total_b - 1) * B) * 128u;
     uint64_t goff = il.grp_off[grp];
     goff = ((uint64_t)__reduce_max_sync(FULL, (uint32_t)(goff >> 32)) << 32) | __reduce_max_sync(FULL, (uint32_t)goff);
     const uint32_t *gsrc = il.words + goff;
@@ -174,17 +179,17 @@
     asm("createpolicy.fractional.L2::evict_first.b64 %0, 1.0;" : "=l"(pol));
     auto issue = [&](uint32_t k_any) {
         const uint32_t k = __reduce_max_sync(FULL, k_any);
-        const uint32_t s = k % NB, dst = win + s * (B * 128), bar = bar0 + s * 8;
+        const uint32_t s = k % NB, dst = win + s * (B * 128), bar = bar0 + s * 8, bytes = k + 1 == total_b ? last_bytes : B * 128;
         const uint32_t *src = gsrc + (size_t)k * (B * 32);
         if (s == 0)
             asm volatile("{\n.reg .pred p;\nelect.sync _|p, 0xffffffff;\n@p mbarrier.arrive.expect_tx.shared::cta.b64 _, [%0], %1;\n"
                          "@p cp.async.bulk.shared::cluster.global.mbarrier::complete_tx::bytes.L2::cache_hint [%2], [%3], %4, [%0], %6;\n"
                          "@p cp.async.bulk.shared::cluster.global.mbarrier::complete_tx::bytes.L2::cache_hint [%5], [%3], 256, [%0], %6;\n}"
-                         ::"r"(bar), "r"(B * 128 + 256u), "r"(dst), "l"(src), "r"(B * 128), "r"(win + NW * 128), "l"(pol) : "memory");
+                         ::"r"(bar), "r"(bytes + 256u), "r"(dst), "l"(src), "r"(bytes), "r"(win + NW * 128), "l"(pol) : "memory");
         else
             asm volatile("{\n.reg .pred p;\nelect.sync _|p, 0xffffffff;\n@p mbarrier.arrive.expect_tx.shared::cta.b64 _, [%0], %1;\n"
                          "@p cp.async.bulk.shared::cluster.global.mbarrier::complete_tx::bytes.L2::cache_hint [%2], [%3], %1, [%0], %4;\n}"
-                         ::"r"(bar), "r"(B * 128), "r"(dst), "l"(src), "l"(pol) : "memory");
+                         ::"r"(bar), "r"(bytes), "r"(dst), "l"(src), "l"(pol) : "memory");
     };
     {
         const uint32_t first = total_b < NB ? total_b : NB;
@@ -454,13 +459,14 @@
             if (__all_sync(FULL, ev || done)) break;
         }
     }
-    if (active && (qp >> 5) >= rows_w) bad = 1;
+    if (active && ((qp + ((lwin & OG_IL_PACKED) ? (lwin >> 8) & 63u : sr)) >> 5) >= rows_w) bad = 1;
 #ifdef OG_IL_STATS
     const long long st_e0 = clock64();
     if (lane == 0) { atomicAdd((unsigned *)&ch.err[4], st_common); atomicAdd((unsigned *)&ch.err[5], st_rare); atomicAdd((unsigned *)&ch.err[6], st_notgo); atomicAdd((unsigned *)&ch.err[7], st_sit); }
 #endif
     while (ready_b < issued_b && hung != 1) { if (!mbar_wait(bar0 + (ready_b % NB) * 8, (ready_b / NB) & 1)) hung = 1; ready_b++; }
     if (hung && lane == 0) report_err(ch.err, D_WATCHDOG, (grp << 2) | hung);
+    if (lane == 0 && issued_b) atomicAdd(ch.fetch_bytes, 128ull * min(issued_b * B, rows_w));
     if (FOLD && uni) {
         __syncwarp();
         const uint32_t w_tail = fold_edges ? b_end - b0 : OG_IL_WCAP;
diff --git a/opengemini_b200/csrc/il_build.cuh b/opengemini_b200/csrc/il_build.cuh
--- a/opengemini_b200/csrc/il_build.cuh
+++ b/opengemini_b200/csrc/il_build.cuh
@@ -104,14 +104,17 @@
     if ((rank & 31) == 0) a.grp_col[g] = (a.J ? dom / a.J : 0u) * a.cols_per_super + rank / 32;
 }
 
-__global__ void k_il_group_rows(uint32_t n_groups, const uint32_t *lane_seg, const uint32_t *seg_words, uint32_t *grp_rows) {
+__global__ void k_il_group_rows(uint32_t n_groups, const uint32_t *lane_seg, const uint32_t *lane_rows, const uint16_t *lane_win,
+                                const uint32_t *seg_words, uint32_t *grp_rows, uint32_t *grp_fetch) {
     uint32_t g = (blockIdx.x * blockDim.x + threadIdx.x) >> 5, lane = threadIdx.x & 31;
     if (g >= n_groups) return;
-    uint32_t seg = lane_seg[(size_t)g * 32 + lane];
+    const size_t slot = (size_t)g * 32 + lane;
+    uint32_t seg = lane_seg[slot];
     uint32_t w = seg != OG_IL_NONE ? seg_words[seg] : 0;
+    uint32_t f = seg != OG_IL_NONE ? il_fetch_words(w, lane_rows[slot], lane_win[slot]) : 0;
 #pragma unroll
-    for (int o = 16; o; o >>= 1) w = max(w, __shfl_xor_sync(0xffffffffu, w, o));
-    if (lane == 0) grp_rows[g] = (w + OG_IL_B - 1) / OG_IL_B * OG_IL_B;
+    for (int o = 16; o; o >>= 1) { w = max(w, __shfl_xor_sync(0xffffffffu, w, o)); f = max(f, __shfl_xor_sync(0xffffffffu, f, o)); }
+    if (lane == 0) { grp_rows[g] = (w + OG_IL_B - 1) / OG_IL_B * OG_IL_B; grp_fetch[g] = f; }
 }
 
 __global__ void k_il_repack(DirP d, int col, const uint32_t *lane_seg, const uint16_t *lane_win, const uint64_t *grp_off, const uint32_t *grp_rows,
diff --git a/opengemini_b200/csrc/internal.h b/opengemini_b200/csrc/internal.h
--- a/opengemini_b200/csrc/internal.h
+++ b/opengemini_b200/csrc/internal.h
@@ -81,12 +81,15 @@
     std::vector<og_colval_view> seg_views;
     struct IlCol { int state = 0;
                    uint32_t *words = nullptr; uint64_t *grp_off = nullptr; uint32_t *grp_rows = nullptr, *grp_col = nullptr;
+                   uint32_t *grp_fetch = nullptr;
                    uint32_t *lane_seg = nullptr, *lane_rows = nullptr, *lane_series = nullptr; uint16_t *lane_win = nullptr; int64_t *lane_t0 = nullptr; uint64_t *lane_dt = nullptr;
                    uint32_t *gen_list = nullptr; std::vector<uint32_t> gen_host;
                    uint32_t n_groups = 0, J = 0;
                    bool aligned = false;
                    uint32_t n_super = 1, cols_per_super = 0; std::vector<uint32_t> super_grp_first;
-                   uint64_t n_words = 0, n_packed = 0;  double build_ms = 0; };
+                   std::vector<uint32_t> super_ranks;
+                   uint64_t n_words = 0, n_packed = 0;  double build_ms = 0;
+                   void free_dev() { ogpu::dev_free_all(words, grp_off, grp_rows, grp_col, grp_fetch, lane_seg, lane_rows, lane_series, lane_win, lane_t0, lane_dt, gen_list); } };
     std::vector<IlCol> il;
     std::mutex il_mu;
     std::shared_ptr<ogpu::LiveQueries> live = std::make_shared<ogpu::LiveQueries>();
@@ -95,8 +98,7 @@
         if (owns_data) dev_free_all(d_data);
         dev_free_all(d_series_seg_begin, d_seg_series, d_seg_rows, d_tmin, d_tmax, d_page_off, d_page_len, d_sids, d_seg_buf);
         if (h_seg_buf) cudaFreeHost(h_seg_buf);
-        for (IlCol &c : il)
-            dev_free_all(c.words, c.grp_off, c.grp_rows, c.grp_col, c.lane_seg, c.lane_rows, c.lane_series, c.lane_win, c.lane_t0, c.lane_dt, c.gen_list);
+        for (IlCol &c : il) c.free_dev();
     }
 };
 
@@ -146,6 +148,7 @@
     std::vector<og_colval_view> rv_cols;
     int path_used = 0;
     bool cells_dirty = true;
+    bool gcells_dirty = true;
     bool planned = false;
     uint32_t chunk_series = 0, tile_segs = 0;
     int *d_err = nullptr;
diff --git a/opengemini_b200/csrc/merge.cu b/opengemini_b200/csrc/merge.cu
--- a/opengemini_b200/csrc/merge.cu
+++ b/opengemini_b200/csrc/merge.cu
@@ -701,8 +701,7 @@
     if ((rc = upload_files(files, n_files, names, types, s->device, fd, nw, new_rows))) return rc;
     {
         std::lock_guard<std::mutex> il_lock(s->il_mu);
-        for (og_shard::IlCol &c : s->il)
-            dev_free_all(c.words, c.grp_off, c.grp_rows, c.grp_col, c.lane_seg, c.lane_rows, c.lane_series, c.lane_win, c.lane_t0, c.lane_dt, c.gen_list);
+        for (og_shard::IlCol &c : s->il) c.free_dev();
         s->il.assign(s->n_columns, og_shard::IlCol{});
     }
     Scratch d_maps;
```

Result: faster. 511.5 billion, median of 6 (+2.3%).
